# FelTris/durf

Hardware: AMD Instinct MI355X
Metric: train_rays_per_sec (higher is better)
Workload: dtype bf16

## Files before the change

### durf_amd/_sigs.py

```python
import ctypes as C

vp, i32, f32, u64 = C.c_void_p, C.c_int, C.c_float, C.c_size_t

SIGS = {
    'durf_last_error': (C.c_char_p, []),
    'durf_version': (i32, []),
    'durf_dispatch_seen': (i32, []),
    'durf_dispatch_reset': (i32, []),
    'durf_step_policy': (C.c_uint, [u64]),
    'durf_overlap_min_rows': (u64, []),
    'durf_mlp_param_count': (u64, [i32, i32]),
    'durf_mlp_layer_offset': (u64, [i32, i32, i32, i32]),
    'durf_wpack_fwd_bytes': (u64, [i32]),
    'durf_wpack_bwd_bytes': (u64, [i32]),
    'durf_pack_weights': (i32, [vp, i32, i32, vp, vp, vp]),
    'durf_pack_weights_all': (i32, [vp, vp, i32, vp, vp, i32, vp, u64, i32, vp, vp]),
    'durf_ray_setup': (i32, [vp, i32, i32, vp, vp, vp, vp, vp, vp, vp, vp]),
    'durf_ray_setup_masked': (i32, [vp, i32, i32, vp, vp, vp, vp, vp, vp, vp, vp, vp]),
    'durf_compact_hits': (i32, [vp, i32, i32, vp, vp, vp, vp]),
    'durf_compact_classes': (i32, [vp, i32, i32, i32, vp, vp, vp, vp, vp]),
    'durf_compact_all': (i32, [vp, i32, i32, i32, vp, vp, vp, vp, vp, vp, vp, vp]),
    'durf_ray_prologue': (i32, [vp, i32, i32, i32, vp, vp, vp, vp, vp, vp, vp, vp, vp, vp, vp, vp, vp, i32, vp, vp, vp, u64, C.c_uint32, C.c_uint32, vp]),
    'durf_ray_prologue_pack': (i32, [vp, i32, i32, i32, vp, vp, vp, vp, vp, vp, vp, vp, vp, vp, vp, vp, vp, i32, vp, vp, vp, u64, C.c_uint32, C.c_uint32, vp, vp, i32, vp, vp, i32, vp, u64, i32, vp, vp, vp, u64]),
    'durf_ray_prologue_pack_masked': (i32, [vp, i32, i32, i32, vp, vp, vp, vp, vp, vp, vp, vp, vp, vp, vp, vp, vp, i32, vp, vp, vp, u64, C.c_uint32, C.c_uint32, vp, vp, i32, vp, vp, i32, vp, u64, i32, vp, vp, vp, u64, vp]),
# ... 27 lines not shown
    'durf_forward_workspace_bytes': (u64, [i32, i32, i32]),
    'durf_forward': (i32, [vp, vp, vp, u64]),
    'durf_render_image_workspace_bytes': (u64, [i32, i32, i32, i32]),
    'durf_render_image': (i32, [vp, vp, u64, i32, vp, vp, vp, vp, u64]),
    'durf_forward_masked': (i32, [vp, vp, vp, vp, u64]),
    'durf_render_layers_workspace_bytes': (u64, [u64, i32, i32, i32, i32]),
    'durf_render_layers': (i32, [vp, vp, vp, u64, i32, vp, vp, vp, vp, vp, vp, vp, vp, vp, u64]),
    'durf_camera_rays': (i32, [vp, C.POINTER(f32), i32, i32, f32, f32, vp, vp, vp, vp, vp, vp]),
    'durf_render_trajectory_workspace_bytes': (u64, [i32, i32, i32, i32, i32]),
    'durf_render_trajectory': (i32, [vp, vp, vp, vp, i32, i32, C.POINTER(f32), C.POINTER(f32), f32, f32, i32, vp, vp, vp, vp, vp, vp, u64]),
    'durf_train_workspace_bytes': (u64, [i32, i32, i32, i32, u64]),
    'durf_train_workspace_bytes_flags': (u64, [i32, i32, i32, i32, u64, i32]),
    'durf_prefetch_join': (i32, [vp]),
    'durf_loss_backward': (i32, [vp, vp, vp, u64]),
    'durf_train_step': (i32, [vp, vp, vp, u64]),
    'durf_comm_available': (i32, []),
    'durf_comm_unique_id': (i32, [vp]),
    'durf_comm_init': (i32, [i32, i32, vp, C.POINTER(vp)]),
    'durf_comm_destroy': (i32, [vp]),
    'durf_allreduce_sum': (i32, [vp, vp, vp, u64]),
    'durf_mlp_f32_act_floats': (u64, [i32, i32]),
    'durf_mlp_f32_dz_floats': (u64, [i32, i32]),
    'durf_mlp_f32_dw_scratch_floats': (u64, [i32, i32, i32]),
    'durf_mlp_f32_wstream_floats': (u64, [i32]),
    'durf_mlp_f32_pack': (i32, [vp, i32, i32, i32, vp, u64, vp]),
    'durf_mlp_fwd_f32': (i32, [vp, i32, i32, u64, i32, vp, vp, vp, vp, vp, vp, vp, vp]),
    'durf_mlp_bwd_f32': (i32, [vp, i32, i32, u64, i32, vp, vp, vp, vp, vp, vp, vp, vp]),
    'durf_mlp_dw_f32': (i32, [vp, i32, i32, u64, i32, vp, vp, vp, i32, vp, vp]),
    'durf_bkgd_const_trunk_f32': (i32, [vp, vp, vp]),
    'durf_bkgd_hit_rays_f32': (i32, [vp, i32, vp, vp, vp, vp, vp, vp]),
    'durf_objf32_act_stride': (u64, [i32, i32]),
    'durf_objf32_dz_stride': (u64, [i32, i32]),
    'durf_encode_obj_f32_batch': (i32, [vp, i32, i32, i32, vp, vp, vp, vp, vp, vp, C.POINTER(f32), i32, vp]),
    'durf_objf32_fwd_batch': (i32, [vp, i32, i32, i32, vp, vp, vp, vp, vp, u64, vp, vp, vp, vp, vp, vp, vp, C.POINTER(f32), i32]),
    'durf_objf32_bwd_batch': (i32, [vp, i32, i32, i32, vp, vp, vp, vp, u64, vp, vp, vp, vp]),
    'durf_mlp_f32_pack_x3': (i32, [vp, i32, vp, u64, vp]),
    'durf_objf32_bwd_batch_x3': (i32, [vp, i32, i32, i32, vp, vp, vp, vp, u64, vp, vp, vp, vp]),
    'durf_objf32_dw_batch': (i32, [vp, i32, i32, i32, vp, i32, C.POINTER(vp), C.POINTER(vp), i32, vp, vp, u64]),
    'durf_obj_enc_stride': (u64, [i32, i32]),
    'durf_obj_view_stride': (u64, [i32, i32]),
    'durf_obj_dzout_stride': (u64, [i32, i32]),
    'durf_pack_weights_batch': (i32, [vp, i32, i32, i32, vp, u64, vp, vp]),
    'durf_obj_fwd_batch': (i32, [vp, i32, i32, i32, vp, vp, vp, vp, vp, vp, C.POINTER(f32), i32, vp, vp, vp, vp, vp, vp, vp]),
    'durf_obj_bwd_batch': (i32, [vp, i32, i32, i32, vp, vp, vp, vp, vp, vp, vp, vp]),
    'durf_obj_bwd_batch_levels': (i32, [vp, i32, i32, i32, i32, vp, vp, C.POINTER(vp), vp, C.POINTER(vp), C.POINTER(vp), C.POINTER(vp)]),
    'durf_mlp_bwd_obj': (i32, [vp, u64, i32, vp, vp, vp, vp, vp, vp, vp, vp, vp, vp, i32, i32, i32, vp, vp, C.POINTER(vp), vp, C.POINTER(vp), C.POINTER(vp), C.POINTER(vp)]),
    'durf_obj_dw_batch': (i32, [vp, i32, i32, i32, vp, i32, C.POINTER(vp), C.POINTER(vp), C.POINTER(vp), C.POINTER(vp), C.POINTER(vp), i32, vp, vp, vp, u64, vp]),
    'durf_obj_dw_partials': (i32, [vp, i32, i32, i32, vp, i32, C.POINTER(vp), C.POINTER(vp), C.POINTER(vp), C.POINTER(vp), C.POINTER(vp), vp, vp]),
    'durf_dw_finalize_all': (i32, [vp, i32, i32, C.POINTER(u64), C.POINTER(i32), C.POINTER(vp), vp, vp, vp, vp, i32, i32, i32, vp, i32, i32, vp, vp, vp, u64, vp]),
    'durf_encode_obj_bwd': (i32, [vp, i32, i32, i32, vp, vp, vp, vp, vp, vp, vp, vp, vp, vp, C.POINTER(f32), vp, vp, i32, i32]),
    'durf_encode_obj_bwd_batch': (i32, [vp, i32, i32, i32, vp, vp, vp, vp, vp, vp, vp, vp, vp, vp, C.POINTER(f32), vp, vp, i32, i32]),
    'durf_encode_obj_bwd_levels': (i32, [vp, i32, i32, i32, i32, vp, vp, C.POINTER(vp), C.POINTER(vp), vp, vp, vp, vp, vp, vp, C.POINTER(f32), vp, vp, i32, i32]),
    'durf_encode_bkgd_bwd_batch': (i32, [vp, i32, i32, i32, vp, vp, vp, vp, vp, vp, vp, vp, vp, vp, vp, vp, vp, f32, vp, vp, i32]),
    'durf_pose_finish': (i32, [vp, i32, vp, vp, i32, i32, vp]),
    'durf_optim_scratch_floats': (u64, [u64]),
    'durf_stats_scrub': (i32, [vp, i32, i32, i32, vp, vp, vp, vp, vp, vp, C.POINTER(vp), C.POINTER(f32), i32, vp, C.POINTER(vp), i32, u64, vp, f32, f32, vp, vp, u64, i32, u64, u64]),
    'durf_adam_apply': (i32, [vp, u64, vp, vp, vp, vp, f32, f32, i32, vp, vp]),
    'durf_poison_multi_hit': (i32, [vp, u64, vp, vp, u64, i32, u64, u64]),
    'durf_clip_adam': (i32, [vp, u64, vp, vp, vp, vp, f32, f32, f32, f32, i32, vp, vp]),
    'durf_weight_decay': (i32, [vp, u64, vp, vp, u64, u64, f32, vp, vp]),
    'durf_gen_batch': (i32, [vp, i32, i32, C.POINTER(f32), vp, f32, f32, vp, vp, vp, i32, vp, vp, vp, vp, vp, vp, vp, vp, vp, vp]),
    'durf_ssim_scratch_floats': (u64, [i32, i32, i32, i32]),
    'durf_ssim': (i32, [vp, i32, i32, i32, vp, vp, f32, i32, vp, f32, f32, vp, vp, vp]),
    'durf_eval_scratch_bytes': (u64, [i32, i32, i32]),
    'durf_eval_frames': (i32, [vp, i32, i32, i32, vp, vp, vp, vp, vp, vp, vp, u64]),
    'durf_vis_scratch_bytes': (u64, [i32, i32, i32]),
    'durf_vis_stats': (i32, [vp, i32, i32, i32, vp, vp, vp, u64]),
    'durf_vis_depth': (i32, [vp, i32, i32, i32, vp, vp, vp, i32, i32, f32, vp, vp, vp]),
    'durf_vis_normals': (i32, [vp, i32, i32, i32, vp, vp, vp, i32, i32, vp, vp]),
    'durf_vis_sinebow': (i32, [vp, u64, vp, vp, vp]),
    'durf_vis_turbo_lut': (i32, [vp]),
}


DURF_MAX_OBJ = 16
DURF_MAX_LEVELS = 8
DURF_MAX_CAMS = 8
DURF_W_BKGD = 256
DURF_W_OBJ = 128
DURF_ENC_CONTRACT = 1
DURF_ENC_NO_INTEGRATION = 2
DURF_ENC_CYLINDER = 4
DURF_FWD_RAW_FULL = 8
DURF_ENC_DIM = 64
DURF_VIEW_DIM = 32
DURF_DISPATCH_FWD256_8W = 0x1
DURF_DISPATCH_FWD256_4W = 0x2
DURF_DISPATCH_FWD128_SAMPLE = 0x4
DURF_DISPATCH_FWD128_MSPLIT = 0x8
DURF_DISPATCH_BWD256_8W = 0x10
DURF_DISPATCH_BWD256_4W = 0x20
DURF_DISPATCH_BWD128_SAMPLE = 0x40
DURF_DISPATCH_BWD128_MSPLIT = 0x80
DURF_DISPATCH_DW256_256WG = 0x100
DURF_DISPATCH_DW256_512WG = 0x200
DURF_DISPATCH_DW128_128WG = 0x400
DURF_DISPATCH_DW128_256WG = 0x800
DURF_DISPATCH_FWD_ENC = 0x1000
DURF_DISPATCH_FWD_RAW_FULL = 0x2000
DURF_DISPATCH_FWD_TAIL = 0x4000
DURF_DISPATCH_F32_DW_TILE = 0x8000
DURF_DISPATCH_F32_DW_B2 = 0x10000
DURF_DISPATCH_BWD_POSE = 0x20000
DURF_DISPATCH_FWD_MIX = 0x40000
DURF_DISPATCH_BWD_MIX = 0x80000
DURF_LAYERLOG_SELECT = 0x100000
DURF_LAYERLOG_PASS2 = 0x200000
DURF_LAYERLOG_BOX_MASK = 0x400000
DURF_LAYERLOG_TRAJ_RAYS = 0x800000
DURF_LAYERLOG_TRAJ_POSE = 0x1000000
DURF_LAYERLOG_TRAJ_PACK = 0x2000000
DURF_OVERLAP_MIN_ROWS = 262144
DURF_POLICY_SIDE_FWD = 0x1
DURF_POLICY_SIDE_BWD = 0x2
DURF_POLICY_SIDE_DW = 0x4
DURF_POLICY_MSPLIT = 0x8
DURF_POLICY_MIX = 0x10


class durf_loss_level(C.Structure):
    _fields_ = [
        ('raw_bkgd', vp),
        ('raw_obj', vp * DURF_MAX_OBJ),
        ('t_vals', vp),
        ('norm', vp),
        ('mults', f32 * 6),
        ('level', i32),
        ('draw', vp),
        ('terms', vp),
        ('rgb_out', vp),
        ('depth_out', vp),
        ('acc_out', vp),
        ('weights_out', vp),
        ('t_mids_out', vp),
        ('t_dists_out', vp),
        ('draw_ray_sum', vp),
    ]


DURF_FORWARD_MAX_LEVELS = 4


class durf_forward_args(C.Structure):
    _fields_ = [
        ('B', i32),
        ('N', i32),
        ('K', i32),
        ('num_levels', i32),
        ('enc_flags', i32),
        ('lindisp', i32),
        ('bkgd_mode', i32),
        ('density_bias', f32),
        ('resample_padding', f32),
        ('barf_w', f32 * 10),
        ('origins', vp),
        ('directions', vp),
        ('viewdirs', vp),
        ('radii', vp),
        ('near', vp),
        ('far', vp),
        ('pose', vp),
        ('ext', vp),
        ('bkgd_params', vp),
        ('obj_params', vp),
        ('obj_param_stride', u64),
        ('t_rand', vp),
# ... 106 lines not shown
```

### durf_amd/csrc/api.hip

```cpp
#include <stdarg.h>
#include <atomic>
#include <mutex>
#include "durf_common.h"

static thread_local char g_err[512] = "";

void durf_set_error(const char* fmt, ...) {
    va_list ap;
    va_start(ap, fmt);
    vsnprintf(g_err, sizeof(g_err), fmt, ap);
    va_end(ap);
}

static std::atomic<unsigned> g_dispatch{0u};
void durf::note_dispatch(unsigned bits) { g_dispatch.fetch_or(bits, std::memory_order_relaxed); }

int* durf::next_ticket() {
    constexpr int RING = 16384;
    static std::atomic<int*> tab[64];
    static std::atomic<unsigned> next[64];
    static std::mutex mu;
    int dev = 0;
    if (hipGetDevice(&dev) != hipSuccess || dev < 0 || dev >= 64) return nullptr;
    int* base = tab[dev].load(std::memory_order_acquire);
    if (base == nullptr) {
        std::lock_guard<std::mutex> lock(mu);
        base = tab[dev].load(std::memory_order_relaxed);
        if (base == nullptr) {
            int* p = nullptr;
            if (hipMalloc((void**)&p, RING * sizeof(int)) != hipSuccess) return nullptr;
            if (hipMemset(p, 0, RING * sizeof(int)) != hipSuccess || hipDeviceSynchronize() != hipSuccess) {
                (void)hipFree(p);
                return nullptr;
            }
            tab[dev].store(p, std::memory_order_release);
            base = p;
        }
    }
    return base + (next[dev].fetch_add(1u, std::memory_order_relaxed) % RING);
}

extern "C" {
int durf_dispatch_seen(void) { return (int)g_dispatch.load(std::memory_order_relaxed); }
int durf_dispatch_reset(void) { g_dispatch.store(0u, std::memory_order_relaxed); return 0; }
unsigned durf_step_policy(size_t rows) { return durf::step_policy(rows).bits(); }
size_t durf_overlap_min_rows(void) { return DURF_OVERLAP_MIN_ROWS; }
const char* durf_last_error(void) { return g_err; }
int durf_version(void) { return 41; }
}
```

### durf_amd/csrc/durf_common.h

```cpp
#pragma once
#include <hip/hip_runtime.h>
#include <stdint.h>
#include <algorithm>
#include <cstdlib>
#include <stdio.h>
#include "../../include/durf_hip.h"
#include "policy.h"

typedef __bf16 bf16x8 __attribute__((ext_vector_type(8)));
typedef __bf16 bf16x4 __attribute__((ext_vector_type(4)));
typedef __bf16 bf16x2 __attribute__((ext_vector_type(2)));
typedef float f32x16 __attribute__((ext_vector_type(16)));
typedef float f32x4 __attribute__((ext_vector_type(4)));
typedef float f32x2 __attribute__((ext_vector_type(2)));

#define DURF_WAVE 64

void durf_set_error(const char* fmt, ...);
namespace durf {
void note_dispatch(unsigned bits);
int* next_ticket();
}

#define DURF_CHECK_LAUNCH(name)                                              \
// ... 118 lines not shown
#define MS_ENC_SPLIT 1
#endif
#ifndef MS_RING
#define MS_RING 4
#endif
#ifndef MIX_TICKET_WAVE
#define MIX_TICKET_WAVE 1
#endif
template <class T>
__device__ __forceinline__ void load_kernarg(T& dst, const __attribute__((address_space(4))) char* src) {
    static_assert(sizeof(T) % 4 == 0, "whole dwords");
    unsigned* d = (unsigned*)&dst;
    const __attribute__((address_space(4))) unsigned* s = (const __attribute__((address_space(4))) unsigned*)src;
#pragma unroll
    for (int i = 0; i < (int)(sizeof(T) / 4); i++) d[i] = s[i];
}
template <class T> struct kernarg_param { using type = T; };
template <class F> struct kernarg_last;
template <class... P>
struct kernarg_last<void (*)(P...)> {
    using type = typename decltype((kernarg_param<P>{}, ...))::type;
    static constexpr size_t offset_of_last() {
        size_t off = 0, end = 0;
        ((off = (end + alignof(P) - 1) / alignof(P) * alignof(P), end = off + sizeof(P)), ...);
        return off;
    }
    static constexpr size_t offset = offset_of_last();
};

template <class T>
__device__ __forceinline__ T* as_global(T* p) {
#if defined(__HIP_DEVICE_COMPILE__)
    __builtin_assume(!__builtin_amdgcn_is_shared((const void*)p) && !__builtin_amdgcn_is_private((const void*)p));
#endif
    return p;
}

__device__ __forceinline__ void ms_barrier() {
    asm volatile("s_waitcnt lgkmcnt(0)" ::: "memory");
    __builtin_amdgcn_s_barrier();
}

#define DURF_G(T) __attribute__((address_space(1))) T
#define STREAM_STORE(ptr, val) __builtin_nontemporal_store((val), (DURF_G(bf16x8)*)(ptr))

struct FwdStrides { size_t enc, idx, wpack, raw, stash, mask; };
struct EncIn {
    const float* t_vals; const float* origins_s; const float* dirs_s; const float* radii; const int32_t* hit; int K; int flags;
    int obj; float w[10]; void* view_tile; size_t view_stride;
};
struct BwdStrides { size_t idx, wpack, mask, dz, dz_out, d_enc; };
struct DwStrides { size_t enc, view, stash, dz_out, part, bpart; };

namespace durf {
int launch_pack(void* stream, int width, int in_dim, int K, const float* params, size_t param_stride,
                void* wpack_fwd, void* wpack_bwd);
int launch_encode_obj(void* stream, int K, int max_rays, int N, const int32_t* idx, const int32_t* count,
                      const float* t_vals, const float* origins_s, const float* dirs_s, const float* radii,
                      const float* barf_w, int flags, void* out_tile, size_t out_stride, float* out_f32);
int launch_mlp_fwd(void* stream, int width, size_t rows, int N, const void* enc_tile, const void* view_bf16,
                   const int32_t* ray_idx, const int32_t* count, const void* wpack_fwd, float* raw, void* stash,
                   void* relu_mask, int K, const FwdStrides& st, const int32_t* tail_idx = nullptr,
                   const int32_t* tail_count = nullptr, const EncIn* enc_in = nullptr);
int launch_mlp_bwd(void* stream, int width, size_t rows, int N, const float* draw, const int32_t* ray_idx,
                   const int32_t* count, const void* wpack_bwd, const void* relu_mask, void* dz, void* dz_out,
                   float* d_enc, int K, const BwdStrides& st, const int32_t* tail_idx = nullptr,
                   const int32_t* tail_count = nullptr, const float* draw_ray_sum = nullptr);
int launch_mlp_bwd_ms_levels(void* stream, size_t rows, int N, int nlevels, const float* const* draw, const int32_t* ray_idx,
                             const int32_t* count, const void* wpack_bwd, const void* const* relu_mask, void* const* dz,
                             void* const* dz_out, int K, const BwdStrides& st);
int launch_expand_view(void* stream, size_t rows, int N, const void* view_bf16, const int32_t* ray_idx,
                       const int32_t* count, void* out_tile, int K, size_t idx_stride, size_t out_stride,
                       const int32_t* tail_idx = nullptr, const int32_t* tail_count = nullptr);
struct DwLevels {
    size_t rows[DURF_MAX_LEVELS];
    int n[DURF_MAX_LEVELS];
    const int32_t* count[DURF_MAX_LEVELS];
    int nlevels;
};
int launch_mlp_dw(void* stream, int width, const DwLevels& lv,
                  const void* const* enc_tile, const void* const* view_tile, const void* const* stash,
                  const void* const* dz, const void* const* dz_out, float* part, float* bpart, int K,
                  const DwStrides& st);
int launch_dw_finalize(void* stream, int width, int in_dim, const DwLevels& lv,
                       const float* part, const float* bpart, float* grad_mlp, int K, size_t part_stride,
                       size_t bpart_stride, size_t grad_stride, const float* mlp_params, size_t param_stride);
DwLevels uniform_levels(size_t rows, int N, const int32_t* count, int nlevels);
struct DwFinSpec {
    int width, in_dim, K;
    DwLevels lv;
    const float* part; const float* bpart; float* grad; const float* params;
    size_t part_stride, bpart_stride, grad_stride, param_stride;
};
int launch_dw_finalize2(void* stream, const DwFinSpec& a, const DwFinSpec& b);
int launch_layer_chunk(void* stream, int B, int K, const int32_t* hit, const float* rgb, const float* dist, const float* acc,
                       int bkgd_mode, int32_t* instance, float* bg_rgb, float* bg_dist, float* bg_acc, float* obj_rgba);
int launch_layer_compact(void* stream, int n, const int32_t* instance, int32_t* idx, int32_t* count);
int launch_layer_gather(void* stream, int count, const int32_t* idx, const float* const* src, float* const* dst);
int launch_layer_scatter(void* stream, int count, const int32_t* idx, const float* rgb, const float* dist, const float* acc,
                         float* bg_rgb, float* bg_dist, float* bg_acc);
int launch_camera_rays(void* stream, const float* cam_host, int first, int count, float near, float far, float* const* rays);
int launch_pose_interp(void* stream, int F, int K, const float* times_host, const float* box_centers, float* poses);
int launch_frame_pack(void* stream, int count, const float* rgb, uint8_t* rgb8);
}
```

### durf_amd/csrc/mlp_bwd.hip

```cpp
#include <stdlib.h>
#include <cstddef>
#include "mlp_pack.h"


template <int W>
__global__ void __launch_bounds__(256)
k_pack_bwd(int in_dim, const float* __restrict__ P, bf16x8* __restrict__ out, size_t p_stride, size_t out_stride) {
    P += blockIdx.y * p_stride;
    out = (bf16x8*)((char*)out + blockIdx.y * out_stride);
    pack_bwd_vec<W>(in_dim, P, out, blockIdx.x * blockDim.x + threadIdx.x);
}

template <int NA, int NB>
__device__ __forceinline__ void bmma_tile2(const char* slot0, const char* slot1, int lane, const bf16x8* inA,
                                           const bf16x8* inB, f32x16& acc0, f32x16& acc1) {
#pragma unroll
    for (int r = 0; r < 16; r++) { acc0[r] = 0.0f; acc1[r] = 0.0f; }
    mma_pair_ring<NA, NB, BWD_LDS_RING>(slot0, slot1, lane, inA, inB, acc0, acc1, [](auto) {});
}

template <bool MASK>
__device__ __forceinline__ void bpack_tile(const f32x16& acc, unsigned word, int t, bf16x8& o0, bf16x8& o1) {
#pragma unroll
    for (int e = 0; e < 8; e++) {
// ... 469 lines not shown
            msb_bwd_pair(ow, kp->lv.draw[level], kp->lv.relu_mask[level], kp->lv.dz[level], kp->lv.dz_out[level], lds, lane, role,
                         live, k, pair);
        });
  }
}

__global__ void __launch_bounds__(256)
k_expand_view(size_t rows, int N, const bf16x8* __restrict__ view, const int32_t* __restrict__ ray_idx,
              const int32_t* __restrict__ count, bf16x8* __restrict__ out, size_t idx_stride, size_t out_stride,
              const int32_t* __restrict__ tail_idx, const int32_t* __restrict__ tail_count) {
    if (gridDim.y > 1) {
        ray_idx += blockIdx.y * idx_stride;
        count += blockIdx.y;
        out = (bf16x8*)((char*)out + blockIdx.y * out_stride);
    }
    const size_t gid = (size_t)blockIdx.x * blockDim.x + threadIdx.x;
    const size_t row = gid >> 2;
    const int q = (int)(gid & 3);
    size_t nrows = rows;
    if (count) { const size_t c = (size_t)(*count) * N; nrows = c < rows ? c : rows; }
    const size_t nrows_c = nrows;
    if (tail_count) {
        const size_t t = nrows_c + (size_t)(*tail_count);
        nrows = t < rows ? t : rows;
        if (row >= nrows && row < ((nrows + 31) & ~(size_t)31)) {
            const bf16x8 z = {0, 0, 0, 0, 0, 0, 0, 0};
            *(bf16x8*)((char*)out + tile_vec_offset(row, q, 2)) = z;
        }
    }
    if (row >= nrows) return;
    size_t ray = row / (size_t)N;
    if (tail_count && row >= nrows_c) ray = (size_t)tail_idx[row - nrows_c];
    else if (ray_idx) ray = (size_t)ray_idx[ray];
    *(bf16x8*)((char*)out + tile_vec_offset(row, q, 2)) = view[ray * 4 + q];
}

typedef short s16x4 __attribute__((ext_vector_type(4)));
typedef short s16x8 __attribute__((ext_vector_type(8)));

__device__ __forceinline__ bf16x8 tr_frag(const char* base, int off0, int off1) {
    const s16x4 r0 = __builtin_amdgcn_ds_read_tr16_b64_v4i16((__attribute__((address_space(3))) s16x4*)(base + off0));
    const s16x4 r1 = __builtin_amdgcn_ds_read_tr16_b64_v4i16((__attribute__((address_space(3))) s16x4*)(base + off1));
    const s16x8 r = {r0[0], r0[1], r0[2], r0[3], r1[0], r1[1], r1[2], r1[3]};
    return __builtin_bit_cast(bf16x8, r);
}

#ifndef DW_LDS_KB
#define DW_LDS_KB 144
#endif
#ifndef DW_MAX_STAGES
#define DW_MAX_STAGES 4
#endif
#define DW_LDS_BYTES (DW_LDS_KB * 1024)
__host__ __device__ constexpr int dw_stages(int nc) { return DW_LDS_BYTES / (nc * 1024) > DW_MAX_STAGES ? DW_MAX_STAGES : DW_LDS_BYTES / (nc * 1024); }

#define DW_DMA_POLICY " nt"
__device__ __forceinline__ void lds_dma16(i32x4 rsrc, unsigned soff, unsigned voff, unsigned lds_addr) {
    unsigned keep;
    asm volatile("s_nop 4\n\t"
                 "s_mov_b32 %0, m0\n\t"
                 "s_mov_b32 m0, %1\n\t"
                 "s_nop 0\n\t"
                 "buffer_load_dwordx4 %2, %3, %4 offen" DW_DMA_POLICY " lds\n\t"
                 "s_mov_b32 m0, %0"
                 : "=&s"(keep)
                 : "s"(lds_addr), "v"(voff), "s"(rsrc), "s"(soff)
                 : "memory");
}

struct DwArgs {
    const char* dz[DURF_MAX_LEVELS][12];
    const char* inA[DURF_MAX_LEVELS][12];
    const char* inB[DURF_MAX_LEVELS][12];
    int nlevels;
    const char* dz2[DURF_MAX_LEVELS];
    size_t ks_dz2;
    size_t ks_dz[12], ks_a[12], ks_b[12];
    size_t ks_part, ks_bpart;
    float* part[12];
    float* bpart[12];
    int nsplit[12];
    int first_wg[13];
    int order[12];
};

#ifndef DW_MIN_TPS
#define DW_MIN_TPS 48
#endif
__host__ __device__ inline size_t dw_tiles_per_split(size_t nt_all, int nsplit) {
    const size_t even = (nt_all + nsplit - 1) / nsplit;
    size_t floor_ = DW_MIN_TPS;
    const size_t small = (nt_all + 15) / 16;
    if (small < floor_) floor_ = small < 8 ? 8 : small;
    return even > floor_ ? even : floor_;
}

__host__ __device__ inline size_t dw_level_tiles(const durf::DwLevels& lv, int l, size_t obj) {
    size_t nrows = lv.rows[l];
#if defined(__HIP_DEVICE_COMPILE__)
    if (lv.count[l]) { const size_t c = (size_t)lv.count[l][obj] * (size_t)lv.n[l]; nrows = c < nrows ? c : nrows; }
#endif
    return (nrows + 31) >> 5;
}

template <int NKO, int NKA, int NKB, int NKO2 = 0>
__device__ __forceinline__ void dw_job(const durf::DwLevels& lv, const DwArgs& a, int job,
                                       int nsplit, int split_idx, float* __restrict__ part,
                                       float* __restrict__ bpart, char* smem) {
    constexpr int NKI = NKA + NKB;
    constexpr int NC = NKO + NKI;
    constexpr int CPW = (NC + 7) / 8;
    constexpr int MO = (NKO + 1) / 2, NI = NKI / 2;
    constexpr int RM = (MO + 3) / 4, RN = (NI + 1) / 2;
    constexpr int STAGE = NC * 1024;
    constexpr int S = dw_stages(NC);
    const int lane = threadIdx.x & 63;
    const int wave = __builtin_amdgcn_readfirstlane(threadIdx.x >> 6);
    const int wm = wave >> 1, wn = wave & 1;
    const size_t obj = blockIdx.y;
    if (gridDim.y > 1) { part += obj * a.ks_part; bpart += obj * a.ks_bpart; }
    size_t nt_all = 0;
    for (int l = 0; l < a.nlevels; l++) nt_all += dw_level_tiles(lv, l, obj);
    const size_t tps = dw_tiles_per_split(nt_all, nsplit);
    const size_t g0 = (size_t)split_idx * tps;
    if (g0 >= nt_all) return;
    size_t g1 = g0 + tps;
    if (g1 > nt_all) g1 = nt_all;
    const unsigned lds0 = (unsigned)(size_t)(__attribute__((address_space(3))) char*)smem;
    const int g_hif = lane >> 5, g_p = lane & 31;
    unsigned voff[2];
#pragma unroll
    for (int par = 0; par < 2; par++) {
        const int c = 2 * par + g_hif;
        const int n = (g_p & 16) | ((g_p - 4 * c) & 15);
        voff[par] = (unsigned)((g_hif * 32 + n) * 16);
    }
    constexpr int NKO1 = NKO - NKO2;
    i32x4 r_dz, r_a, r_b, r_dz2;
    auto stage_load = [&](int ti, int slot) {
        ti = __builtin_amdgcn_readfirstlane(ti);
        const unsigned dst = lds0 + (unsigned)(slot * STAGE);
#pragma unroll
        for (int i = 0; i < CPW; i++) {
            int ci = wave + 8 * i;
            if (ci >= NC) ci -= NC;
            if (ci < NKO1) {
                lds_dma16(r_dz, (unsigned)((ti * NKO1 + ci) * 1024), voff[ci & 1], dst + ci * 1024);
            } else if (NKO2 > 0 && ci < NKO) {
                lds_dma16(r_dz2, (unsigned)((ti * NKO2 + ci - NKO1) * 1024), voff[ci & 1], dst + ci * 1024);
            } else if (ci < NKO + NKA) {
                const int ks = ci - NKO;
                lds_dma16(r_a, (unsigned)((ti * NKA + ks) * 1024), voff[ks & 1], dst + ci * 1024);
            } else {
                const int ks = ci - NKO - NKA;
                lds_dma16(r_b, (unsigned)((ti * NKB + ks) * 1024), voff[(ks + NKA) & 1], dst + ci * 1024);
            }
        }
    };
    const int g = lane >> 4, L = lane & 15;
    const int ksp = g & 1, hi = g >> 1, j = L >> 2, q = L & 3, hi_f = q >> 1, half = q & 1;
    const int cc = 2 * ksp + hi_f;
    const int lane_off = hi_f * 512 + half * 8;
    const int poff0 = ((8 * hi + 0 + j + 4 * cc) & 15) * 16;
    const int poff1 = ((8 * hi + 4 + j + 4 * cc) & 15) * 16;

    f32x16 acc[RM][RN];
#pragma unroll
    for (int rm = 0; rm < RM; rm++)
#pragma unroll
        for (int rn = 0; rn < RN; rn++)
#pragma unroll
            for (int r = 0; r < 16; r++) acc[rm][rn][r] = 0.0f;
    float bsum[RM];
#pragma unroll
    for (int rm = 0; rm < RM; rm++) bsum[rm] = 0.0f;

    size_t lo = 0, hi_t = 0;
    for (int lvl = 0; lvl < a.nlevels; lvl++) {
        lo = hi_t;
        hi_t = lo + dw_level_tiles(lv, lvl, obj);
        const size_t b0 = g0 > lo ? g0 : lo, b1 = g1 < hi_t ? g1 : hi_t;
        if (b1 <= b0) continue;
        const size_t t0 = b0 - lo;
        const int nt = (int)(b1 - b0);
        r_dz = make_rsrc(a.dz[lvl][job] + obj * a.ks_dz[job] + t0 * NKO1 * 1024);
        r_dz2 = make_rsrc(NKO2 ? a.dz2[lvl] + obj * a.ks_dz2 + t0 * (NKO2 ? NKO2 : 1) * 1024 : a.dz[lvl][job]);
        r_a = make_rsrc(a.inA[lvl][job] + obj * a.ks_a[job] + t0 * NKA * 1024);
        r_b = make_rsrc(NKB ? a.inB[lvl][job] + obj * a.ks_b[job] + t0 * (NKB ? NKB : 1) * 1024 : a.inA[lvl][job]);
        __builtin_amdgcn_s_barrier();
#pragma unroll
        for (int i = 0; i < S - 1; i++)
            if (i < nt) stage_load(i, i);
        for (int t = 0; t < nt; t++) {
            const int later = nt - 1 - t;
            if (later >= S - 2) asm volatile("s_waitcnt vmcnt(%0)" ::"n"((S - 2) * CPW) : "memory");
            else asm volatile("s_waitcnt vmcnt(0)" ::: "memory");
            __builtin_amdgcn_s_barrier();
            if (t + S - 1 < nt) stage_load(t + S - 1, (t + S - 1) % S);
            const char* st = smem + (t % S) * STAGE;
#pragma unroll
            for (int kk = 0; kk < 2; kk++) {
                bf16x8 af[RM], bf[RN];
#pragma unroll
                for (int rm = 0; rm < RM; rm++) {
                    const int mo = wm + 4 * rm;
                    if (mo < MO) {
                        int ks = 2 * mo + ksp;
                        if (ks > NKO - 1) ks = NKO - 1;
                        const char* base = st + ks * 1024 + lane_off + kk * 256;
                        af[rm] = tr_frag(base, poff0, poff1);
                    }
                }
#pragma unroll
                for (int rn = 0; rn < RN; rn++) {
                    const int ni = wn + 2 * rn;
                    if (ni < NI) {
                        const char* base = st + (NKO + 2 * ni + ksp) * 1024 + lane_off + kk * 256;
                        bf[rn] = tr_frag(base, poff0, poff1);
                    }
                }
#pragma unroll
                for (int rm = 0; rm < RM; rm++) {
                    if (wm + 4 * rm < MO) {
#pragma unroll
                        for (int rn = 0; rn < RN; rn++)
                            if (wn + 2 * rn < NI)
                                acc[rm][rn] = __builtin_amdgcn_mfma_f32_32x32x16_bf16(af[rm], bf[rn], acc[rm][rn], 0, 0, 0);
                        if (wn == 0) {
                            float s = 0.0f;
#pragma unroll
                            for (int e = 0; e < 8; e++) s += (float)af[rm][e];
                            bsum[rm] += s;
                        }
                    }
                }
            }
        }
    }
    const size_t sp = (size_t)split_idx;
#pragma unroll
    for (int rm = 0; rm < RM; rm++) {
        const int mo = wm + 4 * rm;
        if (mo < MO) {
#pragma unroll
            for (int rn = 0; rn < RN; rn++) {
                const int ni = wn + 2 * rn;
                if (ni < NI) {
                    float* dst = part + (((sp * MO + mo) * NI + ni) * 64 + lane) * 16;
#pragma unroll
                    for (int v = 0; v < 4; v++) {
                        const f32x4 o = {acc[rm][rn][4 * v], acc[rm][rn][4 * v + 1], acc[rm][rn][4 * v + 2], acc[rm][rn][4 * v + 3]};
                        *(f32x4*)(dst + 4 * v) = o;
                    }
                }
            }
            if (wn == 0) {
                const float tot = bsum[rm] + __shfl_xor(bsum[rm], 32, 64);
                if (lane < 32) bpart[(sp * MO + mo) * 32 + lane] = tot;
            }
        }
    }
}



template <int W>
__global__ void __launch_bounds__(512, 2)
k_dw_all(durf::DwLevels lv, DwArgs a) {
    using S = MlpSpec<W>;
    extern __shared__ __attribute__((aligned(16))) char smem[];
    int oi = 0;
#pragma unroll
    for (int i = 1; i < 12; i++) oi += ((int)blockIdx.x >= a.first_wg[i]) ? 1 : 0;
    const int job = a.order[oi], sp = (int)blockIdx.x - a.first_wg[oi];
    const int ns = a.nsplit[job];
#define DW_CALL(...) dw_job<__VA_ARGS__>(lv, a, job, ns, sp, a.part[job], a.bpart[job], smem)
    switch (job) {
        case 0: DW_CALL(S::KW, S::KE, 0); break;
        case 5: DW_CALL(S::KW, S::KW, S::KE); break;
        case 8: if (W != 256) DW_CALL(1, S::KW, 0); break;
        case 10:
            if (W == 256) DW_CALL(S::KC + 1, S::KW, S::KV, 1);
            else DW_CALL(S::KC, S::KW, S::KV);
            break;
        case 11: DW_CALL(1, S::KC, 0); break;
        default: DW_CALL(S::KW, S::KW, 0); break;
    }
#undef DW_CALL
}

__host__ __device__ inline int cperm_slot(int f) {
    const int w = f & 15;
    return 16 * (f >> 4) + 8 * ((w >> 2) & 1) + (w & 3) + 4 * (w >> 3);
}

struct DwJob {
    int layer;
    int out_nat_off;
    int in_perm_rows;
    int in_nat_base;
    int MO, NI;
};

__host__ __device__ inline int cperm_feat(int s) {
    const int e = s & 7;
    return 16 * (s >> 4) + (e & 3) + 8 * (e >> 2) + 4 * ((s >> 3) & 1);
}

struct DwJobs { DwJob j[12]; size_t part_off[12], bpart_off[12]; int nparts[12]; };

struct FinMlp {
    int W, in_dim, count, NI10;
    DwJobs jobs;
    const float* part; const float* bpart; float* grad; const float* params;
    size_t part_stride, bpart_stride, grad_stride, param_stride;
    durf::DwLevels lv;
};
struct FinArgs { FinMlp m[2]; int job_blk[2][13]; };

__global__ void __launch_bounds__(256)
k_dw_finalize(FinArgs A) {
    const int n0 = A.m[0].count * A.job_blk[0][12];
    const int cls = (int)blockIdx.x < n0 ? 0 : 1;
    const FinMlp& M = A.m[cls];
    const int rel = (int)blockIdx.x - (cls ? n0 : 0);
    const size_t obj = rel / A.job_blk[cls][12];
    const int rb = rel % A.job_blk[cls][12];
    int jb = 0;
#pragma unroll
    for (int j = 1; j < 12; j++) jb += (rb >= A.job_blk[cls][j]) ? 1 : 0;
    const int xblk = rb - A.job_blk[cls][jb];
    const int W = M.W, in_dim = M.in_dim;
    const DwJobs& jobs = M.jobs;
    const durf::DwLevels& lv = M.lv;
    const float* part_all = M.part + obj * M.part_stride;
    const float* bpart_all = M.bpart + obj * M.bpart_stride;
    float* grad_mlp = M.grad + obj * M.grad_stride;
    size_t nt_all = 0;
    for (int l = 0; l < lv.nlevels; l++) nt_all += dw_level_tiles(lv, l, obj);
    const DwJob job = jobs.j[jb];
    const size_t tps_ = dw_tiles_per_split(nt_all, jobs.nparts[jb]);
    const int nparts = (int)((nt_all + tps_ - 1) / tps_);
    const float* part = part_all + jobs.part_off[jb];
    const float* bpart = bpart_all + jobs.bpart_off[jb];
    int fi, fo;
    durf_layer_shape(W, in_dim, job.layer, &fi, &fo);
    const int nfrag = job.MO * job.NI * 1024;
    const int nb = job.MO * 32;
    const int idx0 = (xblk * 256 + (int)threadIdx.x) * 4;
    if (idx0 >= nfrag + nb) return;
    f32x4 s4 = {0.0f, 0.0f, 0.0f, 0.0f};
    {
        const float* p0 = idx0 < nfrag ? part + idx0 : bpart + (idx0 - nfrag);
        const size_t stride = idx0 < nfrag ? (size_t)nfrag : (size_t)nb;
        for (int p = 0; p < nparts; p += 8) {
            f32x4 v[8];
#pragma unroll
            for (int u = 0; u < 8; u++) v[u] = (p + u < nparts) ? *(const f32x4*)(p0 + (size_t)(p + u) * stride) : f32x4{0.0f, 0.0f, 0.0f, 0.0f};
#pragma unroll
            for (int u = 0; u < 8; u++)
                if (p + u < nparts) { s4[0] += v[u][0]; s4[1] += v[u][1]; s4[2] += v[u][2]; s4[3] += v[u][3]; }
// ... 350 lines not shown
}

int launch_mlp_bwd(void* stream, int width, size_t rows, int N, const float* draw, const int32_t* ray_idx,
                   const int32_t* count, const void* wpack_bwd, const void* relu_mask, void* dz, void* dz_out,
                   float* d_enc, int K, const BwdStrides& st, const int32_t* tail_idx, const int32_t* tail_count,
                   const float* draw_ray_sum) {
    DURF_REQUIRE(width == 256 || width == 128, "width must be 256 or 128");
    DURF_REQUIRE(rows % 32 == 0, "rows must be a multiple of 32");
    DURF_REQUIRE(K == 1 || (ray_idx && count), "batched launches are for compacted object rays");
    if (rows == 0 || K <= 0) return 0;
    hipStream_t s = (hipStream_t)stream;
    if (width == 128 && ray_idx && count && !d_enc && !tail_idx && step_policy(rows).msplit) {
        MsBwdLevels lv{};
        lv.draw[0] = draw; lv.relu_mask[0] = (const uint4*)relu_mask; lv.dz[0] = (bf16x8*)dz; lv.dz_out[0] = (bf16x8*)dz_out; lv.n = 1;
        const MsBwd A{rows, N, lv, ray_idx, count, (const char*)wpack_bwd, st, K, nullptr};
        hipLaunchKernelGGL(k_mlp_bwd_ms, dim3(ms_grid((size_t)K * durf_cdiv(rows, 64))), dim3(256), msb::LDS_BYTES, s, A);
        DURF_CHECK_LAUNCH("durf_mlp_bwd (M-split)");
        note_dispatch(DURF_DISPATCH_BWD128_MSPLIT);
        return 0;
    }
    const MlpBlockShape shape = mlp_block_shape(width, K, rows, d_enc != nullptr);
    const bool half = shape.half;
    dim3 grid(shape.grid_x, K), block(shape.block);
#define LAUNCH_B(WW, PP, NWV)                                                                              \
    {                                                                                                      \
        constexpr int lds = 2 * 4 * (MlpSpec<WW>::KW + 1) * 1024;                                          \
        dynamic_lds_once<k_mlp_bwd<WW, PP, NWV>>(lds);                                                       \
        hipLaunchKernelGGL((k_mlp_bwd<WW, PP, NWV>), grid, block, lds, s, rows, N, draw, ray_idx, count,    \
                           (const char*)wpack_bwd, (const uint4*)relu_mask, (bf16x8*)dz, (bf16x8*)dz_out,  \
                           d_enc, st, tail_idx, tail_count, draw_ray_sum, MsBwd{});                        \
    }
    if (half) LAUNCH_B(256, false, 4)
    else if (width == 256) { if (d_enc) LAUNCH_B(256, true, 8) else LAUNCH_B(256, false, 8) }
    else { if (d_enc) LAUNCH_B(128, true, 8) else LAUNCH_B(128, false, 8) }
#undef LAUNCH_B
    DURF_CHECK_LAUNCH("durf_mlp_bwd");
    note_dispatch((width == 128 ? DURF_DISPATCH_BWD128_SAMPLE : (half ? DURF_DISPATCH_BWD256_4W : DURF_DISPATCH_BWD256_8W)) |
                  (d_enc ? DURF_DISPATCH_BWD_POSE : 0u));
    return 0;
}

int launch_mlp_bwd_ms_levels(void* stream, size_t rows, int N, int nlevels, const float* const* draw, const int32_t* ray_idx,
                             const int32_t* count, const void* wpack_bwd, const void* const* relu_mask, void* const* dz,
                             void* const* dz_out, int K, const BwdStrides& st) {
    DURF_REQUIRE(nlevels >= 1 && nlevels <= DURF_MAX_LEVELS && rows % 32 == 0 && ray_idx && count, "1 <= nlevels <= DURF_MAX_LEVELS, compacted rays");
    if (rows == 0 || K <= 0) return 0;
    MsBwdLevels lv{};
    lv.n = nlevels;
    for (int l = 0; l < nlevels; l++) {
        lv.draw[l] = draw[l]; lv.relu_mask[l] = (const uint4*)relu_mask[l]; lv.dz[l] = (bf16x8*)dz[l]; lv.dz_out[l] = (bf16x8*)dz_out[l];
    }
    const MsBwd A{rows, N, lv, ray_idx, count, (const char*)wpack_bwd, st, K, nullptr};
    hipLaunchKernelGGL(k_mlp_bwd_ms, dim3(ms_grid((size_t)nlevels * K * durf_cdiv(rows, 64))), dim3(256), msb::LDS_BYTES, (hipStream_t)stream, A);
    DURF_CHECK_LAUNCH("durf_obj_bwd_batch_levels (M-split)");
    note_dispatch(DURF_DISPATCH_BWD128_MSPLIT);
    return 0;
}

int launch_expand_view(void* stream, size_t rows, int N, const void* view_bf16, const int32_t* ray_idx,
                       const int32_t* count, void* out_tile, int K, size_t idx_stride, size_t out_stride,
                       const int32_t* tail_idx, const int32_t* tail_count) {
    if (rows == 0 || K <= 0) return 0;
    hipLaunchKernelGGL(k_expand_view, dim3(durf_cdiv(rows * 4, 256), K), dim3(256), 0, (hipStream_t)stream, rows, N,
                       (const bf16x8*)view_bf16, ray_idx, count, (bf16x8*)out_tile, idx_stride, out_stride, tail_idx,
                       tail_count);
    DURF_CHECK_LAUNCH("durf_expand_view");
    return 0;
}

DwLevels uniform_levels(size_t rows, int N, const int32_t* count, int nlevels) {
    DwLevels lv;
    lv.nlevels = nlevels;
    for (int l = 0; l < DURF_MAX_LEVELS; l++) { lv.rows[l] = rows; lv.n[l] = N; lv.count[l] = count; }
    return lv;
}

int launch_mlp_dw(void* stream, int width, const DwLevels& lv,
                  const void* const* enc_tile, const void* const* view_tile, const void* const* stash,
                  const void* const* dz, const void* const* dz_out, float* part, float* bpart, int K,
                  const DwStrides& st) {
    const int nlevels = lv.nlevels;
    DURF_REQUIRE(width == 256 || width == 128, "width must be 256 or 128");
    DURF_REQUIRE(nlevels >= 1 && nlevels <= DURF_MAX_LEVELS, "1 <= nlevels <= DURF_MAX_LEVELS");
    size_t total_rows = 0;
    for (int l = 0; l < nlevels; l++) {
        DURF_REQUIRE(lv.rows[l] % 32 == 0, "rows must be a multiple of 32");
        DURF_REQUIRE(K == 1 || lv.count[l], "batched launches are for compacted object rays");
        total_rows += lv.rows[l];
    }
    if (total_rows == 0 || K <= 0) return 0;
    hipStream_t s = (hipStream_t)stream;
    const DwPlan P = dw_plan(width, total_rows);
    {
        const DwPlan big = dw_plan(width);
        DURF_REQUIRE(P.part_total <= big.part_total && P.bpart_total <= big.bpart_total, "split plan exceeds the partial buffers");
    }
    const int KW = width / 16;
    auto region = [&](const void* base, int j, int l) { return (const char*)base + ((size_t)j * KW * (lv.rows[l] >> 5)) * 1024; };
    DwArgs a;
    a.nlevels = nlevels;
    a.ks_part = st.part; a.ks_bpart = st.bpart;
    a.ks_dz2 = st.dz_out;
    for (int j = 0; j < 12; j++) {
        a.ks_dz[j] = (j == 8 || j == 11) ? st.dz_out : st.stash;
        a.ks_a[j] = j == 0 ? st.enc : st.stash;
        a.ks_b[j] = j == 5 ? st.enc : (j == 10 ? st.view : 0);
    }
    for (int j = 0; j < 12; j++) {
        a.part[j] = part + P.part_off[j];
        a.bpart[j] = bpart + P.bpart_off[j];
        a.nsplit[j] = P.nsplit[j];
    }
    for (int l = 0; l < DURF_MAX_LEVELS; l++) {
        const int ll = l < nlevels ? l : 0;
        for (int j = 0; j < 12; j++) {
            a.inB[l][j] = nullptr;
            if (j <= 7) {
                a.dz[l][j] = region(dz[ll], j, ll);
                a.inA[l][j] = j == 0 ? (const char*)enc_tile[ll] : region(stash[ll], j - 1, ll);
            }
        }
        a.inB[l][5] = (const char*)enc_tile[ll];
        a.dz[l][8] = (const char*)dz_out[ll]; a.inA[l][8] = region(stash[ll], 7, ll);
        a.dz2[l] = (const char*)dz_out[ll];
        a.dz[l][9] = nullptr; a.inA[l][9] = nullptr;
        a.dz[l][10] = region(dz[ll], 9, ll); a.inA[l][10] = region(stash[ll], 7, ll); a.inB[l][10] = (const char*)view_tile[ll];
        a.dz[l][11] = (const char*)dz_out[ll]; a.inA[l][11] = region(stash[ll], 9, ll);
    }
    static const int order[12] = {11, 8, 0, 10, 5, 1, 2, 3, 4, 6, 7, 9};
    int total = 0;
    for (int i = 0; i < 12; i++) {
        a.order[i] = order[i];
        a.first_wg[i] = total;
        total += P.nsplit[order[i]];
    }
    a.first_wg[12] = total;
    dim3 grid(total, K), block(512);
    if (width == 256) {
        constexpr int lds = DW_LDS_BYTES;
        (void)hipFuncSetAttribute((const void*)k_dw_all<256>, hipFuncAttributeMaxDynamicSharedMemorySize, lds);
        hipLaunchKernelGGL(k_dw_all<256>, grid, block, lds, s, lv, a);
    } else {
        constexpr int lds = dw_stages(20) * 20 * 1024;
        (void)hipFuncSetAttribute((const void*)k_dw_all<128>, hipFuncAttributeMaxDynamicSharedMemorySize, lds);
        hipLaunchKernelGGL(k_dw_all<128>, grid, block, lds, s, lv, a);
    }
    DURF_CHECK_LAUNCH("durf_mlp_dw");
    note_dispatch(width == 256 ? (P.total_wgs <= 256 ? DURF_DISPATCH_DW256_256WG : DURF_DISPATCH_DW256_512WG)
                               : (P.total_wgs <= 128 ? DURF_DISPATCH_DW128_128WG : DURF_DISPATCH_DW128_256WG));
    return 0;
}

static int fin_class(FinMlp& M, int width, int in_dim, const DwLevels& lv, const float* part, const float* bpart,
                     float* grad_mlp, int K, size_t part_stride, size_t bpart_stride, size_t grad_stride,
                     const float* mlp_params, size_t param_stride, int* max_el, int* max_tiles) {
    DURF_REQUIRE(mlp_params != nullptr, "the bottleneck gradients need the MLP's parameters");
    DURF_REQUIRE(width == 256 || width == 128, "width must be 256 or 128");
    const int W = width, KW = W / 16;
    size_t total_rows = 0;
    for (int l = 0; l < lv.nlevels; l++) total_rows += lv.rows[l];
    const DwPlan P = dw_plan(width, total_rows);
    M.W = W; M.in_dim = in_dim; M.count = K; M.NI10 = P.NI[10];
    M.part = part; M.bpart = bpart; M.grad = grad_mlp; M.params = mlp_params;
    M.part_stride = part_stride; M.bpart_stride = bpart_stride; M.grad_stride = grad_stride; M.param_stride = param_stride;
    M.lv = lv;
    for (int job = 0; job < 12; job++) {
        DwJob& J = M.jobs.j[job];
        J.layer = job;
        J.out_nat_off = -1;
        J.in_perm_rows = W; J.in_nat_base = KW * 16;
        if (job == 0) { J.in_perm_rows = 0; J.in_nat_base = 0; }
        else if (job == 8) { J.out_nat_off = 3; }
        else if (job == 11) { J.out_nat_off = 0; J.in_perm_rows = 128; J.in_nat_base = 128; }
        J.MO = P.MO[job]; J.NI = P.NI[job];
        M.jobs.part_off[job] = P.part_off[job];
        M.jobs.bpart_off[job] = P.bpart_off[job];
        M.jobs.nparts[job] = P.nsplit[job];
        const int el = J.MO * J.NI * 1024 + J.MO * 32;
        if (el > *max_el) *max_el = el;
    }
    const int ntiles = (W / 32) * (W / 32) + (W / 32) * 4;
    if (ntiles > *max_tiles) *max_tiles = ntiles;
    return 0;
}

static int launch_fin(void* stream, FinArgs& A, int max_el, int max_tiles) {
    const int n = A.m[0].count + A.m[1].count;
    if (n <= 0) return 0;
    hipStream_t s = (hipStream_t)stream;
    int total = 0;
    for (int c = 0; c < 2; c++) {
        int b = 0;
        for (int j = 0; j < 12; j++) {
            A.job_blk[c][j] = b;
            if (A.m[c].count > 0 && A.m[c].jobs.nparts[j] > 0)
                b += durf_cdiv(A.m[c].jobs.j[j].MO * A.m[c].jobs.j[j].NI * 1024 + A.m[c].jobs.j[j].MO * 32, 1024);
        }
        A.job_blk[c][12] = b > 0 ? b : 1;
        total += A.m[c].count * b;
    }
    (void)max_el;
    hipLaunchKernelGGL(k_dw_finalize, dim3(total), dim3(256), 0, s, A);
    hipLaunchKernelGGL(k_bottleneck_grads, dim3(max_tiles, n), dim3(256), 0, s, A);
    DURF_CHECK_LAUNCH("durf_mlp_dw_finalize");
    return 0;
}

int launch_dw_finalize(void* stream, int width, int in_dim, const DwLevels& lv,
                       const float* part, const float* bpart, float* grad_mlp, int K, size_t part_stride,
                       size_t bpart_stride, size_t grad_stride, const float* mlp_params, size_t param_stride) {
    if (K <= 0) return 0;
// ... 24 lines not shown
```

### durf_amd/csrc/mlp_fwd.hip

```cpp
#include <stdlib.h>
#include <cstddef>
#include "mlp_pack.h"
#include "enc_lane.h"

template <int W>
__global__ void __launch_bounds__(256)
k_pack_fwd(int in_dim, const float* __restrict__ P, bf16x8* __restrict__ out, size_t p_stride, size_t out_stride) {
    P += blockIdx.y * p_stride;
    out = (bf16x8*)((char*)out + blockIdx.y * out_stride);
    pack_fwd_vec<W>(in_dim, P, out, blockIdx.x * blockDim.x + threadIdx.x);
}

__global__ void __launch_bounds__(256)
k_pack_all(PackAll a) {
    pack_all_vec(a, (int)blockIdx.y, (int)(blockIdx.x * blockDim.x + threadIdx.x));
}

template <int NA, int NB>
__device__ __forceinline__ f32x16 mma_tile(const char* slot, int lane, const bf16x8* inA,
                                           const bf16x8* inB) {
    const f32x4* bp = (const f32x4*)(slot + (NA + NB) * 1024 + (lane >> 5) * 64);
    f32x16 acc;
#pragma unroll
    for (int g = 0; g < 4; g++) {
        const f32x4 b4 = bp[g];
        acc[4 * g + 0] = b4[0]; acc[4 * g + 1] = b4[1]; acc[4 * g + 2] = b4[2]; acc[4 * g + 3] = b4[3];
    }
    const char* ap = slot + lane * 16;
#pragma unroll
    for (int ks = 0; ks < NA; ks++) {
        const bf16x8 a = *(const bf16x8*)(ap + ks * 1024);
        acc = __builtin_amdgcn_mfma_f32_32x32x16_bf16(a, inA[ks], acc, 0, 0, 0);
    }
#pragma unroll
    for (int ks = 0; ks < NB; ks++) {
        const bf16x8 a = *(const bf16x8*)(ap + (NA + ks) * 1024);
        acc = __builtin_amdgcn_mfma_f32_32x32x16_bf16(a, inB[ks], acc, 0, 0, 0);
    }
    return acc;
}

template <int NA, int NB, bool SPREAD = false>
__device__ __forceinline__ void mma_tile2(const char* slot0, const char* slot1, int lane, const bf16x8* inA,
                                          const bf16x8* inB, f32x16& acc0, f32x16& acc1,
                                          const bf16x8* sv = nullptr, char* sp = nullptr, bool do_store = false) {
    constexpr int T = NA + NB;
    const f32x4* bp0 = (const f32x4*)(slot0 + (NA + NB) * 1024 + (lane >> 5) * 64);
    const f32x4* bp1 = (const f32x4*)(slot1 + (NA + NB) * 1024 + (lane >> 5) * 64);
#pragma unroll
    for (int g = 0; g < 4; g++) {
        const f32x4 b0 = bp0[g], b1 = bp1[g];
        acc0[4 * g + 0] = b0[0]; acc0[4 * g + 1] = b0[1]; acc0[4 * g + 2] = b0[2]; acc0[4 * g + 3] = b0[3];
        acc1[4 * g + 0] = b1[0]; acc1[4 * g + 1] = b1[1]; acc1[4 * g + 2] = b1[2]; acc1[4 * g + 3] = b1[3];
    }
    mma_pair_ring<NA, NB, FWD_LDS_RING>(slot0, slot1, lane, inA, inB, acc0, acc1, [&](auto ks_) {
        constexpr int ks = decltype(ks_)::value;
        if constexpr (SPREAD) {
            static_for<0, 4>([&](auto q_) {
                constexpr int q = decltype(q_)::value;
                if constexpr (ks == (q + 1) * T / 4 - 1) {
                    __builtin_amdgcn_sched_barrier(0);
                    if (do_store) STREAM_STORE(sp + q * 1024, sv[q]);
                    __builtin_amdgcn_sched_barrier(0);
                }
            });
        }
    });
}

template <bool RELU, bool BITS>
__device__ __forceinline__ unsigned pack_tile(const f32x16& acc, bf16x8& o0, bf16x8& o1) {
    static_assert(RELU || !BITS, "mask bits are taken from the ReLU output");
#pragma unroll
    for (int e = 0; e < 8; e++) {
        float v0 = acc[e], v1 = acc[8 + e];
        if (RELU) {
            v0 = __builtin_amdgcn_fmed3f(v0, 0.0f, 3.0e38f);
            v1 = __builtin_amdgcn_fmed3f(v1, 0.0f, 3.0e38f);
        }
        o0[e] = (__bf16)v0;
        o1[e] = (__bf16)v1;
    }
    unsigned bits = 0;
    if (BITS) {
        typedef unsigned u32x4_ __attribute__((ext_vector_type(4)));
        const u32x4_ d0 = __builtin_bit_cast(u32x4_, o0), d1 = __builtin_bit_cast(u32x4_, o1);
        const unsigned ones = 0x00010001u;
#pragma unroll
        for (int j = 0; j < 8; j++) {
            unsigned t;
            const unsigned d = j < 4 ? d0[j & 3] : d1[j & 3];
            asm("v_pk_min_u16 %0, %1, %2" : "=v"(t) : "v"(d), "s"(ones));
            asm("v_lshl_or_b32 %0, %1, %2, %0" : "+v"(bits) : "v"(t), "n"(j));
        }
    }
    return bits;
}

template <int SLOT, int NA, int NB, int NMT, bool RELU, bool TRAIN, int PREV_NMT, bool STORE_OUT = true>
__device__ __forceinline__ void run_stage(WPipe& p, const bf16x8* inA, const bf16x8* inB,
                                          bf16x8* out, int next_stage_chunks, char* stash_dst,
                                          bool valid, const bf16x8* prev_out, char* prev_dst,
                                          char* prev_mask_dst, uint4& mask_carry) {
    constexpr int CH = NA + NB + 1;
    constexpr int G = group_tiles(NMT, CH, SLOT);
    static_assert(NMT % 2 == 0 && G % 2 == 0, "stages processed by run_stage have an even tile count");
    unsigned mb[4] = {0u, 0u, 0u, 0u};
    const char* slot = nullptr;
#pragma unroll
    for (int mo = 0; mo < NMT; mo += 2) {
        if (mo % G == 0) {
            const int rest = NMT - mo - G;
            slot = p.begin(rest > 0 ? (rest < G ? rest : G) * CH : next_stage_chunks);
        }
        f32x16 acc0, acc1;
        const char* s0 = slot + (mo % G) * CH * 1024;
        const char* s1 = slot + (mo % G + 1) * CH * 1024;
        if (TRAIN) {
            if (mo > 0 && STORE_OUT) {
                mma_tile2<NA, NB, true>(s0, s1, p.lane, inA, inB, acc0, acc1, out + 2 * mo - 4,
                                        stash_dst + (2 * mo - 4) * 1024 + p.lane * 16, valid);
                if (valid) p.since += 4;
            } else if (mo == 0 && PREV_NMT > 0) {
                const bool st = valid && prev_dst != nullptr;
                mma_tile2<NA, NB, true>(s0, s1, p.lane, inA, inB, acc0, acc1, prev_out + 2 * PREV_NMT - 4,
                                        prev_dst + (2 * PREV_NMT - 4) * 1024 + p.lane * 16, st);
                if (st) p.since += 4;
                if (valid && prev_mask_dst) *(uint4*)(prev_mask_dst + p.lane * 16) = mask_carry;
            } else {
                mma_tile2<NA, NB>(s0, s1, p.lane, inA, inB, acc0, acc1);
            }
        } else {
            mma_tile2<NA, NB>(s0, s1, p.lane, inA, inB, acc0, acc1);
        }
        constexpr bool BITS = TRAIN && RELU;
        const unsigned bits0 = pack_tile<RELU, BITS>(acc0, out[2 * mo], out[2 * mo + 1]);
        const unsigned bits1 = pack_tile<RELU, BITS>(acc1, out[2 * mo + 2], out[2 * mo + 3]);
        if (TRAIN && RELU) mb[mo >> 1] |= bits0 | (bits1 << 8);
    }
    if (TRAIN && RELU) mask_carry = make_uint4(mb[0], mb[1], mb[2], mb[3]);
}


namespace ms {
using S = MlpSpec<128>;
constexpr int NT = 2;
constexpr int X_BYTES = NT * S::KW * 1024;
constexpr int OFF_X = 0;
constexpr int OFF_E = 2 * X_BYTES;
constexpr int OFF_V = OFF_E + NT * S::KE * 1024;
constexpr int OFF_M = OFF_V + NT * S::KV * 1024;
constexpr int LDS_BYTES = OFF_M + 2 * NT * 4 * 64 * 4;
}

struct MsFwd {
    size_t rows; int N; const bf16x8* enc; const bf16x8* view; const int32_t* ray_idx; const int32_t* count; const char* wpack;
    float* raw; bf16x8* stash; uint4* relu_mask; FwdStrides bs; EncIn ei; int nobj;
    int* ticket;
};
__device__ __forceinline__ size_t ms_pairs_of(const MsFwd& A, int k) {
    const size_t c = (size_t)as_global(A.count)[k] * (size_t)A.N;
    return ((c < A.rows ? c : A.rows) + 32 * ms::NT - 1) / (32 * ms::NT);
}
__device__ __forceinline__ bool ms_item(const MsFwd& A, size_t item, size_t& k_out, size_t& pair_out) {
    size_t k = 0, pair = item;
    for (; k < (size_t)A.nobj; k++) {
        const size_t np = ms_pairs_of(A, (int)k);
        if (pair < np) break;
        pair -= np;
    }
    const bool ok = k < (size_t)A.nobj;
    k_out = (size_t)__builtin_amdgcn_readfirstlane((unsigned)(ok ? k : 0));
    pair_out = ok ? pair : 0;
    return ok;
}

#ifndef MS_PROBE_ONEW
#define MS_PROBE_ONEW 0
#endif
#ifndef MS_PROBE_NOSTORE
// ... 421 lines not shown
    const size_t tile32 = blk * NWV + wave;
    const size_t row = tile32 * 32 + (lane & 31);
    const bool valid = row < nrows;
    const bool tile_valid = tile32 * 32 < nrows;

    const bf16x8 zero8 = {0, 0, 0, 0, 0, 0, 0, 0};
    const bool tail = tail_count != nullptr && tile32 * 32 >= nrows_c;
    auto const_enc = [&](int k) -> bf16x8 {
        bf16x8 v;
#pragma unroll
        for (int e = 0; e < 8; e++) {
            const int f = 16 * k + 8 * (lane >> 5) + e;
            v[e] = (f >= 30 && f < 60) ? (__bf16)1.0f : (__bf16)0.0f;
        }
        return v;
    };
    bf16x8 encf[S::KE];
    const char* enc_u = (const char*)enc + tile32 * (S::KE * 1024);
    if constexpr (ENC) {
#pragma unroll
        for (int k = 0; k < S::KE; k++) encf[k] = (tile_valid && tail) ? const_enc(k) : zero8;
        if (tile_valid && !tail) {
            const int j = (int)(row / (size_t)N), n = (int)(row % (size_t)N);
            const int b = ray_idx ? ray_idx[j] : j;
            const bool hi = lane >= 32;
            auto keep = [&](auto q_, const bf16x8& o8) {
                constexpr int q = decltype(q_)::value;
                if (hi == (bool)(q & 1)) encf[q >> 1] = o8;
            };
            if constexpr (W == 128) {
                const float t0 = ei.t_vals[(size_t)b * (N + 1) + n], t1 = ei.t_vals[(size_t)b * (N + 1) + n + 1];
                float o[3] = {ei.origins_s[b * 3], ei.origins_s[b * 3 + 1], ei.origins_s[b * 3 + 2]};
                float d[3] = {ei.dirs_s[b * 3], ei.dirs_s[b * 3 + 1], ei.dirs_s[b * 3 + 2]};
                Gauss g = frustum_gaussian(t0, t1, o, d, ei.radii[b], (ei.flags & DURF_ENC_CYLINDER) != 0);
                if (ei.flags & DURF_ENC_NO_INTEGRATION) g.var[0] = g.var[1] = g.var[2] = 0.0f;
                BarfW bw;
#pragma unroll
                for (int i = 0; i < 10; i++) bw.w[i] = ei.w[i];
                lane_features<true>(g, bw, keep);
            } else {
                const Gauss g = bkgd_sample_gaussian(b, n, N, ei.t_vals, ei.origins_s, ei.dirs_s, ei.radii, ei.hit, ei.K, ei.flags);
                lane_features<false>(g, BarfW{}, keep);
            }
        }
        if (tile_valid && (TRAIN || !tail)) {
#pragma unroll
            for (int k = 0; k < S::KE; k++) *(bf16x8*)(const_cast<char*>(enc_u) + k * 1024 + lane * 16) = encf[k];
            p.since += S::KE;
        }
    } else {
#pragma unroll
        for (int k = 0; k < S::KE; k++)
            encf[k] = tile_valid ? (tail ? const_enc(k) : *(const bf16x8*)(enc_u + k * 1024 + lane * 16)) : zero8;
        if (TRAIN && tail && tile_valid) {
#pragma unroll
            for (int k = 0; k < S::KE; k++) *(bf16x8*)(const_cast<char*>(enc_u) + k * 1024 + lane * 16) = encf[k];
            p.since += S::KE;
        }
    }
    bool poison = false;
#pragma unroll
    for (int k = 0; k < S::KE; k++)
#pragma unroll
        for (int e = 0; e < 8; e++) {
            const float f = (float)encf[k][e];
            poison |= !(fabsf(f) <= 3.0e38f);
        }
    poison |= (__shfl_xor((int)poison, 32, 64) != 0);

    bf16x8 a[S::KW], b[S::KW];
    auto stash_at = [&](int j) -> char* {
        return (char*)stash + ((size_t)S::stash_ks_before(j) * ntile32 + tile32 * S::stash_ks(j)) * 1024;
    };
    auto mask_at = [&](int j) -> char* {
        return relu_mask ? (char*)relu_mask + ((size_t)j * ntile32 + tile32) * 1024 : nullptr;
    };
    constexpr int CHW = S::KW + 1;
    constexpr int GW = group_tiles(S::WT, CHW, SLOT) * CHW;
    constexpr int G5 = group_tiles(S::WT, S::KW + S::KE + 1, SLOT) * (S::KW + S::KE + 1);
    constexpr int G9 = group_tiles(S::CT, S::KW + S::KV + 1, SLOT) * (S::KW + S::KV + 1);
    uint4 mcarry = make_uint4(0u, 0u, 0u, 0u);
#define ST(j) (TRAIN ? stash_at(j) : nullptr)
#define MK(j) (TRAIN ? mask_at(j) : nullptr)
    run_stage<SLOT, 0, S::KE, S::WT, true, TRAIN, 0>(p, nullptr, encf, a, GW, ST(0), tile_valid, nullptr, nullptr, nullptr, mcarry);
    run_stage<SLOT, S::KW, 0, S::WT, true, TRAIN, S::WT>(p, a, nullptr, b, GW, ST(1), tile_valid, a, ST(0), MK(0), mcarry);
    run_stage<SLOT, S::KW, 0, S::WT, true, TRAIN, S::WT>(p, b, nullptr, a, GW, ST(2), tile_valid, b, ST(1), MK(1), mcarry);
    run_stage<SLOT, S::KW, 0, S::WT, true, TRAIN, S::WT>(p, a, nullptr, b, GW, ST(3), tile_valid, a, ST(2), MK(2), mcarry);
    run_stage<SLOT, S::KW, 0, S::WT, true, TRAIN, S::WT>(p, b, nullptr, a, G5, ST(4), tile_valid, b, ST(3), MK(3), mcarry);
    bf16x8 encs[S::KE];
#pragma unroll
    for (int k = 0; k < S::KE; k++)
        encs[k] = tile_valid ? (tail ? const_enc(k) : *(const bf16x8*)(enc_u + k * 1024 + lane * 16)) : zero8;
    run_stage<SLOT, S::KW, S::KE, S::WT, true, TRAIN, S::WT>(p, a, encs, b, GW, ST(5), tile_valid, a, ST(4), MK(4), mcarry);
    run_stage<SLOT, S::KW, 0, S::WT, true, TRAIN, S::WT>(p, b, nullptr, a, GW, ST(6), tile_valid, b, ST(5), MK(5), mcarry);
    run_stage<SLOT, S::KW, 0, S::WT, true, TRAIN, S::WT>(p, a, nullptr, b, GW, ST(7), tile_valid, a, ST(6), MK(6), mcarry);
    run_stage<SLOT, S::KW, 0, S::WT, false, TRAIN, S::WT, false>(p, b, nullptr, a, CHW, nullptr, tile_valid, b, ST(7), MK(7), mcarry);
    float dens;
    {
        const char* slot = p.begin(G9);
        const f32x16 acc = mma_tile<S::KW, 0>(slot, lane, b, nullptr);
        dens = acc[0];
    }
    bf16x8 vf[S::KV];
    {
        size_t ray = row / (size_t)N;
        if (tail) ray = valid ? (size_t)tail_idx[row - nrows_c] : 0;
        else if (ray_idx && valid) ray = (size_t)ray_idx[ray];
        unsigned hi_v = (unsigned)lane;
        if (ENC) asm volatile("" : "+v"(hi_v));
        hi_v >>= 5;
#pragma unroll
        for (int k = 0; k < S::KV; k++)
            vf[k] = valid ? view[ray * (DURF_VIEW_DIM / 8) + 2 * k + hi_v] : zero8;
        if constexpr (ENC) {
            if (TRAIN && ei.view_tile && tile_valid) {
#pragma unroll
                for (int k = 0; k < S::KV; k++) *(bf16x8*)((char*)ei.view_tile + (tile32 * S::KV + k) * 1024 + lane * 16) = vf[k];
                p.since += S::KV;
            }
        }
    }
    bf16x8 c[S::KC];
    run_stage<SLOT, S::KW, S::KV, S::CT, true, TRAIN, S::WT>(p, a, vf, c, S::KC + 1, ST(9), tile_valid, a, nullptr, nullptr, mcarry);
    {
        p.gnext = 0;
        const char* slot = p.begin(has_next ? G0 : 0);
        if (TRAIN && tile_valid) {
#pragma unroll
            for (int q = 4; q >= 1; q--) STREAM_STORE(ST(9) + (2 * S::CT - q) * 1024 + lane * 16, c[2 * S::CT - q]);
            p.since += 4;
            if (MK(8)) {
                unsigned lo = (unsigned)lane * 16u;
                asm volatile("" : "+v"(lo));
                *(uint4*)(MK(8) + lo) = mcarry;
            }
        }
        const f32x16 acc = mma_tile<S::KC, 0>(slot, lane, c, nullptr);
        const float qn = __builtin_nanf("");
        const float o0 = poison ? qn : acc[0], o1 = poison ? qn : acc[1], o2 = poison ? qn : acc[2], o3 = poison ? qn : dens;
        const f32x4 o = {o0, o1, o2, o3};
        bool scattered = false;
        if constexpr (ENC) scattered = (ei.flags & DURF_FWD_RAW_FULL) != 0 && ray_idx != nullptr;
        if (!scattered) {
            if (valid && lane < 32) *(f32x4*)(raw + row * 4) = o;
        } else if (!tail) {
            const unsigned row0 = __builtin_amdgcn_readfirstlane((unsigned)(tile32 * 32));
            unsigned Nu = (unsigned)N;
            asm volatile("" : "+s"(Nu));
            const unsigned j = row0 / Nu;
            const unsigned b = (unsigned)ray_idx[tile_valid ? j : 0u];
            unsigned l31 = (unsigned)lane;
            asm volatile("" : "+v"(l31));
            l31 &= 31u;
            if (valid && lane < 32) *(f32x4*)(raw + ((size_t)(b * Nu + (row0 - j * Nu)) + l31) * 4) = o;
        } else if (tile_valid) {
            unsigned l64 = (unsigned)lane;
            asm volatile("" : "+v"(l64));
            const unsigned l31 = l64 & 31u;
            const unsigned ti = __builtin_amdgcn_readfirstlane((unsigned)(tile32 * 32 - nrows_c));
            const int rr = (valid && lane < 32) ? tail_idx[ti + l31] : -1;
#pragma unroll 1
            for (int r = 0; r < 32; r++) {
                const int ray = __builtin_amdgcn_readlane(rr, r);
                if (ray < 0) break;
                const float v0 = __builtin_bit_cast(float, __builtin_amdgcn_readlane(__builtin_bit_cast(int, o0), r));
                const float v1 = __builtin_bit_cast(float, __builtin_amdgcn_readlane(__builtin_bit_cast(int, o1), r));
                const float v2 = __builtin_bit_cast(float, __builtin_amdgcn_readlane(__builtin_bit_cast(int, o2), r));
                const float v3 = __builtin_bit_cast(float, __builtin_amdgcn_readlane(__builtin_bit_cast(int, o3), r));
                const f32x4 v = {v0, v1, v2, v3};
                float* dst = raw + (size_t)((unsigned)ray * (unsigned)N) * 4;
                for (unsigned n = l64; n < (unsigned)N; n += 64) *(f32x4*)(dst + (size_t)n * 4) = v;
            }
        }
    }
#undef ST
#undef MK
  }
  if constexpr (MIX) {
    if (has_block) __builtin_amdgcn_s_setprio(0);
    ms_barrier();
    mix_object_items<decltype(&k_mlp_fwd<W, TRAIN, NWV, ENC, MIX>), MsFwd, ms::LDS_BYTES, false>(smem, wave, (int)gridDim.x, ms_pairs_of,
                                                                                                 ms_fwd_pair<TRAIN>);
  }
}

extern "C" {

size_t durf_mlp_param_count(int width, int in_dim) { return durf_layer_offset(width, in_dim, 12, 0); }
size_t durf_mlp_layer_offset(int width, int in_dim, int layer, int want_bias) {
    return durf_layer_offset(width, in_dim, layer, want_bias);
}
size_t durf_wpack_fwd_bytes(int width) {
    return (size_t)(width == 256 ? MlpSpec<256>::TOTAL_CHUNKS : MlpSpec<128>::TOTAL_CHUNKS) * 1024;
}
size_t durf_mlp_mask_bytes(size_t rows) { return ((rows + 31) / 32) * 9 * 1024; }
size_t durf_mlp_stash_bytes(int width, size_t rows) {
    const size_t kb = width == 256 ? MlpSpec<256>::STASH_KS_TOTAL : MlpSpec<128>::STASH_KS_TOTAL;
    return ((rows + 31) / 32) * kb * 1024;
}

int durf_pack_weights_all(void* stream, const float* bkgd_params, int in_bkgd, void* bkgd_fwd, void* bkgd_bwd, int K,
                          const float* obj_params, size_t obj_param_stride, int in_obj, void* obj_fwd, void* obj_bwd) {
    DURF_REQUIRE(bkgd_params == nullptr || (bkgd_fwd != nullptr && in_bkgd > 0 && in_bkgd <= DURF_ENC_DIM),
                 "background MLP: forward stream and 1 <= in_dim <= 64");
    DURF_REQUIRE(K == 0 || (obj_params != nullptr && obj_fwd != nullptr && in_obj > 0 && in_obj <= DURF_ENC_DIM),
                 "object MLPs: parameters, forward streams and 1 <= in_dim <= 64");
    if (K < 0 || (bkgd_params == nullptr && K == 0)) return 0;
    PackAll a;
    a.p_bkgd = bkgd_params; a.f_bkgd = (bf16x8*)bkgd_fwd; a.b_bkgd = (bf16x8*)bkgd_bwd; a.in_bkgd = in_bkgd;
    a.p_obj = obj_params; a.f_obj = (bf16x8*)obj_fwd; a.b_obj = (bf16x8*)obj_bwd; a.in_obj = in_obj;
    a.p_stride = obj_param_stride; a.f_stride = durf_wpack_fwd_bytes(128); a.b_stride = durf_wpack_bwd_bytes(128);
    size_t nv = durf_wpack_fwd_bytes(256) / 16 + durf_wpack_bwd_bytes(256) / 16;
    if (bkgd_params == nullptr) nv = durf_wpack_fwd_bytes(128) / 16 + durf_wpack_bwd_bytes(128) / 16;
    hipLaunchKernelGGL(k_pack_all, dim3(durf_cdiv(nv, 256), 1 + K), dim3(256), 0, (hipStream_t)stream, a);
    DURF_CHECK_LAUNCH("durf_pack_weights_all");
    return 0;
}

int durf_pack_weights(void* stream, int width, int in_dim, const float* mlp_params, void* wpack_fwd,
                      void* wpack_bwd) {
    return durf::launch_pack(stream, width, in_dim, 1, mlp_params, 0, wpack_fwd, wpack_bwd);
}

static int fwd_enc_args(size_t rows, int N, const float* t_vals, const float* origins_s, const float* dirs_s, const float* radii,
                        const int32_t* hit, int K, int enc_flags, const void* enc_tile, const int32_t* ray_idx, const int32_t* count,
                        const void* stash, const int32_t* tail_idx, const int32_t* tail_count, void* view_tile, EncIn* ei) {
    DURF_REQUIRE((tail_idx == nullptr) == (tail_count == nullptr), "tail_idx and tail_count go together");
    DURF_REQUIRE(tail_idx == nullptr || (count != nullptr && N % 32 == 0), "tail rows follow a compacted ray list");
    DURF_REQUIRE((ray_idx == nullptr) == (count == nullptr), "ray_idx and count go together");
    DURF_REQUIRE(view_tile == nullptr || stash != nullptr, "the view-direction tile is a training output");
    DURF_REQUIRE(t_vals && origins_s && dirs_s && radii && enc_tile, "ray data and the encoding tile buffer are required");
    DURF_REQUIRE(K >= 0 && K <= DURF_MAX_OBJ && (K == 0 || hit != nullptr), "0 <= K <= DURF_MAX_OBJ, hit [B,K]");
    DURF_REQUIRE(N > 0 && (count != nullptr ? N % 32 == 0 : rows % 32 == 0), "whole 32-sample tiles");
    DURF_REQUIRE(!(enc_flags & DURF_FWD_RAW_FULL) || rows < ((size_t)1 << 32), "DURF_FWD_RAW_FULL: 32-bit row numbers");
    *ei = EncIn{};
    ei->t_vals = t_vals; ei->origins_s = origins_s; ei->dirs_s = dirs_s; ei->radii = radii; ei->hit = hit; ei->K = K; ei->flags = enc_flags;
    ei->view_tile = view_tile;
    return 0;
}

int durf_mlp_fwd_enc(void* stream, size_t rows, int N, const float* t_vals, const float* origins_s, const float* dirs_s,
                     const float* radii, const int32_t* hit, int K, int enc_flags, void* enc_tile, const void* view_bf16,
                     const int32_t* ray_idx, const int32_t* count, const void* wpack_fwd, float* raw, void* stash,
                     void* relu_mask, const int32_t* tail_idx, const int32_t* tail_count, void* view_tile) {
    EncIn ei;
    if (int rc = fwd_enc_args(rows, N, t_vals, origins_s, dirs_s, radii, hit, K, enc_flags, enc_tile, ray_idx, count, stash, tail_idx,
                              tail_count, view_tile, &ei)) return rc;
    return durf::launch_mlp_fwd(stream, 256, rows, N, enc_tile, view_bf16, ray_idx, count, wpack_fwd, raw, stash,
                                relu_mask, 1, FwdStrides{}, tail_idx, tail_count, &ei);
}

int durf_mlp_fwd_enc_obj(void* stream, size_t rows, int N, const float* t_vals, const float* origins_s, const float* dirs_s,
                         const float* radii, const int32_t* hit, int K, int enc_flags, void* enc_tile, const void* view_bf16,
                         const int32_t* ray_idx, const int32_t* count, const void* wpack_fwd, float* raw, void* stash,
                         void* relu_mask, const int32_t* tail_idx, const int32_t* tail_count, void* view_tile,
                         int B, const int32_t* obj_idx, const int32_t* obj_count, const float* barf_w, int obj_flags,
                         const void* obj_wpack_fwd, void* obj_enc, float* obj_raw, void* obj_stash, void* obj_relu_mask,
                         void* obj_view_tile) {
    DURF_REQUIRE(K > 0 && B > 0 && (size_t)B * N == rows, "K object MLPs over rows = B * N sample rows");
    DURF_REQUIRE(obj_idx && obj_count && barf_w && obj_wpack_fwd && obj_enc && obj_raw, "the object launch's buffers");
    DURF_REQUIRE((stash == nullptr) == (obj_stash == nullptr), "training or inference: both MLP classes alike");
    const bool mix = durf::step_policy(rows).mix_enabled && stash != nullptr && obj_relu_mask != nullptr && N % 32 == 0 && ray_idx != nullptr;
    if (!mix) {
        int rc = durf_mlp_fwd_enc(stream, rows, N, t_vals, origins_s, dirs_s, radii, hit, K, enc_flags, enc_tile, view_bf16, ray_idx,
                                  count, wpack_fwd, raw, stash, relu_mask, tail_idx, tail_count, view_tile);
        if (rc) return rc;
        return durf_obj_fwd_batch(stream, K, B, N, obj_idx, obj_count, t_vals, origins_s, dirs_s, radii, barf_w, obj_flags, view_bf16,
                                  obj_wpack_fwd, obj_enc, obj_raw, obj_stash, obj_relu_mask, obj_view_tile);
    }
    EncIn ei;
    if (int rc = fwd_enc_args(rows, N, t_vals, origins_s, dirs_s, radii, hit, K, enc_flags, enc_tile, ray_idx, count, stash, tail_idx,
                              tail_count, view_tile, &ei)) return rc;
    MsFwd ow{};
    ow.rows = rows; ow.N = N; ow.enc = (const bf16x8*)obj_enc; ow.view = (const bf16x8*)view_bf16; ow.ray_idx = obj_idx;
    ow.count = obj_count; ow.wpack = (const char*)obj_wpack_fwd; ow.raw = obj_raw; ow.stash = (bf16x8*)obj_stash;
    ow.relu_mask = (uint4*)obj_relu_mask; ow.nobj = K;
    ow.bs.enc = durf_obj_enc_stride(B, N); ow.bs.idx = (size_t)B; ow.bs.wpack = durf_wpack_fwd_bytes(DURF_W_OBJ);
    ow.bs.raw = rows * 4 * sizeof(float); ow.bs.stash = durf_mlp_stash_bytes(DURF_W_OBJ, rows); ow.bs.mask = durf_mlp_mask_bytes(rows);
    ow.ei.t_vals = t_vals; ow.ei.origins_s = origins_s; ow.ei.dirs_s = dirs_s; ow.ei.radii = radii;
    ow.ei.flags = obj_flags & (DURF_ENC_NO_INTEGRATION | DURF_ENC_CYLINDER); ow.ei.obj = 1;
    for (int i = 0; i < 10; i++) ow.ei.w[i] = barf_w[i];
    ow.ei.view_tile = obj_view_tile; ow.ei.view_stride = durf_obj_view_stride(B, N);
    ow.ticket = durf::next_ticket();
    DURF_REQUIRE(ow.ticket != nullptr, "no item counter for the mixed launch (device allocation failed)");
#ifdef DURF_MIX_PROBES
    if (const char* pr = getenv("DURF_MIX_PROBE")) {
        if (pr[0] == '1') ow.nobj = 0;
        if (pr[0] == '2') ei.flags |= 1 << 30;
    }
#endif
    const unsigned g = mix_launch_grid<k_mlp_fwd<256, true, 8, true, true>, ms::LDS_BYTES>(rows, (size_t)K * durf_cdiv(rows, 64));
    hipLaunchKernelGGL((k_mlp_fwd<256, true, 8, true, true>), dim3(g), dim3(512), MIX_LDS_BYTES, (hipStream_t)stream, rows, N, (const bf16x8*)enc_tile,
                       (const bf16x8*)view_bf16, ray_idx, count, (const char*)wpack_fwd, raw, (bf16x8*)stash, (uint4*)relu_mask,
                       FwdStrides{}, tail_idx, tail_count, ei, ow);
    DURF_CHECK_LAUNCH("durf_mlp_fwd_enc_obj");
    durf::note_dispatch(DURF_DISPATCH_FWD256_8W | DURF_DISPATCH_FWD_ENC | DURF_DISPATCH_FWD_MIX | (tail_idx ? DURF_DISPATCH_FWD_TAIL : 0u) |
                        ((enc_flags & DURF_FWD_RAW_FULL) ? DURF_DISPATCH_FWD_RAW_FULL : 0u));
    return 0;
}

int durf_mlp_fwd(void* stream, int width, size_t rows, int N, const void* enc_tile,
                 const void* view_bf16, const int32_t* ray_idx, const int32_t* count,
                 const void* wpack_fwd, float* raw, void* stash, void* relu_mask,
                 const int32_t* tail_idx, const int32_t* tail_count) {
    DURF_REQUIRE((tail_idx == nullptr) == (tail_count == nullptr), "tail_idx and tail_count go together");
    DURF_REQUIRE(tail_idx == nullptr || (count != nullptr && N % 32 == 0), "tail rows follow a compacted ray list");
    return durf::launch_mlp_fwd(stream, width, rows, N, enc_tile, view_bf16, ray_idx, count, wpack_fwd, raw, stash,
                                relu_mask, 1, FwdStrides{}, tail_idx, tail_count);
}

}

namespace durf {

int pack_bwd_launch(void* stream, int width, int in_dim, int K, const float* params, size_t param_stride, void* wpack_bwd);

int launch_pack(void* stream, int width, int in_dim, int K, const float* params, size_t param_stride,
                void* wpack_fwd, void* wpack_bwd) {
    DURF_REQUIRE(width == 256 || width == 128, "width must be 256 or 128");
    DURF_REQUIRE(in_dim > 0 && in_dim <= DURF_ENC_DIM, "in_dim <= 64");
    if (K <= 0) return 0;
    hipStream_t s = (hipStream_t)stream;
    if (wpack_fwd) {
        const size_t ostride = durf_wpack_fwd_bytes(width);
        if (width == 256)
            hipLaunchKernelGGL(k_pack_fwd<256>, dim3(durf_cdiv(MlpSpec<256>::TOTAL_CHUNKS * 64, 256), K), dim3(256), 0, s,
                               in_dim, params, (bf16x8*)wpack_fwd, param_stride, ostride);
        else
            hipLaunchKernelGGL(k_pack_fwd<128>, dim3(durf_cdiv(MlpSpec<128>::TOTAL_CHUNKS * 64, 256), K), dim3(256), 0, s,
                               in_dim, params, (bf16x8*)wpack_fwd, param_stride, ostride);
        DURF_CHECK_LAUNCH("durf_pack_weights (fwd)");
    }
    if (wpack_bwd) return pack_bwd_launch(stream, width, in_dim, K, params, param_stride, wpack_bwd);
    return 0;
}

int launch_mlp_fwd(void* stream, int width, size_t rows, int N, const void* enc_tile, const void* view_bf16,
                   const int32_t* ray_idx, const int32_t* count, const void* wpack_fwd, float* raw, void* stash,
                   void* relu_mask, int K, const FwdStrides& st, const int32_t* tail_idx, const int32_t* tail_count,
                   const EncIn* enc_in) {
    DURF_REQUIRE(width == 256 || width == 128, "width must be 256 or 128");
    const bool msplit = width == 128 && ray_idx && count && step_policy(rows).msplit;
    DURF_REQUIRE(enc_in == nullptr || (width == 256 && K == 1 && !enc_in->obj) || (width == 128 && ray_idx && count && (enc_in->obj || msplit)),
                 "the self-encoding forward: the background MLP, or the object MLPs on their compacted ray lists");
    DURF_REQUIRE(rows % 32 == 0, "rows must be a multiple of 32");
    DURF_REQUIRE(K == 1 || (ray_idx && count), "batched launches are for compacted object rays");
    if (rows == 0 || K <= 0) return 0;
    hipStream_t s = (hipStream_t)stream;
    const MlpBlockShape shape = mlp_block_shape(width, K, rows, false);
    const bool half = shape.half;
    dim3 grid(shape.grid_x, K), block(shape.block);
    const EncIn ei = enc_in ? *enc_in : EncIn{};
    if (msplit) {
        dim3 g(ms_grid((size_t)K * durf_cdiv(rows, 64))), b(256);
        const MsFwd A{rows, N, (const bf16x8*)enc_tile, (const bf16x8*)view_bf16, ray_idx, count, (const char*)wpack_fwd, raw,
                      (bf16x8*)stash, (uint4*)relu_mask, st, ei, K, nullptr};
        if (stash)
            hipLaunchKernelGGL((k_mlp_fwd_ms<true>), g, b, ms::LDS_BYTES, s, A);
        else
            hipLaunchKernelGGL((k_mlp_fwd_ms<false>), g, b, ms::LDS_BYTES, s, A);
        DURF_CHECK_LAUNCH("durf_mlp_fwd (M-split)");
        note_dispatch(DURF_DISPATCH_FWD128_MSPLIT | (ei.obj ? DURF_DISPATCH_FWD_ENC : 0u));
        return 0;
    }
#define LAUNCH_F(WW, TR, NWV, EN)                                                                 \
    {                                                                                             \
        constexpr int lds = 2 * 4 * (MlpSpec<WW>::KW + 1) * 1024;                                 \
        dynamic_lds_once<k_mlp_fwd<WW, TR, NWV, EN>>(lds);                                        \
        hipLaunchKernelGGL((k_mlp_fwd<WW, TR, NWV, EN>), grid, block, lds, s, rows, N, (const bf16x8*)enc_tile, \
                           (const bf16x8*)view_bf16, ray_idx, count, (const char*)wpack_fwd, raw,  \
                           (bf16x8*)stash, (uint4*)relu_mask, st, tail_idx, tail_count, ei, MsFwd{}); \
    }
    if (enc_in && width == 128) { if (stash) LAUNCH_F(128, true, 8, true) else LAUNCH_F(128, false, 8, true) }
    else if (enc_in) {
        if (half) { if (stash) LAUNCH_F(256, true, 4, true) else LAUNCH_F(256, false, 4, true) }
        else { if (stash) LAUNCH_F(256, true, 8, true) else LAUNCH_F(256, false, 8, true) }
    }
    else if (half) { if (stash) LAUNCH_F(256, true, 4, false) else LAUNCH_F(256, false, 4, false) }
    else if (width == 256) { if (stash) LAUNCH_F(256, true, 8, false) else LAUNCH_F(256, false, 8, false) }
    else { if (stash) LAUNCH_F(128, true, 8, false) else LAUNCH_F(128, false, 8, false) }
#undef LAUNCH_F
    DURF_CHECK_LAUNCH("durf_mlp_fwd");
    note_dispatch((width == 128 ? DURF_DISPATCH_FWD128_SAMPLE : (half ? DURF_DISPATCH_FWD256_4W : DURF_DISPATCH_FWD256_8W)) |
                  (enc_in ? DURF_DISPATCH_FWD_ENC : 0u) | (tail_idx ? DURF_DISPATCH_FWD_TAIL : 0u) |
                  ((enc_in && (enc_in->flags & DURF_FWD_RAW_FULL) && ray_idx) ? DURF_DISPATCH_FWD_RAW_FULL : 0u));
    return 0;
}

}
```

### durf_amd/csrc/mlp_spec.h

```cpp
#pragma once
#include <type_traits>
#include "durf_common.h"

template <int W_>
struct MlpSpec {
    static constexpr int W = W_;
    static constexpr int WT = W / 32;
    static constexpr int KW = W / 16;
    static constexpr int KE = DURF_ENC_DIM / 16;
    static constexpr int KV = DURF_VIEW_DIM / 16;
    static constexpr int WC = 128;
    static constexpr int KC = WC / 16;
    static constexpr int CT = WC / 32;
    static constexpr int NSTAGE = 11;
    __host__ __device__ static constexpr int n_mt(int s) { return s <= 7 ? WT : (s == 8 ? WT + 1 : (s == 9 ? CT : 1)); }
    __host__ __device__ static constexpr int n_ks(int s) {
        return s == 0 ? KE : (s == 5 ? KW + KE : (s == 9 ? KW + KV : (s == 10 ? KC : KW)));
    }
    __host__ __device__ static constexpr int n_ks_perm(int s) { return s == 0 ? 0 : (s == 10 ? KC : KW); }
    __host__ __device__ static constexpr int tile_chunks(int s) { return n_ks(s) + 1; }
    __host__ __device__ static constexpr int stage_chunk_base(int s) {
        int c = 0;
        for (int i = 0; i < s; i++) c += n_mt(i) * tile_chunks(i);
        return c;
// ... 25 lines not shown
        durf_layer_shape(W, in_dim, l, &fi, &fo);
        off += (size_t)fi * fo + fo;
    }
    if (want_bias) {
        int fi, fo;
        durf_layer_shape(W, in_dim, layer, &fi, &fo);
        off += (size_t)fi * fo;
    }
    return off;
}

template <int W>
__host__ __device__ inline void durf_fwd_out_col(int s, int mo, int i, int* layer, int* col) {
    using S = MlpSpec<W>;
    int L = -1, c = 0;
    if (s <= 7) { L = s; c = 32 * mo + i; }
    else if (s == 8) { if (mo < S::WT) { L = 9; c = 32 * mo + i; } else if (i < 1) { L = 8; c = i; } }
    else if (s == 9) { L = 10; c = 32 * mo + i; }
    else { if (i < 3) { L = 11; c = i; } }
    *layer = L; *col = c;
}
template <int W>
__host__ __device__ inline int durf_fwd_in_row(int s, int ks, int hi, int e, int in_dim) {
    using S = MlpSpec<W>;
    const int np = S::n_ks_perm(s);
    if (ks < np) return 16 * ks + (e & 3) + 8 * (e >> 2) + 4 * hi;
    const int f = 16 * (ks - np) + 8 * hi + e;
    if (s == 0) return f < in_dim ? f : -1;
    if (s == 5) return f < in_dim ? W + f : -1;
    if (s == 9) return f < 27 ? W + f : -1;
    return -1;
}

#ifndef FWD_LDS_RING
#define FWD_LDS_RING 2
#endif
#ifndef BWD_LDS_RING
#define BWD_LDS_RING 4
#endif
typedef int v4i_ __attribute__((ext_vector_type(4)));
template <int I, int N, class F>
__device__ __forceinline__ void static_for(F&& f) {
    if constexpr (I < N) {
        f(std::integral_constant<int, I>{});
        static_for<I + 1, N>(f);
    }
}
template <int OFF>
__device__ __forceinline__ v4i_ lds_read16(unsigned addr) {
    v4i_ r;
    asm volatile("ds_read_b128 %0, %1 offset:%2" : "=v"(r) : "v"(addr), "n"(OFF));
    return r;
}
template <int N>
__device__ __forceinline__ void lds_wait(v4i_& frag) {
    asm volatile("s_waitcnt lgkmcnt(%1)" : "+v"(frag) : "n"(N));
}
__device__ __forceinline__ unsigned lds_addr_of(const char* p) {
    return (unsigned)(size_t)(const __attribute__((address_space(3))) char*)p;
}
template <int NA, int NB, int RING, class H>
__device__ __forceinline__ void mma_pair_ring(const char* slot0, const char* slot1, int lane, const bf16x8* inA,
                                              const bf16x8* inB, f32x16& acc0, f32x16& acc1, H&& hook) {
    constexpr int T = NA + NB, NR = 2 * T;
    constexpr int D = RING < NR ? RING : NR;
    const unsigned l0 = lds_addr_of(slot0) + lane * 16, l1 = lds_addr_of(slot1) + lane * 16;
    v4i_ ring[D];
    static_for<0, D>([&](auto i_) {
        constexpr int i = decltype(i_)::value;
        ring[i] = lds_read16<(i >> 1) * 1024>((i & 1) ? l1 : l0);
    });
    static_for<0, NR>([&](auto i_) {
        constexpr int i = decltype(i_)::value, ks = i >> 1;
        constexpr int later = (NR - 1 - i) < (D - 1) ? (NR - 1 - i) : (D - 1);
        lds_wait<later>(ring[i % D]);
        const bf16x8 a = __builtin_bit_cast(bf16x8, ring[i % D]);
        const bf16x8 b = ks < NA ? inA[ks < NA ? ks : 0] : inB[ks < NA ? 0 : ks - NA];
        if constexpr (i & 1) acc1 = __builtin_amdgcn_mfma_f32_32x32x16_bf16(a, b, acc1, 0, 0, 0);
        else acc0 = __builtin_amdgcn_mfma_f32_32x32x16_bf16(a, b, acc0, 0, 0, 0);
        if constexpr (i + D < NR) ring[i % D] = lds_read16<((i + D) >> 1) * 1024>(((i + D) & 1) ? l1 : l0);
        if constexpr (i & 1) hook(std::integral_constant<int, ks>{});
    });
}

struct WPipe {
    i32x4 rsrc;
    unsigned gnext;
    unsigned lds0;
    char* lds;
    int slot_bytes;
    int par;
    int wave, lane;
    int nw;
    int since;
    __device__ __forceinline__ void skip(int chunks) { gnext += chunks * 1024u; }
    __device__ __forceinline__ void issue(int slot, int chunks) {
        const unsigned dst = lds0 + (unsigned)(slot * slot_bytes);
        for (int c = wave; c < chunks; c += nw)
            lds_dma16_cached(rsrc, gnext + c * 1024u, lane * 16u, dst + c * 1024u);
        gnext += chunks * 1024u;
        since = 0;
    }
    __device__ __forceinline__ const char* begin(int next_chunks) {
        wait_vmcnt_le(since);
        __builtin_amdgcn_s_barrier();
        issue(par ^ 1, next_chunks);
        const char* cur = lds + par * slot_bytes;
        par ^= 1;
        return cur;
    }
};

__host__ __device__ constexpr int group_tiles(int nmt, int ch, int slot) {
    int g = nmt < slot / ch ? nmt : slot / ch;
    return (g > 1) ? (g & ~1) : g;
}

template <class KERNEL, class ARGS, int ITEM_LDS, bool LEVELS, class PairsOf, class Item>
__device__ __forceinline__ void mix_object_items(char* smem, int wave, int nwg, PairsOf&& pairs_of, Item&& item) {
    static_assert(std::is_same<typename kernarg_last<KERNEL>::type, ARGS>::value, "the object arguments are the kernel's LAST parameter");
    typedef const __attribute__((address_space(4))) char* kptr_t;
    kptr_t ka = (kptr_t)__builtin_amdgcn_kernarg_segment_ptr();
    asm volatile("" : "+s"(ka));
    const __attribute__((address_space(4))) ARGS* const kp = (const __attribute__((address_space(4))) ARGS*)(ka + kernarg_last<KERNEL>::offset);
    const unsigned smem_lds = lds_addr_of(smem);
    ARGS ow;
    load_kernarg(ow, (kptr_t)kp);
    const int lane = (int)__builtin_amdgcn_mbcnt_hi(~0u, __builtin_amdgcn_mbcnt_lo(~0u, 0u));
    const bool first = wave == MIX_TICKET_WAVE && lane == 0;
    const int half = wave >> 2, w4 = (wave + MIX_ROLE_ROT * half) & 3;
    char* const lds = smem + half * ITEM_LDS;
    volatile __attribute__((address_space(3))) int* const tk =
        (volatile __attribute__((address_space(3))) int*)(size_t)(__builtin_amdgcn_readfirstlane(smem_lds) + 2u * ITEM_LDS);
    volatile __attribute__((address_space(3))) int* const npl = tk + 4;
    if (wave == 0 && lane < ow.nobj) npl[lane] = (int)pairs_of(ow, lane);
    ms_barrier();
    size_t total = 0;
    for (int k = 0; k < ow.nobj; k++) total += (size_t)npl[k];
    total = (size_t)__builtin_amdgcn_readfirstlane((unsigned)total);
    size_t items = total;
    if constexpr (LEVELS) items = total * (size_t)ow.lv.n;
    const int last = 2 * (int)((items + 1) / 2 + nwg - 1);
    int t = 0;
    DURF_G(int)* const ticket = (DURF_G(int)*)ow.ticket;
    if (first) { t = __hip_atomic_fetch_add(ticket, 2, __ATOMIC_RELAXED, __HIP_MEMORY_SCOPE_AGENT); *tk = t; }
    ms_barrier();
    t = __builtin_amdgcn_readfirstlane(*tk);
    while ((size_t)t < items) {
        int tn = 0;
        if (first) tn = __hip_atomic_fetch_add(ticket, 2, __ATOMIC_RELAXED, __HIP_MEMORY_SCOPE_AGENT);
        const size_t it = (size_t)t + (size_t)half;
        const bool live = it < items;
        int level = 0;
        if constexpr (LEVELS) level = __builtin_amdgcn_readfirstlane(live ? (int)(it / total) : 0);
        size_t k = 0, pair = live ? it - (size_t)level * total : 0;
        for (; live && k + 1 < (size_t)ow.nobj; k++) {
            const size_t np = (size_t)npl[k];
            if (pair < np) break;
            pair -= np;
        }
        k = (size_t)__builtin_amdgcn_readfirstlane((unsigned)(live ? k : 0));
        item(ow, kp, level, lds, lane, w4, live, k, pair);
        if (first) *tk = tn;
        ms_barrier();
        t = __builtin_amdgcn_readfirstlane(*tk);
    }
// ... 28 lines not shown
```

### durf_amd/csrc/policy.h

```cpp
#pragma once
#include <cstdlib>
#include <cstring>
#include "../../include/durf_hip.h"

namespace durf {

struct StepPolicy {
    bool side_fwd, side_bwd, side_dw;
    bool msplit;
    bool mix_enabled;
    bool side() const { return side_fwd || side_bwd || side_dw; }
    unsigned bits() const {
        return (side_fwd ? DURF_POLICY_SIDE_FWD : 0u) | (side_bwd ? DURF_POLICY_SIDE_BWD : 0u) | (side_dw ? DURF_POLICY_SIDE_DW : 0u) |
               (msplit ? DURF_POLICY_MSPLIT : 0u) | (mix_enabled ? DURF_POLICY_MIX : 0u);
    }
};

inline StepPolicy step_policy(size_t rows) {
    const bool large = rows >= DURF_OVERLAP_MIN_ROWS;
    const char* e = getenv("DURF_OVERLAP_OBJECTS");
    if (e == nullptr || !strcmp(e, "auto")) e = large ? "2" : "0";
    const char* ms = getenv("DURF_OBJ_MSPLIT");
    const char* mx = getenv("DURF_OBJ_MIX");
    StepPolicy p;
    p.side_dw = !strcmp(e, "2");
    p.side_bwd = p.side_dw || !strcmp(e, "3");
    p.side_fwd = p.side_bwd || !strcmp(e, "1");
    p.msplit = !large && !(ms && ms[0] == '0');
    p.mix_enabled = p.msplit && !(mx && mx[0] == '0');
    return p;
}

}
```

### durf_amd/csrc/train.hip

```cpp
#include "durf_common.h"
#include "../../include/durf_hip.h"
#include "side_stream.h"
#include "workspace.h"

namespace {

constexpr int ML = DURF_FORWARD_MAX_LEVELS;
constexpr int OBJ32_NSPLIT = 8;

__global__ void k_tv_rows(int K, const float* __restrict__ pose, const float* __restrict__ prev, float c, float* __restrict__ g) {
    const int i = threadIdx.x, k = i / 3, q = i % 3;
    if (k >= K) return;
    const float t = pose[k * 6 + q] - prev[k * 6 + q];
    const float t2 = c * t;
    g[k * 6 + q] = g[k * 6 + q] + t2;
}

struct TrainWs : durf::RayHeadWs {
    float *norms, *prep, *ray_sums, *sums, *part, *bpart, *opart, *obpart, *scratch, *u_rand, *weight_l2;
    float* draw[ML];
    float *raw_c[ML], *raw_b[ML], *obj_raw[ML], *terms[ML];
    void *wf_bkgd, *wb_bkgd, *wf_obj, *wb_obj, *view_tile, *obj_view_tile;
    void *enc[ML], *stash[ML], *mask[ML], *dz[ML], *dz_out[ML];
    void *obj_enc[ML], *obj_stash[ML], *obj_mask[ML], *obj_dz[ML], *obj_dz_out[ML];
// ... 80 lines not shown
    DURF_REQUIRE(f.K >= 0 && f.K <= DURF_MAX_OBJ, "0 <= K <= DURF_MAX_OBJ");
    DURF_REQUIRE(f.num_levels >= 2 && f.num_levels <= DURF_FORWARD_MAX_LEVELS, "2 <= num_levels <= DURF_FORWARD_MAX_LEVELS");
    DURF_REQUIRE(((size_t)workspace & 255) == 0, "workspace aligned to 256 bytes");
    DURF_REQUIRE(a->box_floats + a->mlp0_floats + (size_t)f.K * a->obj_floats == a->n_params,
                 "flat layout: box_centers | MLP_0 | K object MLPs");
    DURF_REQUIRE(f.bkgd_params == a->params + a->box_floats &&
                 (f.K == 0 || (f.obj_params == a->params + a->box_floats + a->mlp0_floats && f.obj_param_stride == a->obj_floats)),
                 "f.bkgd_params / f.obj_params point into params");
    DURF_REQUIRE(f.bkgd_mode >= 0 && f.bkgd_mode <= 2, "bkgd_mode: 0 grey / 1 white / 2 none (rand_bkgd: bg = 0)");
    for (int l = 0; l < f.num_levels && f.density_noise != 0.0f; l++)
        DURF_REQUIRE(f.density_rand[l] != nullptr || f.draw_noise, "density_noise: density_rand[level] or draw_noise");
    DURF_REQUIRE(!f.draw_noise || (f.t_rand == nullptr && f.u_rand == nullptr), "draw_noise: the library makes the draws");
    DURF_REQUIRE((a->flags & ~(DURF_TRAIN_OBJ_FP32 | DURF_TRAIN_POSE_OPT | DURF_TRAIN_OBJ_X3)) == 0, "unknown flags");
    DURF_REQUIRE(!(a->flags & DURF_TRAIN_OBJ_X3) || (a->flags & DURF_TRAIN_OBJ_FP32), "DURF_TRAIN_OBJ_X3 is a variant of the fp32 object branch");
    if (a->flags & DURF_TRAIN_POSE_OPT) {
        DURF_REQUIRE(f.K > 0 && (a->flags & DURF_TRAIN_OBJ_FP32), "box-pose optimisation runs behind the fp32 object branch");
        DURF_REQUIRE(a->want_pos || a->want_rot, "pose optimisation without a pose gradient to compute");
        DURF_REQUIRE(f.pose >= a->params && f.pose + (size_t)f.K * 6 <= a->params + a->box_floats,
                     "f.pose must be this timestep's rows of box_centers inside params (their gradient goes to the same rows of grad)");
        DURF_REQUIRE(a->prev6 != nullptr || a->tv_loss_mult == 0.0f, "the TV prior needs prev6");
    }
    DURF_REQUIRE(a->params && a->grad && a->stats, "params, grad and stats buffers");
    DURF_REQUIRE(((size_t)a->grad & 15) == 0, "grad aligned to 16 bytes");
    for (int l = 0; l < f.num_levels; l++)
        DURF_REQUIRE(f.t_vals[l] && f.weights[l] && f.rgb[l] && f.depth[l] && f.acc[l] && f.t_mids[l] && f.t_dists[l],
                     "per-level output buffers (t_vals, rgb, depth, acc, weights, t_mids, t_dists)");
    return 0;
}

#define STEP(call) do { rc = (call); if (rc != 0) return rc; } while (0)
#define TIMED(id, call) do {                                                                       \
        if (tm && tm->begin[id]) (void)hipEventRecord((hipEvent_t)tm->begin[id], hs);               \
        STEP(call);                                                                                \
        if (tm && tm->end[id]) (void)hipEventRecord((hipEvent_t)tm->end[id], hs);                   \
    } while (0)

__global__ void k_scale(int n, float* __restrict__ x, float c) {
    const int i = blockIdx.x * blockDim.x + threadIdx.x;
    if (i < n) x[i] *= c;
}

struct TailIn {
    const float *tv[ML], *terms[ML];
    const float *wl2, *pose, *prev6, *target6;
    TailIn(const durf_train_args* a, const TrainWs& w) {
        const bool K = a->f.K != 0;
        for (int l = 0; l < a->f.num_levels; l++) { tv[l] = a->f.t_vals[l]; terms[l] = w.terms[l]; }
        wl2 = a->weight_decay_mult != 0.0f ? w.weight_l2 : nullptr;
        pose = K ? a->f.pose : nullptr; prev6 = K ? a->prev6 : nullptr; target6 = K ? a->target6 : nullptr;
    }
};

int loss_backward(void* stream, const durf_train_args* a, const TrainWs& w, const TailIn* tail) {
    const durf_forward_args& f = a->f;
    const int B = f.B, N = f.N, K = f.K, L = f.num_levels;
    const size_t rows = (size_t)B * N;
    hipStream_t hs = (hipStream_t)stream;
    const durf_step_timing* tm = a->timing;
    int rc;
    const bool f32o = K > 0 && (a->flags & DURF_TRAIN_OBJ_FP32), pose_opt = f32o && (a->flags & DURF_TRAIN_POSE_OPT);
    const bool x3 = f32o && (a->flags & DURF_TRAIN_OBJ_X3);
    const int Kb = f32o ? 0 : K;
    STEP(durf_ray_prologue_pack(stream, B, K, N, f.origins, f.directions, f.pose, f.ext, w.o_s, w.d_s, w.hit, f.zo, f.viewdirs, w.view,
                                f.near, f.far, f.t_rand, f.lindisp, f.t_vals[0], K > 0 ? a->pose_used : nullptr, a->grad, a->n_params, f.seed_lo, f.seed_hi,
                                f.draw_noise ? w.u_rand : nullptr, f.bkgd_params, 60, w.wf_bkgd, w.wb_bkgd, Kb, f.obj_params,
                                f.obj_param_stride, 63, w.wf_obj, w.wb_obj,
                                K == 0 ? (float*)f.dyn_mask : (pose_opt ? w.pose_sums : nullptr),
                                K == 0 ? (size_t)B : (pose_opt ? (size_t)K * 21 : (size_t)0)));
    if (K > 0)
        STEP(durf_compact_all(stream, B, K, N, w.hit, w.idx_obj, w.count_obj, w.slot_obj, w.idx_cls, w.count_cls, w.slot_cls,
                              f.dyn_mask));
    if (f32o) {
        STEP(durf_view_enc(stream, B, f.viewdirs, nullptr, w.view27));
        if (x3) STEP(durf_mlp_f32_pack_x3(stream, K, f.obj_params, f.obj_param_stride, w.obj_ws));
        else STEP(durf_mlp_f32_pack(stream, 128, 63, K, f.obj_params, f.obj_param_stride, w.obj_ws));
    }
    const float* raw_obj[ML][DURF_MAX_OBJ];
    for (int l = 0; l < L; l++)
        for (int k = 0; k < K; k++) raw_obj[l][k] = w.obj_raw[l] + (size_t)k * rows * 4;
    const int obj_flags = f.enc_flags & (DURF_ENC_NO_INTEGRATION | DURF_ENC_CYLINDER);
    const durf::StepPolicy policy = durf::step_policy(rows);
    const durf::Overlap ov = durf::overlap_for(stream, policy, Kb);
    const bool mix = Kb > 0 && !ov.sd && policy.mix_enabled && N % 32 == 0;
    for (int lvl = 0; lvl < L; lvl++) {
        float* t_vals = f.t_vals[lvl];
        if (ov.sd) {
            STEP(ov.fork());
            STEP(durf_obj_fwd_batch(ov.obj(), K, B, N, w.idx_obj, w.count_obj, t_vals, w.o_s, w.d_s, f.radii, f.barf_w, obj_flags,
                                    w.view, w.wf_obj, w.obj_enc[lvl], w.obj_raw[lvl], w.obj_stash[lvl], w.obj_mask[lvl],
                                    lvl == 0 ? w.obj_view_tile : nullptr));
        }
        if (K > 0) {
            if (mix)
                TIMED(DURF_TIMED_FWD + lvl,
                      durf_mlp_fwd_enc_obj(stream, rows, N, t_vals, w.o_s, w.d_s, f.radii, w.hit, K, f.enc_flags | DURF_FWD_RAW_FULL,
                                           w.enc[lvl], w.view, w.idx_cls, w.count_cls, w.wf_bkgd, w.raw_b[lvl], w.stash[lvl], w.mask[lvl],
                                           w.idx_cls + B, w.count_cls + 1, lvl == 0 ? w.view_tile : nullptr, B, w.idx_obj, w.count_obj,
                                           f.barf_w, obj_flags, w.wf_obj, w.obj_enc[lvl], w.obj_raw[lvl], w.obj_stash[lvl], w.obj_mask[lvl],
                                           lvl == 0 ? w.obj_view_tile : nullptr));
            else
            TIMED(DURF_TIMED_FWD + lvl,
                  durf_mlp_fwd_enc(stream, rows, N, t_vals, w.o_s, w.d_s, f.radii, w.hit, K, f.enc_flags | (f32o ? 0 : DURF_FWD_RAW_FULL),
                                   w.enc[lvl], w.view, w.idx_cls, w.count_cls, w.wf_bkgd, f32o ? w.raw_c[lvl] : w.raw_b[lvl], w.stash[lvl],
                                   w.mask[lvl], w.idx_cls + B, w.count_cls + 1, lvl == 0 ? w.view_tile : nullptr));
            if (f32o && lvl == 0) {
                float* trunk = a->const_trunk ? a->const_trunk : w.trunk;
                STEP(durf::join_prefetch(stream));
                if (!(a->const_trunk && a->const_trunk_valid))
                    STEP(durf_bkgd_const_trunk_f32(stream, f.bkgd_params, trunk));
                STEP(durf_bkgd_hit_rays_f32(stream, B, w.view27, f.bkgd_params, w.idx_cls + B, w.count_cls + 1, trunk, w.raw_tail));
            }
            if (f32o) STEP(durf_expand_raw(stream, B, N, w.raw_c[lvl], w.count_cls, w.slot_cls, w.raw_b[lvl], w.raw_tail));
            if (f32o)
                STEP(durf_objf32_fwd_batch(stream, K, B, N, w.idx_obj, w.count_obj, nullptr, w.view27, f.obj_params,
                                           f.obj_param_stride, w.obj_ws, w.obj_raw[lvl], w.act32[lvl], t_vals, w.o_s, w.d_s,
                                           f.radii, f.barf_w, obj_flags | (x3 ? DURF_F32_X3 : 0)));
            else if (!ov.sd && !mix)
                STEP(durf_obj_fwd_batch(stream, K, B, N, w.idx_obj, w.count_obj, t_vals, w.o_s, w.d_s, f.radii, f.barf_w, obj_flags,
                                        w.view, w.wf_obj, w.obj_enc[lvl], w.obj_raw[lvl], w.obj_stash[lvl], w.obj_mask[lvl],
                                        lvl == 0 ? w.obj_view_tile : nullptr));
            STEP(ov.join());
        } else {
            TIMED(DURF_TIMED_FWD + lvl,
                  durf_mlp_fwd_enc(stream, rows, N, t_vals, w.o_s, w.d_s, f.radii, nullptr, 0, f.enc_flags, w.enc[lvl], w.view, nullptr,
                                   nullptr, w.wf_bkgd, w.raw_b[lvl], w.stash[lvl], w.mask[lvl], nullptr, nullptr,
                                   lvl == 0 ? w.view_tile : nullptr));
        }
        if (f.density_noise != 0.0f)
            STEP(durf_density_noise(stream, rows, w.raw_b[lvl], f.density_noise, f.density_rand[lvl], f.seed_lo, f.seed_hi, lvl));
        if (lvl + 1 < L)
            TIMED(DURF_TIMED_COMPOSITE + lvl,
                 durf_composite_resample(stream, B, N, K, w.raw_b[lvl], raw_obj[lvl], w.slot_obj, t_vals, w.d_s, f.density_bias,
                                         f.bkgd_mode, f.rgb[lvl], f.depth[lvl], f.acc[lvl], f.weights[lvl], f.t_mids[lvl],
                                         f.t_dists[lvl], f.resample_padding, f.draw_noise ? w.u_rand + (size_t)lvl * B * (N + 1) : f.u_rand, f.t_vals[lvl + 1], a->lossmult, a->gt_depth,
                                         a->sky, f.dyn_mask, f.zo, a->eps, a->box_loss_mult, lvl, a->disable_multiscale,
                                         lvl == 0 ? w.prep : nullptr, lvl == 0 ? w.norms : nullptr, w.prep + (size_t)5 * B,
                                         w.norms + (size_t)(lvl + 1) * 5));
    }
    {
        durf_loss_level ll[ML] = {};
        for (int lvl = 0; lvl < L; lvl++) {
            const bool last = lvl == L - 1;
            durf_loss_level& h = ll[lvl];
            h.raw_bkgd = w.raw_b[lvl]; h.t_vals = f.t_vals[lvl]; h.norm = w.norms + (size_t)lvl * 5; h.level = lvl;
            for (int k = 0; k < K; k++) h.raw_obj[k] = raw_obj[lvl][k];
            for (int i = 0; i < 6; i++) h.mults[i] = a->level_mults[lvl][i];
            h.draw = w.draw[lvl]; h.terms = w.terms[lvl];
            if (last) { h.rgb_out = f.rgb[lvl]; h.depth_out = f.depth[lvl]; h.acc_out = f.acc[lvl]; h.weights_out = f.weights[lvl];
                        h.t_mids_out = f.t_mids[lvl]; h.t_dists_out = f.t_dists[lvl]; }
            h.draw_ray_sum = K > 0 ? w.ray_sums + (size_t)lvl * B * 4 : nullptr;
        }
        STEP(durf_loss_bwd_levels(stream, B, N, K, L, ll, w.slot_obj, w.d_s, a->pixels, a->lossmult, a->gt_depth, a->sky, f.dyn_mask,
                                  f.zo, a->eps, a->box_loss_mult, a->disable_multiscale, a->bg, f.density_bias));
    }
    STEP(ov.fork());
    if (Kb > 0 && !mix) {
        const float* dr[ML]; const void* mk[ML]; void* dzl[ML]; void* dzo[ML];
        for (int l = 0; l < L; l++) { dr[l] = w.draw[L - 1 - l]; mk[l] = w.obj_mask[L - 1 - l]; dzl[l] = w.obj_dz[L - 1 - l]; dzo[l] = w.obj_dz_out[L - 1 - l]; }
        STEP(durf_obj_bwd_batch_levels(ov.obj(), K, B, N, L, w.idx_obj, w.count_obj, dr, w.wb_obj, mk, dzl, dzo));
    }
    if (f32o) {
        const float *de[ML], *tv[ML];
        for (int lvl = L - 1; lvl >= 0; lvl--) {
            STEP((x3 ? durf_objf32_bwd_batch_x3 : durf_objf32_bwd_batch)(stream, K, B, N, w.idx_obj, w.count_obj, w.draw[lvl], f.obj_params,
                                                                         f.obj_param_stride, w.obj_ws, w.act32[lvl], w.dz32[lvl],
                                                                         pose_opt ? w.d_enc32[lvl] : nullptr));
            de[L - 1 - lvl] = w.d_enc32[lvl]; tv[L - 1 - lvl] = f.t_vals[lvl];
        }
        if (pose_opt)
            STEP(durf_encode_obj_bwd_levels(stream, K, B, N, L, w.idx_obj, w.count_obj, de, tv, w.o_s, w.d_s, f.radii, f.origins,
                                            f.directions, f.pose, f.barf_w, w.pose_scratch, w.pose_sums, 1, obj_flags));
    }
    for (int lvl = L - 1; lvl >= 0; lvl--) {
        float* rs = K > 0 ? w.ray_sums + (size_t)lvl * B * 4 : nullptr;
        if (mix) {
            const float* dr1[1] = {w.draw[lvl]}; const void* mk1[1] = {w.obj_mask[lvl]};
            void* dz1[1] = {w.obj_dz[lvl]}; void* dzo1[1] = {w.obj_dz_out[lvl]};
            TIMED(DURF_TIMED_BWD + lvl,
                  durf_mlp_bwd_obj(stream, rows, N, w.draw[lvl], w.idx_cls, w.count_cls, w.wb_bkgd, w.mask[lvl], w.dz[lvl], w.dz_out[lvl],
                                   w.idx_cls + B, w.count_cls + 1, rs, K, B, 1, w.idx_obj, w.count_obj, dr1, w.wb_obj, mk1, dz1, dzo1));
        } else if (K > 0) {
            TIMED(DURF_TIMED_BWD + lvl,
                  durf_mlp_bwd(stream, 256, rows, N, w.draw[lvl], w.idx_cls, w.count_cls, w.wb_bkgd, w.mask[lvl], w.dz[lvl], w.dz_out[lvl],
                               nullptr, w.idx_cls + B, w.count_cls + 1, rs));
        } else {
            TIMED(DURF_TIMED_BWD + lvl,
                  durf_mlp_bwd(stream, 256, rows, N, w.draw[lvl], nullptr, nullptr, w.wb_bkgd, w.mask[lvl], w.dz[lvl], w.dz_out[lvl], nullptr,
                               nullptr, nullptr, nullptr));
        }
    }
    const void *enc[ML], *vt[ML], *stash[ML], *dz[ML], *dzo[ML], *ovt[ML];
    size_t seg_rows[ML];
    int per_ray[ML];
    const int32_t* seg_count[ML];
    for (int l = 0; l < L; l++) {
        vt[l] = w.view_tile; ovt[l] = w.obj_view_tile;
        seg_rows[l] = rows;
        per_ray[l] = K > 0 ? 1 : N;
        seg_count[l] = K > 0 ? w.count_cls + 2 : nullptr;
    }
    float* g_bkgd = a->grad + a->box_floats;
    float* g_obj = g_bkgd + a->mlp0_floats;
    if (f32o) {
        const float *act[ML], *dz32[ML];
        for (int l = 0; l < L; l++) { act[l] = w.act32[l]; dz32[l] = w.dz32[l]; }
        STEP(durf_objf32_dw_batch(stream, K, B, N, w.count_obj, L, act, dz32, OBJ32_NSPLIT, w.dw32_scratch, g_obj, a->obj_floats));
    } else if (K > 0) {
// ... 114 lines not shown
```

### durf_amd/obbpose_model.py

```python
import dataclasses
import math
from typing import Any

import torch

from . import camera, ops
from . import utils

IN_BKGD, IN_OBJ, W_BKGD, W_OBJ = 60, 63, ops.W_BKGD, ops.W_OBJ


def _layer_shapes(width, in_dim, use_viewdirs=True):
    trunk = [(in_dim, width)] + [(width, width)] * 4 + [(width + in_dim, width)] + [(width, width)] * 2
    if not use_viewdirs:
        return trunk + [(width, 1), (width, 3)]
    return trunk + [(width, 1), (width, width), (width + 27, 128), (128, 3)]


class ParamLayout:

    def __init__(self, T, K, use_viewdirs=True):
        self.T, self.K, self.use_viewdirs = T, K, bool(use_viewdirs)
        self.box = (0, T * K * 6)
        off = T * K * 6
# ... 155 lines not shown
    def _scene_edit(self, variables, ts, pose, box_enable, train=False):
        K = variables.layout.K
        dev = variables.flat.device
        if train and (pose is not None or box_enable is not None):
            raise NotImplementedError('box_enable / pose edit the scene of an inference render: training has no such knob')
        if pose is None:
            pose = variables['params']['box_centers'][int(ts)].contiguous()
        else:
            pose = torch.as_tensor(pose)
            if tuple(pose.shape) != (K, 6):
                raise ValueError('pose: shape %s, expected (%d, 6)' % (tuple(pose.shape), K))
            pose = pose.detach().to(device=dev, dtype=torch.float32).contiguous()
        en = ops._enable(box_enable, K, dev)
        return pose, (en if K > 0 else None)

    def _forward(self, variables, rng, rays, init, ext, ts, randomized, rand_bkgd, white_bkgd, alpha,
                 train=False, noise=None, loss_prep=None, zero_fill=None, box_enable=None, pose=None):
        self._check()
        variables = self._kernel_variables(variables)
        lay = variables.layout
        K, N = lay.K, self.num_samples
        Kd = K if self.dynamics else 0
        B = rays.origins.shape[0]
        dev = rays.origins.device
        ts = int(ts)
        pose, box_enable = self._scene_edit(variables, ts, pose, box_enable, train)
        ext = ext.reshape(-1, 3).contiguous() if K > 0 else torch.zeros(0, 3, device=dev)
        radii = rays.radii.reshape(-1).contiguous()
        near, far = rays.near.reshape(-1).contiguous(), rays.far.reshape(-1).contiguous()
        f32 = self.mlp_precision == 'f32'
        obj_f32 = bool(Kd) and not f32 and self.object_precision() == 'f32'
        Kb = 0 if obj_f32 else Kd
        g = _make_generator(rng, dev) if randomized else None
        seed = None
        if randomized and noise is None:
            if isinstance(rng, torch.Generator):
                u = torch.rand(2, B, N + 1, device=dev, generator=g)
                noise = dict(t_rand=u[0], u_rand=u[1])
            else:
                seed = int(rng) if rng is not None else 0
        use_dd = bool(Kd) and not f32 and (ops.DEDUP_HIT_RAYS or obj_f32)
        tail_side = trunk = None
        if obj_f32:
            tail_side = ops.side_stream(dev)
            cached = getattr(variables, '_trunk_cache', None)
            variables._trunk_cache = None
            if cached is not None and cached[1] == (variables.flat._version, ops.param_generation(variables.flat)):
                trunk = cached[0]
            else:
                tail_side.wait_stream(torch.cuda.current_stream())
                with torch.cuda.stream(tail_side):
                    trunk = ops.bkgd_const_trunk_f32(variables.mlp_flat('MLP_0'))
        pose_used = torch.empty_like(pose)
        pack_arg = None
        if not f32:
            o0 = lay.mlp_off['BoxMLP_0'] if Kb else 0
            pack_arg = (variables.mlp_flat('MLP_0'), Kb, variables.flat[o0:o0 + Kb * lay.mlp_size[W_OBJ]] if Kb else None,
                        lay.mlp_size[W_OBJ], train)
        pro = ops.ray_prologue(rays.origins, rays.directions, pose, ext, rays.viewdirs, near, far, N,
                               noise['t_rand'] if (randomized and seed is None) else None, self.lindisp,
                               pose_copy=pose_used, zero=zero_fill, seed=seed, pack=pack_arg, box_enable=box_enable)
        o_s, d_s, hit, zo, view, t_vals0 = pro[:6]
        if seed is not None:
            noise = dict(t_rand=None, u_rand=pro[6])
        if use_dd:
            (idx, count, slot), cls = ops.compact_all(hit, N)
        else:
            (idx, count, slot), cls = ops.compact_hits(hit), None
        static_f32 = self.static_hit_f32(K)
        view27 = ops.view_enc(rays.viewdirs, want_f32=True)[1] if (f32 or obj_f32 or static_f32) else None
        packs = {}
        if not f32:
            pk_b, pk_o = pro[-1]
            packs = {'MLP_0': pk_b}
            if Kb:
                packs['obj'] = pk_o
        bk = ops.BKGD_RAND if rand_bkgd else (ops.BKGD_WHITE if white_bkgd else ops.BKGD_GREY)
        rows = B * N
        cyl = self.ray_shape == 'cylinder'
        view_tiles_obj = ops.obj_view_tiles(Kb, B, N, dev) if (train and Kb and not f32) else None
        ctx = dict(o_s=o_s, d_s=d_s, hit=hit, zo=zo, idx=idx, count=count, slot=slot, view=view,
                   packs=packs, levels=[], B=B, N=N, K=Kd, ts=ts, policy=ops.step_policy(rows), bkgd_mode=bk, view_tiles_obj=view_tiles_obj,
                   obj_f32=obj_f32 or (f32 and bool(Kd)), obj_x3=obj_f32 and self.object_x3())
        obj_flat = None
        if ctx['obj_f32']:
            o0 = lay.mlp_off['BoxMLP_0']
            obj_flat = variables.flat[o0:o0 + Kd * lay.mlp_size[W_OBJ]]
            ctx['obj_ws'] = ops.mlp_f32_pack(W_OBJ, IN_OBJ, obj_flat, K=Kd, param_stride=lay.mlp_size[W_OBJ], x3=ctx['obj_x3'])
        if f32 or static_f32:
            ctx['bkgd_ws'] = ops.mlp_f32_pack(W_BKGD, IN_BKGD, variables.mlp_flat('MLP_0'))
        if static_f32:
            hi, hc, hs = ops.compact_hits(hit.amax(dim=1, keepdim=True))
            ctx['hit_rows'] = dict(idx=hi, count=hc, slot=hs.reshape(-1), mask=(hs.reshape(B, 1, 1) >= 0))
        raw_tail = None
        ret = []
        t_vals = weights = None
        box_rot0 = pose_used[0, 3:] if K > 0 else ops.const_tensor(dev, (3,))
        if cls is not None:
            dyn_mask = cls[3].reshape(B, 1)
        elif K > 1:
            dyn_mask = hit.sum(dim=-1, keepdim=True, dtype=torch.int32)
        else:
            dyn_mask = hit if K == 1 else ops.const_tensor(dev, (B, 1), torch.int32)
        if loss_prep is not None:
            if self.num_levels < 2:
                loss_prep = None
            else:
                loss_prep = dict(loss_prep, dyn=dyn_mask.reshape(-1).to(torch.int32).contiguous(), zo=zo)
        fused = train and loss_prep is not None
        dd = None
        if cls is not None:
            dd = dict(idx=cls[0], count=cls[1], slot=cls[2], nrows=cls[1][2:3], multi_hit=cls[1][3])
            ctx['dedup'] = dd
        t_next = None
        for lvl in range(self.num_levels):
            last = lvl == self.num_levels - 1
            if lvl == 0:
                t_vals = t_vals0
            elif t_next is not None:
                t_vals = t_next
            else:
                t_vals = ops.resample(t_vals, weights, self.resample_padding,
                                      _u_plane(noise, lvl - 1) if randomized else None)
            if f32:
                lvd = self._level_f32(variables, obj_flat, ctx, train, t_vals, o_s, d_s, radii, hit, Kd, cyl, view27, idx, count,
                                      alpha, B, N)
                raw_b, slabs = lvd['raw_b'], None
                enc_b = stash_b = mask_b = None
                raws = lvd['raws']
            else:
                lvd = None
                stash_b = torch.empty(ops.mlp_stash_bytes(W_BKGD, rows), dtype=torch.uint8, device=dev) if train else None
                mask_b = torch.empty(ops.mlp_mask_bytes(rows), dtype=torch.uint8, device=dev) if train else None
                side = ops.on_side(dev, bool(Kb) and ctx['policy'].side_fwd)
                enc_kw = dict(contraction=self.contraction, disable_integration=self.disable_integration, cylinder=cyl)
                slabs = None
                obj_first = bool(Kb) and side.enabled

                def launch_objects():
                    with side:
                        ops.obj_fwd_batch(slabs, idx, count, t_vals, o_s, d_s, radii, alpha, view, packs['obj'][0],
                                          view_tile=view_tiles_obj if lvl == 0 else None,
                                          disable_integration=self.disable_integration, cylinder=cyl)
                if Kb:
                    slabs = ops.ObjSlabs(Kd, B, N, dev, train)
                if obj_first:
                    side.fork()
                    launch_objects()
                vt = None
                if train and lvl == 0 and ops.FUSED_ENCODE:
                    vt = ctx['view_tile'] = torch.empty(ops.tile_rows(rows), ops.VIEW_DIM, dtype=torch.bfloat16, device=dev)
                mixed = (train and bool(Kb) and dd is not None and ops.FUSED_ENCODE and ops.FWD_SCATTER_RAW and
                         not side.enabled and ctx['policy'].mix)
                if mixed:
                    scatter = True
                    raw_c, enc_b = ops.mlp_fwd_enc_obj(rows, N, t_vals, o_s, d_s, radii, hit, view, packs['MLP_0'][0], slabs, idx,
                                                       count, alpha, packs['obj'][0], dd['idx'][0], dd['count'][0:1], dd['idx'][1],
                                                       dd['count'][1:2], stash_b, mask_b, view_tile=vt,
                                                       obj_view_tile=view_tiles_obj if lvl == 0 else None, **enc_kw)
                    obj_first = True
                elif dd is not None and ops.FUSED_ENCODE:
                    side.fork()
                    scatter = not obj_f32 and ops.FWD_SCATTER_RAW
                    raw_c, enc_b = ops.mlp_fwd_enc(rows, N, t_vals, o_s, d_s, radii, hit, view, packs['MLP_0'][0],
                                                   ray_idx=dd['idx'][0], count=dd['count'][0:1], stash=stash_b,
                                                   relu_mask=mask_b, tail_idx=dd['idx'][1], tail_count=dd['count'][1:2],
                                                   view_tile=vt, raw_full=scatter, **enc_kw)
                elif dd is not None:
                    scatter = False
                    enc_b, _ = ops.encode_bkgd(t_vals, o_s, d_s, radii, hit, self.contraction,
                                               disable_integration=self.disable_integration, cylinder=cyl,
                                               idx=dd['idx'][0], count=dd['count'][0:1])
                    side.fork()
                    raw_c = ops.mlp_fwd(W_BKGD, rows, N, enc_b, view, packs['MLP_0'][0], ray_idx=dd['idx'][0],
                                        count=dd['count'][0:1], stash=stash_b, relu_mask=mask_b,
                                        tail_idx=dd['idx'][1], tail_count=dd['count'][1:2])
                if dd is not None:
                    if tail_side is not None:
                        torch.cuda.current_stream().wait_stream(tail_side)
                        tail_side = None
                    if obj_f32 and lvl == 0:
                        if trunk is not None:
                            trunk.record_stream(torch.cuda.current_stream())
                        raw_tail = ops.bkgd_hit_rays_f32(B, view27, variables.mlp_flat('MLP_0'), dd['idx'][1],
                                                         dd['count'][1:2], trunk=trunk)
                    raw_b = raw_c if scatter else ops.expand_raw(B, N, raw_c, dd['slot'], dd['count'], raw_tail=raw_tail)
                elif ops.FUSED_ENCODE:
                    side.fork()
                    raw_b, enc_b = ops.mlp_fwd_enc(rows, N, t_vals, o_s, d_s, radii, hit if Kd else None, view,
                                                   packs['MLP_0'][0], stash=stash_b, relu_mask=mask_b, view_tile=vt, **enc_kw)
                else:
                    enc_b, _ = ops.encode_bkgd(t_vals, o_s, d_s, radii, hit if Kd else None, self.contraction,
                                               disable_integration=self.disable_integration, cylinder=cyl)
                    side.fork()
                    raw_b = ops.mlp_fwd(W_BKGD, rows, N, enc_b, view, packs['MLP_0'][0], stash=stash_b, relu_mask=mask_b)
                if obj_f32:
                    lvd = self._objects_f32(obj_flat, lay.mlp_size[W_OBJ], ctx['obj_ws'], train, t_vals, o_s, d_s, radii, Kd, cyl,
                                            view27, idx, count, alpha, B, N)
                if Kb:
                    if not obj_first:
                        launch_objects()
                    side.join()
                raws = slabs.raws() if Kb else (lvd['raws'] if obj_f32 else [])
            if static_f32:
                hr = ctx['hit_rows']
                _, enc32 = ops.encode_bkgd(t_vals, o_s, d_s, radii, None, self.contraction, tile=False, f32=True,
                                           disable_integration=self.disable_integration, cylinder=cyl, idx=hr['idx'], count=hr['count'])
                out32 = ops.mlp_fwd_f32(W_BKGD, IN_BKGD, rows, N, enc32, view27, variables.mlp_flat('MLP_0'),
                                        ray_idx=hr['idx'], count=hr['count'], want_act=train, wstream=ctx['bkgd_ws'])
                raw32, act32 = out32 if train else (out32, None)
                raw_b = torch.where(hr['mask'], raw32.view(B, N, 4)[hr['slot'].clamp(min=0)], raw_b.view(B, N, 4)).reshape(rows, 4)
                lvd = dict(act_hit=act32)
            if randomized and self.density_noise > 0:
                if 'density' in noise:
                    ops.density_noise(raw_b, self.density_noise, normal=noise['density'][lvl])
                elif seed is not None:
                    ops.density_noise(raw_b, self.density_noise, seed=seed, level=lvl)
                else:
# ... 225 lines not shown
```

### durf_amd/ops.py

```python
import collections
import ctypes as C
import math
import os

import torch

from . import _lib, camera
from . import _sigs as _H, _field_sigs, _flow_sigs, _geom_sigs, _lidar_sigs, _mesh_sigs, _overlay_sigs, _parts_sigs, _raster_sigs, _tsdf_sigs, _cast_sigs, _closest_sigs



def _by_prefix(table, prefix):
    return {k[len(prefix):]: v for k, v in vars(table).items() if k.startswith(prefix) and type(v) is int}


for _table in (_H, _overlay_sigs, _lidar_sigs, _flow_sigs, _field_sigs, _mesh_sigs, _geom_sigs, _parts_sigs, _raster_sigs, _tsdf_sigs, _cast_sigs, _closest_sigs):
    globals().update(_by_prefix(_table, 'DURF_'))
del OVERLAP_MIN_ROWS


def _stream():
    return torch.cuda.current_stream().cuda_stream


# ... 254 lines not shown
    k = np.arange(max_deg, dtype=np.float32)
    a = np.clip(np.float32(alpha) - k, 0, 1).astype(np.float32) * np.float32(math.pi)
    return ((np.float32(1) - np.cos(a, dtype=np.float32)) / np.float32(2)).astype(np.float32)


def encode_obj(max_rays, idx_k, count_k, t_vals, origins_s, dirs_s, radii, alpha, tile=True, f32=False,
               disable_integration=False, cylinder=False):
    N = t_vals.shape[1] - 1
    dev = t_vals.device
    ot = torch.empty(tile_rows(max_rays * N), ENC_DIM, dtype=torch.bfloat16, device=dev) if tile else None
    of = torch.zeros(max_rays * N, 63, device=dev) if f32 else None
    w = barf_weights(alpha)
    wa = (C.c_float * 10)(*[float(x) for x in w])
    _lib.check(_lib.lib().durf_encode_obj(_stream(), max_rays, N, _p(idx_k), _p(count_k),
                                          _p(_f32(t_vals)), _p(_f32(origins_s)), _p(_f32(dirs_s)),
                                          _p(_f32(radii)), wa,
                                          (ENC_NO_INTEGRATION if disable_integration else 0) | (ENC_CYLINDER if cylinder else 0),
                                          _p(ot), _p(of)), 'durf_encode_obj')
    return ot, of


def mlp_param_count(width, in_dim):
    return int(_lib.lib().durf_mlp_param_count(width, in_dim))


def mlp_layer_offset(width, in_dim, layer, bias):
    return int(_lib.lib().durf_mlp_layer_offset(width, in_dim, layer, int(bias)))


def pack_weights(width, in_dim, mlp_params, want_bwd=False):
    dev = mlp_params.device
    wf = torch.empty(int(_lib.lib().durf_wpack_fwd_bytes(width)), dtype=torch.uint8, device=dev)
    wb = None
    if want_bwd:
        wb = torch.empty(int(_lib.lib().durf_wpack_bwd_bytes(width)), dtype=torch.uint8, device=dev)
    _lib.check(_lib.lib().durf_pack_weights(_stream(), width, in_dim, _p(_f32(mlp_params)), _p(wf),
                                            _p(wb)), 'durf_pack_weights')
    return (wf, wb) if want_bwd else wf


def pack_weights_all(bkgd_params, K, obj_params, obj_param_stride, want_bwd=False):
    L = _lib.lib()
    dev = bkgd_params.device
    u8 = lambda n: torch.empty(int(n), dtype=torch.uint8, device=dev)
    bf = u8(L.durf_wpack_fwd_bytes(W_BKGD_))
    bb = u8(L.durf_wpack_bwd_bytes(W_BKGD_)) if want_bwd else None
    of = ob = None
    if K:
        of = u8(K * int(L.durf_wpack_fwd_bytes(W_OBJ_)))
        ob = u8(K * int(L.durf_wpack_bwd_bytes(W_OBJ_))) if want_bwd else None
    _lib.check(L.durf_pack_weights_all(_stream(), _p(_f32(bkgd_params)), IN_BKGD, _p(bf), _p(bb), int(K),
                                       _p(obj_params) if K else None, int(obj_param_stride), IN_OBJ_, _p(of), _p(ob)),
               'durf_pack_weights_all')
    return (bf, bb), ((of, ob) if K else None)


def mlp_stash_bytes(width, rows):
    return int(_lib.lib().durf_mlp_stash_bytes(width, rows))


def mlp_mask_bytes(rows):
    return int(_lib.lib().durf_mlp_mask_bytes(rows))


def mlp_fwd(width, rows, N, enc_tile, view_bf16, wpack_fwd, ray_idx=None, count=None, stash=None,
            raw=None, relu_mask=None, tail_idx=None, tail_count=None):
    dev = enc_tile.device
    if raw is None:
        raw = torch.empty(rows, 4, device=dev)
    with _Timed('mlp_fwd_%d%s' % (width, '_train' if stash is not None else '')):
        _lib.check(_lib.lib().durf_mlp_fwd(_stream(), width, rows, N, _p(enc_tile), _p(view_bf16),
                                           _p(ray_idx), _p(count), _p(wpack_fwd), _p(raw), _p(stash),
                                           _p(relu_mask), _p(tail_idx), _p(tail_count)),
                   'durf_mlp_fwd')
    return raw


FUSED_ENCODE = os.environ.get('DURF_FUSED_ENCODE', '1') != '0'
FWD_SCATTER_RAW = True


def mlp_fwd_enc(rows, N, t_vals, origins_s, dirs_s, radii, hit, view_bf16, wpack_fwd, contraction=True,
                disable_integration=False, cylinder=False, ray_idx=None, count=None, stash=None, raw=None, relu_mask=None,
                tail_idx=None, tail_count=None, view_tile=None, raw_full=False):
    dev = t_vals.device
    K = 0 if hit is None else hit.shape[1]
    if raw is None:
        raw = torch.empty(rows, 4, device=dev)
    enc_tile = torch.empty(tile_rows(rows), ENC_DIM, dtype=torch.bfloat16, device=dev)
    flags = ((ENC_CONTRACT if contraction else 0) | (ENC_NO_INTEGRATION if disable_integration else 0) |
             (ENC_CYLINDER if cylinder else 0) | (FWD_RAW_FULL if raw_full else 0))
    with _Timed('mlp_fwd_256%s' % ('_train' if stash is not None else '')):
        _lib.check(_lib.lib().durf_mlp_fwd_enc(_stream(), rows, N, _p(_f32(t_vals)), _p(_f32(origins_s)), _p(_f32(dirs_s)),
                                               _p(_f32(radii)), _p(hit), K, flags, _p(enc_tile), _p(view_bf16),
                                               _p(ray_idx), _p(count), _p(wpack_fwd), _p(raw), _p(stash), _p(relu_mask),
                                               _p(tail_idx), _p(tail_count), _p(view_tile)), 'durf_mlp_fwd_enc')
    return raw, enc_tile


class StepPolicy(collections.namedtuple('StepPolicy', 'side_fwd side_bwd side_dw msplit mix_enabled')):
    @property
    def mix(self):
        return self.mix_enabled and not (self.side_fwd or self.side_bwd or self.side_dw)


def step_policy(rows):
    m = int(_lib.lib().durf_step_policy(rows))
    return StepPolicy(*(bool(m & (1 << i)) for i in range(5)))


def __getattr__(name):
    if name == 'OVERLAP_MIN_ROWS':
        return int(_lib.lib().durf_overlap_min_rows())
    if name == '_MODE':
        small, large = overlap_mode(0), overlap_mode(1 << 62)
        return small if small == large else 'auto'
    raise AttributeError('module %r has no attribute %r' % (__name__, name))


def set_overlap_mode(mode):
    os.environ['DURF_OVERLAP_OBJECTS'] = mode


def overlap_mode(rows):
    p = step_policy(rows)
    return '2' if p.side_dw else '3' if p.side_bwd else '1' if p.side_fwd else '0'


def overlap_forward(rows):
    return step_policy(rows).side_fwd


def overlap_backward(rows):
    return step_policy(rows).side_bwd


def overlap_dw(rows):
    return step_policy(rows).side_dw


_SIDE = {}


def side_stream(device):
    key = (device.type, device.index)
    if key not in _SIDE:
        _SIDE[key] = torch.cuda.Stream(device=device)
    return _SIDE[key]


class on_side:

    def __init__(self, device, enabled=True):
        self.enabled = bool(enabled) and device.type == 'cuda'
        self.side = side_stream(device) if self.enabled else None
        self.ctx = None

    def fork(self):
        if self.enabled:
            self.side.wait_stream(torch.cuda.current_stream())

    def join(self):
        if self.enabled:
            torch.cuda.current_stream().wait_stream(self.side)

    def __enter__(self):
        if self.enabled:
            self.ctx = torch.cuda.stream(self.side)
            self.ctx.__enter__()
        return self

    def __exit__(self, *a):
        if self.enabled:
            self.ctx.__exit__(*a)
# ... 302 lines not shown
    with _Timed('mlp_dw_%d' % width):
        _lib.check(_lib.lib().durf_mlp_dw(_stream(), width, rows, N, _p(count), L, arr(enc_tiles), arr(view_tiles),
                                          arr(stashes), arr(dzs), arr(dz_outs), _p(part), _p(bpart)), 'durf_mlp_dw')


def _levels_args(rows_l, n_l, count_l):
    L = len(rows_l)
    return (L, (C.c_size_t * L)(*[int(r) for r in rows_l]), (C.c_int * L)(*[int(n) for n in n_l]),
            (C.c_void_p * L)(*[None if c is None else c.data_ptr() for c in count_l]))


def mlp_dw_levels(width, rows_l, n_l, count_l, enc_tiles, view_tiles, stashes, dzs, dz_outs, part, bpart):
    L, rows_a, n_a, cnt_a = _levels_args(rows_l, n_l, count_l)
    arr = lambda ts: (C.c_void_p * L)(*[t.data_ptr() for t in ts])
    with _Timed('mlp_dw_%d' % width):
        _lib.check(_lib.lib().durf_mlp_dw_levels(_stream(), width, L, rows_a, n_a, cnt_a, arr(enc_tiles), arr(view_tiles),
                                                 arr(stashes), arr(dzs), arr(dz_outs), _p(part), _p(bpart)),
                   'durf_mlp_dw_levels')


def mlp_dw_finalize_levels(width, in_dim, rows_l, n_l, count_l, part, bpart, grad_mlp, mlp_params):
    L, rows_a, n_a, cnt_a = _levels_args(rows_l, n_l, count_l)
    with _Timed('mlp_dw_finalize_%d' % width):
        _lib.check(_lib.lib().durf_mlp_dw_finalize_levels(_stream(), width, in_dim, L, rows_a, n_a, cnt_a, _p(part),
                                                          _p(bpart), _p(grad_mlp), _p(_f32(mlp_params))),
                   'durf_mlp_dw_finalize_levels')


def mlp_dw_finalize(width, in_dim, rows, N, nlevels, part, bpart, grad_mlp, mlp_params, count=None):
    with _Timed('mlp_dw_finalize_%d' % width):
        _lib.check(_lib.lib().durf_mlp_dw_finalize(_stream(), width, in_dim, rows, N, _p(count), nlevels, _p(part),
                                                   _p(bpart), _p(grad_mlp), _p(_f32(mlp_params))), 'durf_mlp_dw_finalize')


W_OBJ_, IN_OBJ_ = W_OBJ, 63
W_BKGD_, IN_BKGD = W_BKGD, 60


class ObjSlabs:

    def __init__(self, K, B, N, device, train):
        L = _lib.lib()
        rows = B * N
        u8 = lambda n: torch.empty(K * int(n), dtype=torch.uint8, device=device)
        self.K, self.B, self.N = K, B, N
        self.enc = u8(L.durf_obj_enc_stride(B, N))
        self.raw = torch.empty(K, rows, 4, device=device)
        self.stash = u8(mlp_stash_bytes(W_OBJ_, rows)) if train else None
        self.mask = u8(mlp_mask_bytes(rows)) if train else None
        self.dz = self.dz_out = self.d_enc = None

    def raws(self):
        return [self.raw[k] for k in range(self.K)]


def pack_weights_batch(K, obj_params, param_stride, want_bwd=False):
    L = _lib.lib()
    dev = obj_params.device
    wf = torch.empty(K * int(L.durf_wpack_fwd_bytes(W_OBJ_)), dtype=torch.uint8, device=dev)
    wb = torch.empty(K * int(L.durf_wpack_bwd_bytes(W_OBJ_)), dtype=torch.uint8, device=dev) if want_bwd else None
    _lib.check(L.durf_pack_weights_batch(_stream(), W_OBJ_, IN_OBJ_, K, _p(obj_params), param_stride, _p(wf), _p(wb)),
               'durf_pack_weights_batch')
    return wf, wb


def obj_fwd_batch(slabs, idx, count, t_vals, origins_s, dirs_s, radii, alpha, view_bf16, wf, view_tile=None,
                  disable_integration=False, cylinder=False):
    w = barf_weights(alpha)
    wa = (C.c_float * 10)(*[float(x) for x in w])
    with _Timed('obj_fwd_batch'):
        _lib.check(_lib.lib().durf_obj_fwd_batch(
            _stream(), slabs.K, slabs.B, slabs.N, _p(idx), _p(count), _p(_f32(t_vals)), _p(_f32(origins_s)),
            _p(_f32(dirs_s)), _p(_f32(radii)), wa,
            (ENC_NO_INTEGRATION if disable_integration else 0) | (ENC_CYLINDER if cylinder else 0), _p(view_bf16),
            _p(wf), _p(slabs.enc), _p(slabs.raw), _p(slabs.stash), _p(slabs.mask), _p(view_tile)), 'durf_obj_fwd_batch')


def obj_mix(rows):
    return step_policy(rows).mix


def mlp_fwd_enc_obj(rows, N, t_vals, origins_s, dirs_s, radii, hit, view_bf16, wpack_fwd, slabs, obj_idx, obj_count, alpha, obj_wf,
                    ray_idx, count, tail_idx, tail_count, stash, relu_mask, contraction=True, disable_integration=False,
                    cylinder=False, view_tile=None, raw_full=True, obj_view_tile=None):
    dev = t_vals.device
    K = hit.shape[1]
    raw = torch.empty(rows, 4, device=dev)
    enc_tile = torch.empty(tile_rows(rows), ENC_DIM, dtype=torch.bfloat16, device=dev)
    flags = ((ENC_CONTRACT if contraction else 0) | (ENC_NO_INTEGRATION if disable_integration else 0) |
             (ENC_CYLINDER if cylinder else 0) | (FWD_RAW_FULL if raw_full else 0))
    wa = (C.c_float * 10)(*[float(x) for x in barf_weights(alpha)])
    with _Timed('mlp_fwd_256%s' % ('_train' if stash is not None else '')):
        _lib.check(_lib.lib().durf_mlp_fwd_enc_obj(
            _stream(), rows, N, _p(_f32(t_vals)), _p(_f32(origins_s)), _p(_f32(dirs_s)), _p(_f32(radii)), _p(hit), K, flags,
            _p(enc_tile), _p(view_bf16), _p(ray_idx), _p(count), _p(wpack_fwd), _p(raw), _p(stash), _p(relu_mask), _p(tail_idx),
            _p(tail_count), _p(view_tile), slabs.B, _p(obj_idx), _p(obj_count), wa,
            (ENC_NO_INTEGRATION if disable_integration else 0) | (ENC_CYLINDER if cylinder else 0), _p(obj_wf), _p(slabs.enc),
            _p(slabs.raw), _p(slabs.stash), _p(slabs.mask), _p(obj_view_tile)), 'durf_mlp_fwd_enc_obj')
    return raw, enc_tile


def mlp_bwd_obj(rows, N, draw, wpack_bwd, relu_mask, ray_idx, count, tail_idx, tail_count, draw_ray_sum, slabs_levels, obj_idx,
                obj_count, obj_draws, obj_wb):
    L = _lib.lib()
    dev = draw.device
    dz = torch.empty(mlp_stash_bytes(256, rows), dtype=torch.uint8, device=dev)
    dz_out = torch.empty(tile_rows(rows), 16, dtype=torch.bfloat16, device=dev)
    s0 = slabs_levels[0]
    K, B, nl = s0.K, s0.B, len(slabs_levels)
    for sl in slabs_levels:
        sl.dz = torch.empty(K * mlp_stash_bytes(W_OBJ_, B * N), dtype=torch.uint8, device=dev)
        sl.dz_out = torch.empty(K * int(L.durf_obj_dzout_stride(B, N)), dtype=torch.uint8, device=dev)
        sl.d_enc = None
    arr = lambda ts: (C.c_void_p * nl)(*[t.data_ptr() for t in ts])
    with _Timed('mlp_bwd_256'):
        _lib.check(L.durf_mlp_bwd_obj(_stream(), rows, N, _p(_f32(draw)), _p(ray_idx), _p(count), _p(wpack_bwd), _p(relu_mask),
                                      _p(dz), _p(dz_out), _p(tail_idx), _p(tail_count), _p(draw_ray_sum), K, B, nl, _p(obj_idx),
                                      _p(obj_count), arr([_f32(d) for d in obj_draws]), _p(obj_wb),
                                      arr([s.mask for s in slabs_levels]), arr([s.dz for s in slabs_levels]),
                                      arr([s.dz_out for s in slabs_levels])), 'durf_mlp_bwd_obj')
    return dz, dz_out


def obj_view_tiles(K, B, N, device):
    return torch.empty(K * int(_lib.lib().durf_obj_view_stride(B, N)), dtype=torch.uint8, device=device)


def obj_bwd_batch(slabs, idx, count, draw, wb, want_d_enc=False):
    L = _lib.lib()
    dev = draw.device
    K, B, N = slabs.K, slabs.B, slabs.N
    slabs.dz = torch.empty(K * mlp_stash_bytes(W_OBJ_, B * N), dtype=torch.uint8, device=dev)
    slabs.dz_out = torch.empty(K * int(L.durf_obj_dzout_stride(B, N)), dtype=torch.uint8, device=dev)
    slabs.d_enc = torch.empty(K, B * N, ENC_DIM, device=dev) if want_d_enc else None
    with _Timed('obj_bwd_batch'):
        _lib.check(L.durf_obj_bwd_batch(_stream(), K, B, N, _p(idx), _p(count), _p(_f32(draw)), _p(wb), _p(slabs.mask),
                                        _p(slabs.dz), _p(slabs.dz_out), _p(slabs.d_enc)), 'durf_obj_bwd_batch')


def obj_bwd_batch_levels(slabs_levels, idx, count, draws, wb):
    L = _lib.lib()
    s0 = slabs_levels[0]
    K, B, N = s0.K, s0.B, s0.N
    nl = len(slabs_levels)
    dev = draws[0].device
    for sl in slabs_levels:
        sl.dz = torch.empty(K * mlp_stash_bytes(W_OBJ_, B * N), dtype=torch.uint8, device=dev)
        sl.dz_out = torch.empty(K * int(L.durf_obj_dzout_stride(B, N)), dtype=torch.uint8, device=dev)
        sl.d_enc = None
    arr = lambda ts: (C.c_void_p * nl)(*[t.data_ptr() for t in ts])
    with _Timed('obj_bwd_batch'):
        _lib.check(L.durf_obj_bwd_batch_levels(_stream(), K, B, N, nl, _p(idx), _p(count), arr([_f32(d) for d in draws]), _p(wb),
                                               arr([s.mask for s in slabs_levels]), arr([s.dz for s in slabs_levels]),
                                               arr([s.dz_out for s in slabs_levels])), 'durf_obj_bwd_batch_levels')


def obj_dw_batch(slabs_levels, view_tile, count, grad_obj, grad_stride, obj_params):
    L = _lib.lib()
    s0 = slabs_levels[0]
    K, B, N = s0.K, s0.B, s0.N
    nl = len(slabs_levels)
    dev = grad_obj.device
    part = torch.empty(K * int(L.durf_dw_part_floats(W_OBJ_)), device=dev)
    bpart = torch.empty(K * int(L.durf_dw_bpart_floats(W_OBJ_)), device=dev)
    arr = lambda ts: (C.c_void_p * nl)(*[t.data_ptr() for t in ts])
    with _Timed('obj_dw_batch'):
        _lib.check(L.durf_obj_dw_batch(_stream(), K, B, N, _p(count), nl, arr([s.enc for s in slabs_levels]),
                                       arr([view_tile] * nl), arr([s.stash for s in slabs_levels]),
                                       arr([s.dz for s in slabs_levels]), arr([s.dz_out for s in slabs_levels]),
                                       IN_OBJ_, _p(part), _p(bpart), _p(grad_obj), grad_stride, _p(_f32(obj_params))),
                   'durf_obj_dw_batch')


# ... 1448 lines not shown
```

### include/durf_ctypes_stub.py

```python
import ctypes as C

vp, i32, f32, u64 = C.c_void_p, C.c_int, C.c_float, C.c_size_t


DURF_MAX_OBJ = 16
DURF_MAX_LEVELS = 8
DURF_MAX_CAMS = 8
DURF_W_BKGD = 256
DURF_W_OBJ = 128
DURF_ENC_CONTRACT = 1
DURF_ENC_NO_INTEGRATION = 2
DURF_ENC_CYLINDER = 4
DURF_FWD_RAW_FULL = 8
DURF_ENC_DIM = 64
DURF_VIEW_DIM = 32
DURF_DISPATCH_FWD256_8W = 0x1
DURF_DISPATCH_FWD256_4W = 0x2
DURF_DISPATCH_FWD128_SAMPLE = 0x4
DURF_DISPATCH_FWD128_MSPLIT = 0x8
DURF_DISPATCH_BWD256_8W = 0x10
DURF_DISPATCH_BWD256_4W = 0x20
DURF_DISPATCH_BWD128_SAMPLE = 0x40
DURF_DISPATCH_BWD128_MSPLIT = 0x80
DURF_DISPATCH_DW256_256WG = 0x100
DURF_DISPATCH_DW256_512WG = 0x200
DURF_DISPATCH_DW128_128WG = 0x400
DURF_DISPATCH_DW128_256WG = 0x800
DURF_DISPATCH_FWD_ENC = 0x1000
DURF_DISPATCH_FWD_RAW_FULL = 0x2000
DURF_DISPATCH_FWD_TAIL = 0x4000
DURF_DISPATCH_F32_DW_TILE = 0x8000
DURF_DISPATCH_F32_DW_B2 = 0x10000
DURF_DISPATCH_BWD_POSE = 0x20000
DURF_DISPATCH_FWD_MIX = 0x40000
DURF_DISPATCH_BWD_MIX = 0x80000
DURF_LAYERLOG_SELECT = 0x100000
DURF_LAYERLOG_PASS2 = 0x200000
DURF_LAYERLOG_BOX_MASK = 0x400000
DURF_LAYERLOG_TRAJ_RAYS = 0x800000
DURF_LAYERLOG_TRAJ_POSE = 0x1000000
DURF_LAYERLOG_TRAJ_PACK = 0x2000000
DURF_OVERLAP_MIN_ROWS = 262144
DURF_POLICY_SIDE_FWD = 0x1
DURF_POLICY_SIDE_BWD = 0x2
DURF_POLICY_SIDE_DW = 0x4
DURF_POLICY_MSPLIT = 0x8
DURF_POLICY_MIX = 0x10


class durf_loss_level(C.Structure):
    _fields_ = [
        ('raw_bkgd', vp),
        ('raw_obj', vp * DURF_MAX_OBJ),
        ('t_vals', vp),
        ('norm', vp),
        ('mults', f32 * 6),
        ('level', i32),
        ('draw', vp),
        ('terms', vp),
        ('rgb_out', vp),
        ('depth_out', vp),
        ('acc_out', vp),
        ('weights_out', vp),
        ('t_mids_out', vp),
        ('t_dists_out', vp),
        ('draw_ray_sum', vp),
    ]


DURF_FORWARD_MAX_LEVELS = 4


class durf_forward_args(C.Structure):
    _fields_ = [
        ('B', i32),
        ('N', i32),
        ('K', i32),
        ('num_levels', i32),
        ('enc_flags', i32),
        ('lindisp', i32),
        ('bkgd_mode', i32),
        ('density_bias', f32),
        ('resample_padding', f32),
        ('barf_w', f32 * 10),
        ('origins', vp),
        ('directions', vp),
        ('viewdirs', vp),
        ('radii', vp),
        ('near', vp),
        ('far', vp),
        ('pose', vp),
        ('ext', vp),
        ('bkgd_params', vp),
        ('obj_params', vp),
        ('obj_param_stride', u64),
        ('t_rand', vp),
# ... 347 lines not shown
```

### include/durf_hip.h

```cpp
#ifndef DURF_HIP_H
#define DURF_HIP_H
#include <stddef.h>
#include <stdint.h>

#ifdef __cplusplus
extern "C" {
#endif

#define DURF_MAX_OBJ 16
#define DURF_MAX_LEVELS 8
#define DURF_MAX_CAMS 8
#define DURF_W_BKGD 256
#define DURF_W_OBJ 128
#define DURF_ENC_CONTRACT 1
#define DURF_ENC_NO_INTEGRATION 2
#define DURF_ENC_CYLINDER 4
#define DURF_FWD_RAW_FULL 8
#define DURF_ENC_DIM 64
#define DURF_VIEW_DIM 32

const char* durf_last_error(void);
int durf_version(void);
#define DURF_DISPATCH_FWD256_8W 0x1
#define DURF_DISPATCH_FWD256_4W 0x2
#define DURF_DISPATCH_FWD128_SAMPLE 0x4
#define DURF_DISPATCH_FWD128_MSPLIT 0x8
#define DURF_DISPATCH_BWD256_8W 0x10
#define DURF_DISPATCH_BWD256_4W 0x20
#define DURF_DISPATCH_BWD128_SAMPLE 0x40
#define DURF_DISPATCH_BWD128_MSPLIT 0x80
#define DURF_DISPATCH_DW256_256WG 0x100
#define DURF_DISPATCH_DW256_512WG 0x200
#define DURF_DISPATCH_DW128_128WG 0x400
#define DURF_DISPATCH_DW128_256WG 0x800
#define DURF_DISPATCH_FWD_ENC 0x1000
#define DURF_DISPATCH_FWD_RAW_FULL 0x2000
#define DURF_DISPATCH_FWD_TAIL 0x4000
#define DURF_DISPATCH_F32_DW_TILE 0x8000
#define DURF_DISPATCH_F32_DW_B2 0x10000
#define DURF_DISPATCH_BWD_POSE 0x20000
#define DURF_DISPATCH_FWD_MIX 0x40000
#define DURF_DISPATCH_BWD_MIX 0x80000
#define DURF_LAYERLOG_SELECT 0x100000
#define DURF_LAYERLOG_PASS2 0x200000
#define DURF_LAYERLOG_BOX_MASK 0x400000
#define DURF_LAYERLOG_TRAJ_RAYS 0x800000
#define DURF_LAYERLOG_TRAJ_POSE 0x1000000
#define DURF_LAYERLOG_TRAJ_PACK 0x2000000
int durf_dispatch_seen(void);
int durf_dispatch_reset(void);
#define DURF_OVERLAP_MIN_ROWS ((size_t)2048 * 128)
#define DURF_POLICY_SIDE_FWD 0x1
#define DURF_POLICY_SIDE_BWD 0x2
#define DURF_POLICY_SIDE_DW 0x4
#define DURF_POLICY_MSPLIT 0x8
#define DURF_POLICY_MIX 0x10
unsigned durf_step_policy(size_t rows);
size_t durf_overlap_min_rows(void);

size_t durf_mlp_param_count(int width, int in_dim);
size_t durf_mlp_layer_offset(int width, int in_dim, int layer, int want_bias);
size_t durf_wpack_fwd_bytes(int width);
size_t durf_wpack_bwd_bytes(int width);
int durf_pack_weights(void* stream, int width, int in_dim, const float* mlp_params,
                      void* wpack_fwd, void* wpack_bwd );
int durf_pack_weights_all(void* stream, const float* bkgd_params, int in_bkgd, void* bkgd_fwd, void* bkgd_bwd,
                          int K, const float* obj_params, size_t obj_param_stride, int in_obj, void* obj_fwd,
                          void* obj_bwd);


int durf_ray_setup(void* stream, int B, int K, const float* origins, const float* dirs,
                   const float* pose, const float* ext, float* origins_s, float* dirs_s,
                   int32_t* hit, float* zo);

int durf_ray_setup_masked(void* stream, int B, int K, const float* origins, const float* dirs,
                          const float* pose, const float* ext, const int32_t* box_enable , float* origins_s,
                          float* dirs_s, int32_t* hit, float* zo);

int durf_compact_hits(void* stream, int B, int K, const int32_t* hit, int32_t* idx,
                      int32_t* count, int32_t* slot);
int durf_compact_classes(void* stream, int B, int K, int N, const int32_t* hit, int32_t* idx, int32_t* count,
                         int32_t* slot, int32_t* dyn);
int durf_compact_all(void* stream, int B, int K, int N, const int32_t* hit, int32_t* idx_obj, int32_t* count_obj,
                     int32_t* slot_obj, int32_t* idx_cls, int32_t* count_cls, int32_t* slot_cls, int32_t* dyn);
int durf_ray_prologue(void* stream, int B, int K, int N, const float* origins, const float* dirs, const float* pose,
                      const float* ext, float* origins_s, float* dirs_s, int32_t* hit, float* zo,
                      const float* viewdirs, void* view_bf16, const float* near, const float* far,
                      const float* t_rand , int lindisp, float* t_vals, float* pose_copy ,
                      float* zero_buf , size_t zero_count, uint32_t seed_lo, uint32_t seed_hi,
                      float* u_rand_out );
int durf_ray_prologue_pack(void* stream, int B, int K, int N, const float* origins, const float* dirs, const float* pose,
                           const float* ext, float* origins_s, float* dirs_s, int32_t* hit, float* zo,
                           const float* viewdirs, void* view_bf16, const float* near, const float* far,
                           const float* t_rand , int lindisp, float* t_vals, float* pose_copy ,
                           float* zero_buf , size_t zero_count, uint32_t seed_lo, uint32_t seed_hi,
                           float* u_rand_out , const float* bkgd_params, int in_bkgd, void* bkgd_fwd,
                           void* bkgd_bwd , int K_pack, const float* obj_params, size_t obj_param_stride,
                           int in_obj, void* obj_fwd, void* obj_bwd ,
                           float* zero_buf2 , size_t zero_count2);
int durf_ray_prologue_pack_masked(void* stream, int B, int K, int N, const float* origins, const float* dirs, const float* pose,
// ... 396 lines not shown
```

Before: 989,800.

## Recompute Dense_0 activations in weight-gradient kernel instead of stashing them

Adds a DURF_FWD_NO_H0 flag so the W=256 training forward skips writing the first layer's bf16 activations to the stash. The dW kernel's job 1 recomputes them per tile from the encoding tile and Dense_0 weights with MFMA, writing them into LDS. This trades a global write plus read of the h0 activations for extra MFMA work, a higher LDS stage footprint, an extra barrier per tile, and a host-side map from stash pointer to weight pack. It is on by default via the step policy, with an environment variable to disable it.

New measurement: 995,000, median of 6. About the same (+0.5%).

```diff
diff --git a/durf_amd/_sigs.py b/durf_amd/_sigs.py
--- a/durf_amd/_sigs.py
+++ b/durf_amd/_sigs.py
@@ -133,6 +133,7 @@
 DURF_ENC_NO_INTEGRATION = 2
 DURF_ENC_CYLINDER = 4
 DURF_FWD_RAW_FULL = 8
+DURF_FWD_NO_H0 = 16
 DURF_ENC_DIM = 64
 DURF_VIEW_DIM = 32
 DURF_DISPATCH_FWD256_8W = 0x1
diff --git a/durf_amd/csrc/api.hip b/durf_amd/csrc/api.hip
--- a/durf_amd/csrc/api.hip
+++ b/durf_amd/csrc/api.hip
@@ -1,6 +1,7 @@
 #include <stdarg.h>
 #include <atomic>
 #include <mutex>
+#include <unordered_map>
 #include "durf_common.h"
 
 static thread_local char g_err[512] = "";
@@ -40,6 +41,19 @@
     return base + (next[dev].fetch_add(1u, std::memory_order_relaxed) % RING);
 }
 
+static std::mutex g_h0_lock;
+static std::unordered_map<const void*, const void*> g_h0_src;
+void durf::note_h0_stash(const void* stash, const void* wpack_fwd) {
+    std::lock_guard<std::mutex> hold(g_h0_lock);
+    if (wpack_fwd) g_h0_src[stash] = wpack_fwd;
+    else g_h0_src.erase(stash);
+}
+const void* durf::h0_stash_source(const void* stash) {
+    std::lock_guard<std::mutex> hold(g_h0_lock);
+    const auto it = g_h0_src.find(stash);
+    return it == g_h0_src.end() ? nullptr : it->second;
+}
+
 extern "C" {
 int durf_dispatch_seen(void) { return (int)g_dispatch.load(std::memory_order_relaxed); }
 int durf_dispatch_reset(void) { g_dispatch.store(0u, std::memory_order_relaxed); return 0; }
diff --git a/durf_amd/csrc/durf_common.h b/durf_amd/csrc/durf_common.h
--- a/durf_amd/csrc/durf_common.h
+++ b/durf_amd/csrc/durf_common.h
@@ -224,6 +224,8 @@
                   const void* const* enc_tile, const void* const* view_tile, const void* const* stash,
                   const void* const* dz, const void* const* dz_out, float* part, float* bpart, int K,
                   const DwStrides& st);
+void note_h0_stash(const void* stash, const void* wpack_fwd);
+const void* h0_stash_source(const void* stash);
 int launch_dw_finalize(void* stream, int width, int in_dim, const DwLevels& lv,
                        const float* part, const float* bpart, float* grad_mlp, int K, size_t part_stride,
                        size_t bpart_stride, size_t grad_stride, const float* mlp_params, size_t param_stride);
diff --git a/durf_amd/csrc/mlp_bwd.hip b/durf_amd/csrc/mlp_bwd.hip
--- a/durf_amd/csrc/mlp_bwd.hip
+++ b/durf_amd/csrc/mlp_bwd.hip
@@ -575,6 +575,7 @@
     int nsplit[12];
     int first_wg[13];
     int order[12];
+    const char* w0;
 };
 
 #ifndef DW_MIN_TPS
@@ -596,17 +597,19 @@
     return (nrows + 31) >> 5;
 }
 
-template <int NKO, int NKA, int NKB, int NKO2 = 0>
+template <int NKO, int NKA, int NKB, int NKO2 = 0, int NKR = 0>
 __device__ __forceinline__ void dw_job(const durf::DwLevels& lv, const DwArgs& a, int job,
                                        int nsplit, int split_idx, float* __restrict__ part,
                                        float* __restrict__ bpart, char* smem) {
     constexpr int NKI = NKA + NKB;
     constexpr int NC = NKO + NKI;
-    constexpr int CPW = (NC + 7) / 8;
+    static_assert(NKR == 0 || (NKB == 0 && NKO2 == 0 && NKA == 16), "the recomputed segment: job 1 of the W = 256 MLP (one output tile per wave)");
+    constexpr int NCD = NKR ? NKO + NKR : NC;
+    constexpr int CPW = (NCD + 7) / 8;
     constexpr int MO = (NKO + 1) / 2, NI = NKI / 2;
     constexpr int RM = (MO + 3) / 4, RN = (NI + 1) / 2;
-    constexpr int STAGE = NC * 1024;
-    constexpr int S = dw_stages(NC);
+    constexpr int STAGE = (NC + NKR) * 1024;
+    constexpr int S = dw_stages(NC + NKR);
     const int lane = threadIdx.x & 63;
     const int wave = __builtin_amdgcn_readfirstlane(threadIdx.x >> 6);
     const int wm = wave >> 1, wn = wave & 1;
@@ -636,8 +639,11 @@
 #pragma unroll
         for (int i = 0; i < CPW; i++) {
             int ci = wave + 8 * i;
-            if (ci >= NC) ci -= NC;
-            if (ci < NKO1) {
+            if (ci >= NCD) ci -= NCD;
+            if (NKR > 0 && ci >= NKO) {
+                const int ks = ci - NKO;
+                lds_dma16(r_a, (unsigned)((ti * NKR + ks) * 1024), (unsigned)lane * 16u, dst + (NC + ks) * 1024);
+            } else if (ci < NKO1) {
                 lds_dma16(r_dz, (unsigned)((ti * NKO1 + ci) * 1024), voff[ci & 1], dst + ci * 1024);
             } else if (NKO2 > 0 && ci < NKO) {
                 lds_dma16(r_dz2, (unsigned)((ti * NKO2 + ci - NKO1) * 1024), voff[ci & 1], dst + ci * 1024);
@@ -667,6 +673,19 @@
     float bsum[RM];
 #pragma unroll
     for (int rm = 0; rm < RM; rm++) bsum[rm] = 0.0f;
+    Dense0Frags<NKR ? 16 * NKA : 256> d0;
+    int h0_off[2] = {0, 0};
+    if constexpr (NKR > 0) {
+        d0.load(a.w0, wave, lane);
+#pragma unroll
+        for (int k = 0; k < NKR; k++) asm volatile("" : "+v"(d0.A[k]));
+#pragma unroll
+        for (int g4 = 0; g4 < 4; g4++) asm volatile("" : "+v"(d0.b[g4]));
+        const int n = lane & 31, hf = lane >> 5;
+#pragma unroll
+        for (int u = 0; u < 2; u++)
+            h0_off[u] = (NKO + 2 * wave + u) * 1024 + (hf * 32 + ((n & 16) | ((n + 4 * (2 * u + hf)) & 15))) * 16;
+    }
 
     size_t lo = 0, hi_t = 0;
     for (int lvl = 0; lvl < a.nlevels; lvl++) {
@@ -678,7 +697,7 @@
         const int nt = (int)(b1 - b0);
         r_dz = make_rsrc(a.dz[lvl][job] + obj * a.ks_dz[job] + t0 * NKO1 * 1024);
         r_dz2 = make_rsrc(NKO2 ? a.dz2[lvl] + obj * a.ks_dz2 + t0 * (NKO2 ? NKO2 : 1) * 1024 : a.dz[lvl][job]);
-        r_a = make_rsrc(a.inA[lvl][job] + obj * a.ks_a[job] + t0 * NKA * 1024);
+        r_a = make_rsrc(a.inA[lvl][job] + obj * a.ks_a[job] + t0 * (NKR ? NKR : NKA) * 1024);
         r_b = make_rsrc(NKB ? a.inB[lvl][job] + obj * a.ks_b[job] + t0 * (NKB ? NKB : 1) * 1024 : a.inA[lvl][job]);
         __builtin_amdgcn_s_barrier();
 #pragma unroll
@@ -691,6 +710,16 @@
             __builtin_amdgcn_s_barrier();
             if (t + S - 1 < nt) stage_load(t + S - 1, (t + S - 1) % S);
             const char* st = smem + (t % S) * STAGE;
+            if constexpr (NKR > 0) {
+                bf16x8 e[NKR], o0, o1;
+#pragma unroll
+                for (int k = 0; k < NKR; k++) e[k] = *(const bf16x8*)(st + (NC + k) * 1024 + lane * 16);
+                d0.apply(e, o0, o1);
+                *(bf16x8*)(smem + (t % S) * STAGE + h0_off[0]) = o0;
+                *(bf16x8*)(smem + (t % S) * STAGE + h0_off[1]) = o1;
+                asm volatile("s_waitcnt lgkmcnt(0)" ::: "memory");
+                __builtin_amdgcn_s_barrier();
+            }
 #pragma unroll
             for (int kk = 0; kk < 2; kk++) {
                 bf16x8 af[RM], bf[RN];
@@ -770,6 +799,12 @@
 #define DW_CALL(...) dw_job<__VA_ARGS__>(lv, a, job, ns, sp, a.part[job], a.bpart[job], smem)
     switch (job) {
         case 0: DW_CALL(S::KW, S::KE, 0); break;
+        case 1:
+            if constexpr (W == 256) {
+                if (a.w0) { DW_CALL(S::KW, S::KW, 0, 0, S::KE); break; }
+            }
+            DW_CALL(S::KW, S::KW, 0);
+            break;
         case 5: DW_CALL(S::KW, S::KW, S::KE); break;
         case 8: if (W != 256) DW_CALL(1, S::KW, 0); break;
         case 10:
@@ -1286,6 +1321,13 @@
     const int nlevels = lv.nlevels;
     DURF_REQUIRE(width == 256 || width == 128, "width must be 256 or 128");
     DURF_REQUIRE(nlevels >= 1 && nlevels <= DURF_MAX_LEVELS, "1 <= nlevels <= DURF_MAX_LEVELS");
+    const void* wpack_fwd = nullptr;
+    if (width == 256 && K == 1) {
+        wpack_fwd = h0_stash_source(stash[0]);
+        for (int l = 1; l < nlevels; l++)
+            DURF_REQUIRE(h0_stash_source(stash[l]) == wpack_fwd, "the levels' forwards disagree about Dense_0's activations (DURF_FWD_NO_H0)");
+    }
+    DURF_REQUIRE(nlevels >= 1 && nlevels <= DURF_MAX_LEVELS, "1 <= nlevels <= DURF_MAX_LEVELS");
     size_t total_rows = 0;
     for (int l = 0; l < nlevels; l++) {
         DURF_REQUIRE(lv.rows[l] % 32 == 0, "rows must be a multiple of 32");
@@ -1330,7 +1372,10 @@
         a.dz[l][9] = nullptr; a.inA[l][9] = nullptr;
         a.dz[l][10] = region(dz[ll], 9, ll); a.inA[l][10] = region(stash[ll], 7, ll); a.inB[l][10] = (const char*)view_tile[ll];
         a.dz[l][11] = (const char*)dz_out[ll]; a.inA[l][11] = region(stash[ll], 9, ll);
-    }
+        if (wpack_fwd) a.inA[l][1] = (const char*)enc_tile[ll];
+    }
+    a.w0 = (const char*)wpack_fwd;
+    if (wpack_fwd) a.ks_a[1] = st.enc;
     static const int order[12] = {11, 8, 0, 10, 5, 1, 2, 3, 4, 6, 7, 9};
     int total = 0;
     for (int i = 0; i < 12; i++) {
diff --git a/durf_amd/csrc/mlp_fwd.hip b/durf_amd/csrc/mlp_fwd.hip
--- a/durf_amd/csrc/mlp_fwd.hip
+++ b/durf_amd/csrc/mlp_fwd.hip
@@ -68,34 +68,6 @@
     });
 }
 
-template <bool RELU, bool BITS>
-__device__ __forceinline__ unsigned pack_tile(const f32x16& acc, bf16x8& o0, bf16x8& o1) {
-    static_assert(RELU || !BITS, "mask bits are taken from the ReLU output");
-#pragma unroll
-    for (int e = 0; e < 8; e++) {
-        float v0 = acc[e], v1 = acc[8 + e];
-        if (RELU) {
-            v0 = __builtin_amdgcn_fmed3f(v0, 0.0f, 3.0e38f);
-            v1 = __builtin_amdgcn_fmed3f(v1, 0.0f, 3.0e38f);
-        }
-        o0[e] = (__bf16)v0;
-        o1[e] = (__bf16)v1;
-    }
-    unsigned bits = 0;
-    if (BITS) {
-        typedef unsigned u32x4_ __attribute__((ext_vector_type(4)));
-        const u32x4_ d0 = __builtin_bit_cast(u32x4_, o0), d1 = __builtin_bit_cast(u32x4_, o1);
-        const unsigned ones = 0x00010001u;
-#pragma unroll
-        for (int j = 0; j < 8; j++) {
-            unsigned t;
-            const unsigned d = j < 4 ? d0[j & 3] : d1[j & 3];
-            asm("v_pk_min_u16 %0, %1, %2" : "=v"(t) : "v"(d), "s"(ones));
-            asm("v_lshl_or_b32 %0, %1, %2, %0" : "+v"(bits) : "v"(t), "n"(j));
-        }
-    }
-    return bits;
-}
 
 template <int SLOT, int NA, int NB, int NMT, bool RELU, bool TRAIN, int PREV_NMT, bool STORE_OUT = true>
 __device__ __forceinline__ void run_stage(WPipe& p, const bf16x8* inA, const bf16x8* inB,
@@ -683,8 +655,9 @@
     uint4 mcarry = make_uint4(0u, 0u, 0u, 0u);
 #define ST(j) (TRAIN ? stash_at(j) : nullptr)
 #define MK(j) (TRAIN ? mask_at(j) : nullptr)
-    run_stage<SLOT, 0, S::KE, S::WT, true, TRAIN, 0>(p, nullptr, encf, a, GW, ST(0), tile_valid, nullptr, nullptr, nullptr, mcarry);
-    run_stage<SLOT, S::KW, 0, S::WT, true, TRAIN, S::WT>(p, a, nullptr, b, GW, ST(1), tile_valid, a, ST(0), MK(0), mcarry);
+    const bool keep_h0 = !(TRAIN && W == 256 && (ei.flags & DURF_FWD_NO_H0) != 0);
+    run_stage<SLOT, 0, S::KE, S::WT, true, TRAIN, 0>(p, nullptr, encf, a, GW, ST(0), tile_valid && keep_h0, nullptr, nullptr, nullptr, mcarry);
+    run_stage<SLOT, S::KW, 0, S::WT, true, TRAIN, S::WT>(p, a, nullptr, b, GW, ST(1), tile_valid, a, keep_h0 ? ST(0) : nullptr, MK(0), mcarry);
     run_stage<SLOT, S::KW, 0, S::WT, true, TRAIN, S::WT>(p, b, nullptr, a, GW, ST(2), tile_valid, b, ST(1), MK(1), mcarry);
     run_stage<SLOT, S::KW, 0, S::WT, true, TRAIN, S::WT>(p, a, nullptr, b, GW, ST(3), tile_valid, a, ST(2), MK(2), mcarry);
     run_stage<SLOT, S::KW, 0, S::WT, true, TRAIN, S::WT>(p, b, nullptr, a, G5, ST(4), tile_valid, b, ST(3), MK(3), mcarry);
@@ -785,6 +758,8 @@
   }
 }
 
+namespace durf { void resolve_no_h0(EncIn* ei, int width, size_t rows, const void* stash, const void* wpack_fwd); }
+
 extern "C" {
 
 size_t durf_mlp_param_count(int width, int in_dim) { return durf_layer_offset(width, in_dim, 12, 0); }
@@ -872,6 +847,7 @@
     EncIn ei;
     if (int rc = fwd_enc_args(rows, N, t_vals, origins_s, dirs_s, radii, hit, K, enc_flags, enc_tile, ray_idx, count, stash, tail_idx,
                               tail_count, view_tile, &ei)) return rc;
+    durf::resolve_no_h0(&ei, 256, rows, stash, wpack_fwd);
     MsFwd ow{};
     ow.rows = rows; ow.N = N; ow.enc = (const bf16x8*)obj_enc; ow.view = (const bf16x8*)view_bf16; ow.ray_idx = obj_idx;
     ow.count = obj_count; ow.wpack = (const char*)obj_wpack_fwd; ow.raw = obj_raw; ow.stash = (bf16x8*)obj_stash;
@@ -914,6 +890,12 @@
 
 namespace durf {
 
+void resolve_no_h0(EncIn* ei, int width, size_t rows, const void* stash, const void* wpack_fwd) {
+    const bool train_bkgd = width == 256 && stash != nullptr;
+    if (!(train_bkgd && step_policy(rows).h0_recompute)) ei->flags &= ~DURF_FWD_NO_H0;
+    if (train_bkgd) note_h0_stash(stash, (ei->flags & DURF_FWD_NO_H0) ? wpack_fwd : nullptr);
+}
+
 int pack_bwd_launch(void* stream, int width, int in_dim, int K, const float* params, size_t param_stride, void* wpack_bwd);
 
 int launch_pack(void* stream, int width, int in_dim, int K, const float* params, size_t param_stride,
@@ -951,7 +933,9 @@
     const MlpBlockShape shape = mlp_block_shape(width, K, rows, false);
     const bool half = shape.half;
     dim3 grid(shape.grid_x, K), block(shape.block);
-    const EncIn ei = enc_in ? *enc_in : EncIn{};
+    EncIn ei = enc_in ? *enc_in : EncIn{};
+    if (K == 1) resolve_no_h0(&ei, width, rows, stash, wpack_fwd);
+    else ei.flags &= ~DURF_FWD_NO_H0;
     if (msplit) {
         dim3 g(ms_grid((size_t)K * durf_cdiv(rows, 64))), b(256);
         const MsFwd A{rows, N, (const bf16x8*)enc_tile, (const bf16x8*)view_bf16, ray_idx, count, (const char*)wpack_fwd, raw,
diff --git a/durf_amd/csrc/mlp_spec.h b/durf_amd/csrc/mlp_spec.h
--- a/durf_amd/csrc/mlp_spec.h
+++ b/durf_amd/csrc/mlp_spec.h
@@ -131,6 +131,58 @@
         if constexpr (i & 1) hook(std::integral_constant<int, ks>{});
     });
 }
+
+template <bool RELU, bool BITS>
+__device__ __forceinline__ unsigned pack_tile(const f32x16& acc, bf16x8& o0, bf16x8& o1) {
+    static_assert(RELU || !BITS, "mask bits are taken from the ReLU output");
+#pragma unroll
+    for (int e = 0; e < 8; e++) {
+        float v0 = acc[e], v1 = acc[8 + e];
+        if (RELU) {
+            v0 = __builtin_amdgcn_fmed3f(v0, 0.0f, 3.0e38f);
+            v1 = __builtin_amdgcn_fmed3f(v1, 0.0f, 3.0e38f);
+        }
+        o0[e] = (__bf16)v0;
+        o1[e] = (__bf16)v1;
+    }
+    unsigned bits = 0;
+    if (BITS) {
+        typedef unsigned u32x4_ __attribute__((ext_vector_type(4)));
+        const u32x4_ d0 = __builtin_bit_cast(u32x4_, o0), d1 = __builtin_bit_cast(u32x4_, o1);
+        const unsigned ones = 0x00010001u;
+#pragma unroll
+        for (int j = 0; j < 8; j++) {
+            unsigned t;
+            const unsigned d = j < 4 ? d0[j & 3] : d1[j & 3];
+            asm("v_pk_min_u16 %0, %1, %2" : "=v"(t) : "v"(d), "s"(ones));
+            asm("v_lshl_or_b32 %0, %1, %2, %0" : "+v"(bits) : "v"(t), "n"(j));
+        }
+    }
+    return bits;
+}
+
+template <int W>
+struct Dense0Frags {
+    using S = MlpSpec<W>;
+    bf16x8 A[S::KE];
+    f32x4 b[4];
+    __device__ __forceinline__ void load(const char* wpack, int mo, int lane) {
+        const char* wt = wpack + (size_t)(S::stage_chunk_base(0) + mo * S::tile_chunks(0)) * 1024;
+#pragma unroll
+        for (int k = 0; k < S::KE; k++) A[k] = *(const bf16x8*)(wt + k * 1024 + lane * 16);
+        const f32x4* bp = (const f32x4*)(wt + S::KE * 1024 + (lane >> 5) * 64);
+#pragma unroll
+        for (int g = 0; g < 4; g++) b[g] = bp[g];
+    }
+    __device__ __forceinline__ void apply(const bf16x8* enc, bf16x8& o0, bf16x8& o1) const {
+        f32x16 acc;
+#pragma unroll
+        for (int g = 0; g < 4; g++) { acc[4 * g] = b[g][0]; acc[4 * g + 1] = b[g][1]; acc[4 * g + 2] = b[g][2]; acc[4 * g + 3] = b[g][3]; }
+#pragma unroll
+        for (int k = 0; k < S::KE; k++) acc = __builtin_amdgcn_mfma_f32_32x32x16_bf16(A[k], enc[k], acc, 0, 0, 0);
+        pack_tile<true, false>(acc, o0, o1);
+    }
+};
 
 struct WPipe {
     i32x4 rsrc;
diff --git a/durf_amd/csrc/policy.h b/durf_amd/csrc/policy.h
--- a/durf_amd/csrc/policy.h
+++ b/durf_amd/csrc/policy.h
@@ -9,6 +9,7 @@
     bool side_fwd, side_bwd, side_dw;
     bool msplit;
     bool mix_enabled;
+    bool h0_recompute;
     bool side() const { return side_fwd || side_bwd || side_dw; }
     unsigned bits() const {
         return (side_fwd ? DURF_POLICY_SIDE_FWD : 0u) | (side_bwd ? DURF_POLICY_SIDE_BWD : 0u) | (side_dw ? DURF_POLICY_SIDE_DW : 0u) |
@@ -22,12 +23,14 @@
     if (e == nullptr || !strcmp(e, "auto")) e = large ? "2" : "0";
     const char* ms = getenv("DURF_OBJ_MSPLIT");
     const char* mx = getenv("DURF_OBJ_MIX");
+    const char* h0 = getenv("DURF_DENSE0_RECOMPUTE");
     StepPolicy p;
     p.side_dw = !strcmp(e, "2");
     p.side_bwd = p.side_dw || !strcmp(e, "3");
     p.side_fwd = p.side_bwd || !strcmp(e, "1");
     p.msplit = !large && !(ms && ms[0] == '0');
     p.mix_enabled = p.msplit && !(mx && mx[0] == '0');
+    p.h0_recompute = !(h0 && h0[0] == '0');
     return p;
 }
 
diff --git a/durf_amd/csrc/train.hip b/durf_amd/csrc/train.hip
--- a/durf_amd/csrc/train.hip
+++ b/durf_amd/csrc/train.hip
@@ -186,6 +186,7 @@
     const durf::StepPolicy policy = durf::step_policy(rows);
     const durf::Overlap ov = durf::overlap_for(stream, policy, Kb);
     const bool mix = Kb > 0 && !ov.sd && policy.mix_enabled && N % 32 == 0;
+    const int fwd_flags = f.enc_flags | (f32o ? 0 : DURF_FWD_NO_H0);
     for (int lvl = 0; lvl < L; lvl++) {
         float* t_vals = f.t_vals[lvl];
         if (ov.sd) {
@@ -197,14 +198,14 @@
         if (K > 0) {
             if (mix)
                 TIMED(DURF_TIMED_FWD + lvl,
-                      durf_mlp_fwd_enc_obj(stream, rows, N, t_vals, w.o_s, w.d_s, f.radii, w.hit, K, f.enc_flags | DURF_FWD_RAW_FULL,
+                      durf_mlp_fwd_enc_obj(stream, rows, N, t_vals, w.o_s, w.d_s, f.radii, w.hit, K, fwd_flags | DURF_FWD_RAW_FULL,
                                            w.enc[lvl], w.view, w.idx_cls, w.count_cls, w.wf_bkgd, w.raw_b[lvl], w.stash[lvl], w.mask[lvl],
                                            w.idx_cls + B, w.count_cls + 1, lvl == 0 ? w.view_tile : nullptr, B, w.idx_obj, w.count_obj,
                                            f.barf_w, obj_flags, w.wf_obj, w.obj_enc[lvl], w.obj_raw[lvl], w.obj_stash[lvl], w.obj_mask[lvl],
                                            lvl == 0 ? w.obj_view_tile : nullptr));
             else
             TIMED(DURF_TIMED_FWD + lvl,
-                  durf_mlp_fwd_enc(stream, rows, N, t_vals, w.o_s, w.d_s, f.radii, w.hit, K, f.enc_flags | (f32o ? 0 : DURF_FWD_RAW_FULL),
+                  durf_mlp_fwd_enc(stream, rows, N, t_vals, w.o_s, w.d_s, f.radii, w.hit, K, fwd_flags | (f32o ? 0 : DURF_FWD_RAW_FULL),
                                    w.enc[lvl], w.view, w.idx_cls, w.count_cls, w.wf_bkgd, f32o ? w.raw_c[lvl] : w.raw_b[lvl], w.stash[lvl],
                                    w.mask[lvl], w.idx_cls + B, w.count_cls + 1, lvl == 0 ? w.view_tile : nullptr));
             if (f32o && lvl == 0) {
@@ -226,7 +227,7 @@
             STEP(ov.join());
         } else {
             TIMED(DURF_TIMED_FWD + lvl,
-                  durf_mlp_fwd_enc(stream, rows, N, t_vals, w.o_s, w.d_s, f.radii, nullptr, 0, f.enc_flags, w.enc[lvl], w.view, nullptr,
+                  durf_mlp_fwd_enc(stream, rows, N, t_vals, w.o_s, w.d_s, f.radii, nullptr, 0, fwd_flags, w.enc[lvl], w.view, nullptr,
                                    nullptr, w.wf_bkgd, w.raw_b[lvl], w.stash[lvl], w.mask[lvl], nullptr, nullptr,
                                    lvl == 0 ? w.view_tile : nullptr));
         }
diff --git a/durf_amd/obbpose_model.py b/durf_amd/obbpose_model.py
--- a/durf_amd/obbpose_model.py
+++ b/durf_amd/obbpose_model.py
@@ -261,6 +261,7 @@
         ctx = dict(o_s=o_s, d_s=d_s, hit=hit, zo=zo, idx=idx, count=count, slot=slot, view=view,
                    packs=packs, levels=[], B=B, N=N, K=Kd, ts=ts, policy=ops.step_policy(rows), bkgd_mode=bk, view_tiles_obj=view_tiles_obj,
                    obj_f32=obj_f32 or (f32 and bool(Kd)), obj_x3=obj_f32 and self.object_x3())
+        ctx['h0_recompute'] = bool(train and not f32 and not ctx['obj_f32'] and not static_f32 and ops.FUSED_ENCODE)
         obj_flat = None
         if ctx['obj_f32']:
             o0 = lay.mlp_off['BoxMLP_0']
@@ -313,6 +314,8 @@
                 mask_b = torch.empty(ops.mlp_mask_bytes(rows), dtype=torch.uint8, device=dev) if train else None
                 side = ops.on_side(dev, bool(Kb) and ctx['policy'].side_fwd)
                 enc_kw = dict(contraction=self.contraction, disable_integration=self.disable_integration, cylinder=cyl)
+                if ctx['h0_recompute']:
+                    enc_kw['no_h0'] = True
                 slabs = None
                 obj_first = bool(Kb) and side.enabled
 
diff --git a/durf_amd/ops.py b/durf_amd/ops.py
--- a/durf_amd/ops.py
+++ b/durf_amd/ops.py
@@ -360,14 +360,14 @@
 
 def mlp_fwd_enc(rows, N, t_vals, origins_s, dirs_s, radii, hit, view_bf16, wpack_fwd, contraction=True,
                 disable_integration=False, cylinder=False, ray_idx=None, count=None, stash=None, raw=None, relu_mask=None,
-                tail_idx=None, tail_count=None, view_tile=None, raw_full=False):
+                tail_idx=None, tail_count=None, view_tile=None, raw_full=False, no_h0=False):
     dev = t_vals.device
     K = 0 if hit is None else hit.shape[1]
     if raw is None:
         raw = torch.empty(rows, 4, device=dev)
     enc_tile = torch.empty(tile_rows(rows), ENC_DIM, dtype=torch.bfloat16, device=dev)
     flags = ((ENC_CONTRACT if contraction else 0) | (ENC_NO_INTEGRATION if disable_integration else 0) |
-             (ENC_CYLINDER if cylinder else 0) | (FWD_RAW_FULL if raw_full else 0))
+             (ENC_CYLINDER if cylinder else 0) | (FWD_RAW_FULL if raw_full else 0) | (FWD_NO_H0 if no_h0 else 0))
     with _Timed('mlp_fwd_256%s' % ('_train' if stash is not None else '')):
         _lib.check(_lib.lib().durf_mlp_fwd_enc(_stream(), rows, N, _p(_f32(t_vals)), _p(_f32(origins_s)), _p(_f32(dirs_s)),
                                                _p(_f32(radii)), _p(hit), K, flags, _p(enc_tile), _p(view_bf16),
@@ -836,13 +836,13 @@
 
 def mlp_fwd_enc_obj(rows, N, t_vals, origins_s, dirs_s, radii, hit, view_bf16, wpack_fwd, slabs, obj_idx, obj_count, alpha, obj_wf,
                     ray_idx, count, tail_idx, tail_count, stash, relu_mask, contraction=True, disable_integration=False,
-                    cylinder=False, view_tile=None, raw_full=True, obj_view_tile=None):
+                    cylinder=False, view_tile=None, raw_full=True, obj_view_tile=None, no_h0=False):
     dev = t_vals.device
     K = hit.shape[1]
     raw = torch.empty(rows, 4, device=dev)
     enc_tile = torch.empty(tile_rows(rows), ENC_DIM, dtype=torch.bfloat16, device=dev)
     flags = ((ENC_CONTRACT if contraction else 0) | (ENC_NO_INTEGRATION if disable_integration else 0) |
-             (ENC_CYLINDER if cylinder else 0) | (FWD_RAW_FULL if raw_full else 0))
+             (ENC_CYLINDER if cylinder else 0) | (FWD_RAW_FULL if raw_full else 0) | (FWD_NO_H0 if no_h0 else 0))
     wa = (C.c_float * 10)(*[float(x) for x in barf_weights(alpha)])
     with _Timed('mlp_fwd_256%s' % ('_train' if stash is not None else '')):
         _lib.check(_lib.lib().durf_mlp_fwd_enc_obj(
diff --git a/include/durf_ctypes_stub.py b/include/durf_ctypes_stub.py
--- a/include/durf_ctypes_stub.py
+++ b/include/durf_ctypes_stub.py
@@ -12,6 +12,7 @@
 DURF_ENC_NO_INTEGRATION = 2
 DURF_ENC_CYLINDER = 4
 DURF_FWD_RAW_FULL = 8
+DURF_FWD_NO_H0 = 16
 DURF_ENC_DIM = 64
 DURF_VIEW_DIM = 32
 DURF_DISPATCH_FWD256_8W = 0x1
diff --git a/include/durf_hip.h b/include/durf_hip.h
--- a/include/durf_hip.h
+++ b/include/durf_hip.h
@@ -16,6 +16,7 @@
 #define DURF_ENC_NO_INTEGRATION 2
 #define DURF_ENC_CYLINDER 4
 #define DURF_FWD_RAW_FULL 8
+#define DURF_FWD_NO_H0 16
 #define DURF_ENC_DIM 64
 #define DURF_VIEW_DIM 32
 
```
